# MIC-DKFZ/MultiTalent

Measured on AMD Instinct MI355X. Metric: CT patches/s (48x192x192) train fwd+bwd, higher is better.
Workload: dtype f32; 1 GPU; Task009_Spleen Generic_UNet nc=2 softmax Dice+CE; batch_per_gpu=2, global_batch=2, parallelism=dp1, step=fwd+loss+bwd+clip12+SGD-nesterov, precision=fp32

## Files before the change

multitalent_amd/csrc/conv_bf16.inc:

```
#define BFP 12
#ifndef BF_SWZ
#define BF_SWZ 1
#endif
#define BFP_SWZ 8
#define BF_BPF 6
#ifndef BF_ABL
#define BF_ABL 0
#endif

#include "conv16_common.h"

template <int LD, int LH, int NW> __host__ __device__ constexpr int bstage_rows() { return ((LD * LH + NW - 1) / NW) * NW; }
template <int LD, int LH, int LW, int VEC, int NW, int PITCH = BFP> __host__ __device__ constexpr int bstage_lwp() {
  constexpr int vps = 64 / (FCK / VEC);
  constexpr int padded = ((LW + vps - 1) / vps) * vps;
  return ((size_t)bstage_rows<LD, LH, NW>() * padded * PITCH * 4 <= (PITCH == BFP ? 80 : 40) * 1024) ? padded : LW;
}
template <int LD, int LH, int LW, int VEC, int NW, int PITCH = BFP> __host__ __device__ constexpr size_t bstage_lds_bytes() {
  return (size_t)bstage_rows<LD, LH, NW>() * bstage_lwp<LD, LH, LW, VEC, NW, PITCH>() * PITCH * 4;
}

template <int LD, int LH, int LW, int VEC, int NW, int XS = MT_F32, int MTY = MT_BF16, int PITCH = BFP>
__device__ __forceinline__ void mt_stage_bf16(unsigned* __restrict__ lds, const mt_conv3d_t& c, const ConvChunk ch,
                                              int nb, int ud0, int uh0, int uw0, int lane, int wave) {
  constexpr int EB = mt_ebytes<XS>();
  constexpr bool XB = XS != MT_F32;
  constexpr int LPV = FCK / VEC, VPS = 64 / LPV, NI = (LW + VPS - 1) / VPS, R = LD * LH, RPW = (R + NW - 1) / NW;
  constexpr int LWP = bstage_lwp<LD, LH, LW, VEC, NW, PITCH>();
  constexpr bool PADW = LWP >= NI * VPS;
  constexpr bool SWZ = PITCH == BFP_SWZ;
  constexpr int RG = (RPW * NI * VEC > 64) ? (RPW + 1) / 2 : RPW;
  typedef float f32x2 __attribute__((ext_vector_type(2)));
  const mt_src_t& S = c.src[ch.src];
  const int cl = (lane % LPV) * VEC, vl = lane / LPV;
  const bool has_aff = S.scale != nullptr;
  float sc[VEC], sh[VEC];
#pragma unroll
  for (int e = 0; e < VEC; ++e) {
    const bool cv = (cl + e) < ch.ck;
    sc[e] = cv ? 1.f : 0.f; sh[e] = 0.f;
    if (has_aff && cv) {
      sc[e] = S.scale[(size_t)nb * S.C + ch.c0 + cl + e];
      sh[e] = S.shift[(size_t)nb * S.C + ch.c0 + cl + e];
    }
  }
  const float slope = has_aff ? S.slope : 1.f;
  const int cs = S.cs;
  const size_t sample_elems = (size_t)c.Di * c.Hi * c.Wi * cs;
  __amdgpu_buffer_rsrc_t rsrc =
      __builtin_amdgcn_make_buffer_rsrc((void*)((const char*)S.ptr + (size_t)nb * sample_elems * EB), 0, (int)(sample_elems * EB), 0x00020000);
  int voff[NI];
  unsigned mval[NI];
#pragma unroll
  for (int i = 0; i < NI; ++i) {
    const int lw = vl + i * VPS;
    const int uw = uw0 + lw;
    const bool ok = (lw < LW) && ((unsigned)uw < (unsigned)c.Wi);
    voff[i] = ok ? (uw * cs + ch.c0 + cl) * EB : (int)0x80000000;
    mval[i] = ok ? 0xffffffffu : 0u;
  }
  unsigned* lbase = lds + (wave * LWP + vl) * PITCH + (SWZ ? (cl & 7) / 2 : cl / 2);
  int hoff[NI];
#pragma unroll
  for (int i = 0; i < NI; ++i) hoff[i] = SWZ ? (((cl >> 3) ^ ((vl + i * VPS) >> 3)) & 1) * 4 : 0;
  const int rowbytes = c.Wi * cs * EB;
  if constexpr (XB && XS == MTY && VEC == 4) {
    if (!has_aff) {
      unsigned cm[2];
      cm[0] = ((cl < ch.ck) ? 0x0000ffffu : 0u) | ((cl + 1 < ch.ck) ? 0xffff0000u : 0u);
      cm[1] = ((cl + 2 < ch.ck) ? 0x0000ffffu : 0u) | ((cl + 3 < ch.ck) ? 0xffff0000u : 0u);
#pragma unroll
      for (int r0 = 0; r0 < RPW; r0 += RG) {
        uint2 rw[RG][NI];
#pragma unroll
        for (int q = 0; q < RG; ++q) {
          if (r0 + q < RPW) {
            const int row = wave + NW * (r0 + q);
            const int ld = row / LH, lhh = row - ld * LH;
            const int ud = ud0 + ld, uh = uh0 + lhh;
            const int rm = ((row < R) && ((unsigned)ud < (unsigned)c.Di) && ((unsigned)uh < (unsigned)c.Hi)) ? -1 : 0;
            const int srow = ((ud * c.Hi + uh) & rm) * rowbytes;
            const int oob = ~rm & (int)0x80000000;
#pragma unroll
            for (int i = 0; i < NI; ++i) rw[q][i] = __builtin_bit_cast(uint2, __builtin_amdgcn_raw_buffer_load_b64(rsrc, voff[i] | oob, srow, 0));
          }
        }
#pragma unroll
        for (int q = 0; q < RG; ++q) {
          if (r0 + q < RPW) {
            unsigned* lrow = lbase + NW * (r0 + q) * (LWP * PITCH);
#pragma unroll
            for (int i = 0; i < NI; ++i) {
              if (PADW || (i + 1) * VPS <= LW || vl + i * VPS < LW) {
                uint2 t; t.x = rw[q][i].x & cm[0]; t.y = rw[q][i].y & cm[1];
                *(uint2*)(lrow + i * VPS * PITCH + hoff[i]) = t;
              }
            }
          }
        }
      }
      return;
    }
  }
#pragma unroll
  for (int r0 = 0; r0 < RPW; r0 += RG) {
    float v[RG][NI][VEC];
    int rowm[RG];
#pragma unroll
    for (int q = 0; q < RG; ++q) {
      if (r0 + q < RPW) {
        const int row = wave + NW * (r0 + q);
        const int ld = row / LH, lhh = row - ld * LH;
        const int ud = ud0 + ld, uh = uh0 + lhh;
        rowm[q] = ((row < R) && ((unsigned)ud < (unsigned)c.Di) && ((unsigned)uh < (unsigned)c.Hi)) ? -1 : 0;
        const int srow = ((ud * c.Hi + uh) & rowm[q]) * rowbytes;
        const int oob = ~rowm[q] & (int)0x80000000;
#pragma unroll
        for (int i = 0; i < NI; ++i) {
          if constexpr (XB && VEC == 4) {
            const uint2 t = __builtin_bit_cast(uint2, __builtin_amdgcn_raw_buffer_load_b64(rsrc, voff[i] | oob, srow, 0));
            v[q][i][0] = mt_lo16<XS>(t.x); v[q][i][1] = mt_hi16<XS>(t.x); v[q][i][2] = mt_lo16<XS>(t.y); v[q][i][3] = mt_hi16<XS>(t.y);
          } else if constexpr (XB) {
            const unsigned t = __builtin_amdgcn_raw_buffer_load_b32(rsrc, voff[i] | oob, srow, 0);
            v[q][i][0] = mt_lo16<XS>(t); v[q][i][1] = mt_hi16<XS>(t);
          } else if constexpr (VEC == 4) {
            const f32x4 t = __builtin_bit_cast(f32x4, __builtin_amdgcn_raw_buffer_load_b128(rsrc, voff[i] | oob, srow, 0));
            v[q][i][0] = t[0]; v[q][i][1] = t[1]; v[q][i][2] = t[2]; v[q][i][3] = t[3];
          } else {
            const float2 t = __builtin_bit_cast(float2, __builtin_amdgcn_raw_buffer_load_b64(rsrc, voff[i] | oob, srow, 0));
            v[q][i][0] = t.x; v[q][i][1] = t.y;
          }
        }
      }
    }
#pragma unroll
    for (int q = 0; q < RG; ++q) {
      if (r0 + q < RPW) {
        float scq[VEC], shq[VEC];
#pragma unroll
        for (int e = 0; e < VEC; ++e) {
          scq[e] = __builtin_bit_cast(float, __builtin_bit_cast(unsigned, sc[e]) & (unsigned)rowm[q]);
          shq[e] = __builtin_bit_cast(float, __builtin_bit_cast(unsigned, sh[e]) & (unsigned)rowm[q]);
        }
        unsigned* lrow = lbase + NW * (r0 + q) * (LWP * PITCH);
#pragma unroll
        for (int i = 0; i < NI; ++i) {
          unsigned pk[VEC / 2];
#pragma unroll
          for (int h = 0; h < VEC / 2; ++h) {
            f32x2 xv2, sc2, sh2, sl2;
            xv2[0] = v[q][i][2 * h]; xv2[1] = v[q][i][2 * h + 1];
            sc2[0] = scq[2 * h]; sc2[1] = scq[2 * h + 1]; sh2[0] = shq[2 * h]; sh2[1] = shq[2 * h + 1];
            sl2[0] = slope; sl2[1] = slope;
            const f32x2 t = __builtin_elementwise_fma(xv2, sc2, sh2);
            const f32x2 u = t * sl2;
            pk[h] = mt_pk16<MTY>(fmaxf(t[0], u[0]), fmaxf(t[1], u[1])) & mval[i];
          }
          if (PADW || (i + 1) * VPS <= LW || vl + i * VPS < LW) {
            if constexpr (VEC == 4) {
              uint2 t; t.x = pk[0]; t.y = pk[1];
              *(uint2*)(lrow + i * VPS * PITCH + hoff[i]) = t;
            } else {
              lrow[i * VPS * PITCH + hoff[i]] = pk[0];
            }
          }
        }
      }
    }
  }
}

template <int MT, int NT, int LH, int LW, int KD = 3, int MTY = MT_BF16, int PITCH = BFP>
__device__ __forceinline__ void bf16_chunk(const unsigned* __restrict__ lds, const int (&abase)[MT][3],
                                           const unsigned* __restrict__ wlane, int wstride, f32x16 (&acc)[NT][MT]) {
  constexpr int NTAP = KD * 9;
  constexpr int NB = BF_BPF + 1;
  bf16x8 b[NB][NT];
  bf16x8 a[2][MT];
#pragma unroll
  for (int t = 0; t < BF_BPF; ++t)
#pragma unroll
    for (int n = 0; n < NT; ++n) b[t][n] = *(const bf16x8*)(wlane + n * wstride + t * 256);
#pragma unroll
  for (int m = 0; m < MT; ++m) a[0][m] = *(const bf16x8*)(lds + abase[m][0]);
#pragma unroll
  for (int t = 0; t < NTAP; ++t) {
    if (t + BF_BPF < NTAP)
#pragma unroll
      for (int n = 0; n < NT; ++n) b[(t + BF_BPF) % NB][n] = *(const bf16x8*)(wlane + n * wstride + (t + BF_BPF) * 256);
    if (t + 1 < NTAP) {
      const int t1 = t + 1;
      const int toff = (((t1 / 9) * LH + (t1 / 3) % 3) * LW + t1 % 3) * PITCH;
#pragma unroll
      for (int m = 0; m < MT; ++m) a[t1 & 1][m] = *(const bf16x8*)(lds + abase[m][t1 % 3] + toff);
    }
    __builtin_amdgcn_sched_barrier(0);
#pragma unroll
    for (int m = 0; m < MT; ++m)
#pragma unroll
      for (int n = 0; n < NT; ++n)
        acc[n][m] = mt_mfma16<MTY>(a[t & 1][m], b[t % NB][n], acc[n][m]);
    __builtin_amdgcn_sched_barrier(0);
  }
}


template <int MW, int RH, int TD, int VEC, int NT, int NW, int KD = 3, int XS = MT_F32, int OS = MT_F32, int MTY = MT_BF16>
__global__ __launch_bounds__(64 * NW) __attribute__((amdgpu_waves_per_eu(TD == 4 ? 3 : 4))) void conv_bf16_kernel(const ConvKParams P) {
  constexpr bool OB = OS != MT_F32;
  constexpr int MH = 32 / MW, TH = MH * RH, TW = MW, NMT = TD * RH, MT = NMT / NW;
  constexpr int PITCH = BF_SWZ ? BFP_SWZ : BFP;
  constexpr int LD = TD + KD - 1, LH = TH + 2, LW = TW + 2, LWP = bstage_lwp<LD, LH, LW, VEC, NW, PITCH>();
  constexpr int NTAP = KD * 9;
  static_assert(NMT % NW == 0, "M tiles must split over the waves");
  extern __shared__ __attribute__((aligned(16))) unsigned ldsu[];
  const mt_conv3d_t& c = P.c;
  const int tid = threadIdx.x, lane = tid & 63;
  const int wave = __builtin_amdgcn_readfirstlane(tid >> 6);
  const int li = lane & 31, lhalf = lane >> 5;
  int ntile_b, td, th, tw, nb;
  const int tile = mt_block_decode(ntile_b);
  const int ntile0 = ntile_b * NT;
  mt_tile_coords(tile, P.tilesD, P.tilesH, P.tilesW, td, th, tw, nb);
  const int sb = (td * P.tilesH + th) * P.tilesW + tw;
  const int od0 = td * TD, oh0 = th * TH, ow0 = tw * TW;

  int abase[MT][3];
#pragma unroll
  for (int m = 0; m < MT; ++m) {
    const int mt = wave * MT + m;
    const int dm = mt / RH, rh = mt % RH;
    const int r = li / MW, col = li % MW;
#pragma unroll
    for (int kw = 0; kw < 3; ++kw)
      abase[m][kw] = ((dm * LH + rh * MH + r) * LWP + col) * PITCH + (BF_SWZ ? ((lhalf ^ ((col + kw) >> 3)) & 1) : lhalf) * 4;
  }
  f32x16 acc[NT][MT];
#pragma unroll
  for (int n = 0; n < NT; ++n)
#pragma unroll
    for (int m = 0; m < MT; ++m)
#pragma unroll
      for (int j = 0; j < 16; ++j) acc[n][m][j] = 0.f;

  const unsigned* wbase = (const unsigned*)c.wpack;
  const int wstride = P.nchunks * (NTAP * 256);
  for (int ch = 0; ch < P.nchunks; ++ch) {
    const ConvChunk cc = P.chunk[ch];
    const unsigned* wlane = wbase + (size_t)(ntile0 * P.nchunks + ch) * (NTAP * 256) + lane * 4;
    __syncthreads();
    if (!(BF_ABL & 1)) mt_stage_bf16<LD, LH, LW, VEC, NW, XS, MTY, PITCH>(ldsu, c, cc, nb, od0 - (KD - 1) / 2, oh0 - 1, ow0 - 1, lane, wave);
    __syncthreads();
    if (!(BF_ABL & 8)) bf16_chunk<MT, NT, LH, LWP, KD, MTY, PITCH>(ldsu, abase, wlane, wstride, acc);
  }

  if (BF_ABL & 4) { if (acc[0][0][0] == 12345.678f) c.out0[0] = acc[NT - 1][MT - 1][3]; return; }
  float* lds = (float*)ldsu;
  if (c.stats_part != nullptr) __syncthreads();
  float a1[NT], a2[NT];
  bf16_store_tile<MW, RH, TD, NT, NW, OS>(c, acc, wave, lane, nb, od0, oh0, ow0, ntile0, a1, a2);
  if (c.stats_part != nullptr) {
#pragma unroll
    for (int n = 0; n < NT; ++n)
      if (lhalf == 0) { lds[((n * NW + wave) * 32 + li) * 2] = a1[n]; lds[((n * NW + wave) * 32 + li) * 2 + 1] = a2[n]; }
  }
  if (c.stats_part != nullptr) {
    __syncthreads();
    if (tid < 32 * NT) {
      const int n = tid >> 5, l = tid & 31;
      const int co = (ntile0 + n) * 32 + l;
      if (co < c.Cout) {
        float t1 = 0.f, t2 = 0.f;
#pragma unroll
        for (int w = 0; w < NW; ++w) { t1 += lds[((n * NW + w) * 32 + l) * 2]; t2 += lds[((n * NW + w) * 32 + l) * 2 + 1]; }
        float* sp = c.stats_part + ((size_t)((size_t)nb * P.nsb + sb) * c.Cout + co) * 2;
        sp[0] = t1; sp[1] = t2;
      }
    }
  }
}
```

multitalent_amd/csrc/conv_lds.hip:

```cpp
#include "mt_common.h"
#include "bwdw_common.h"
#include "conv_stage.h"
#include <cstring>
#include <stdlib.h>
#include <type_traits>


__device__ __forceinline__ int mt_block_decode(int& ntile) {
  const int ny = (int)gridDim.y;
  const int b = mt_xcd_remap((int)(blockIdx.x + gridDim.x * blockIdx.y), (int)(gridDim.x * ny));
  const int t = b / ny;
  ntile = b - t * ny;
  return t;
}
__device__ __forceinline__ void mt_tile_coords(int tile, int tilesD, int tilesH, int tilesW, int& td, int& th, int& tw, int& nb) {
  td = tile % tilesD; tile /= tilesD;
  th = tile % tilesH; tile /= tilesH;
  tw = tile % tilesW;
  nb = tile / tilesW;
}

template <int CK, int LD, int LH, int LW>
__device__ __forceinline__ void mt_stage_fast(float* __restrict__ lds, const mt_conv3d_t& c, const ConvChunk ch,
                                              int nb, int ud0, int uh0, int uw0, int lane, int wave) {
// ... 392 lines not shown
    a[0][m][1] = *(const f32x4*)(lds + abase[m] + 4);
  }
#pragma unroll
  for (int t = 0; t < NTAP; ++t) {
    if (t + CF_BPF < NTAP && !(CF_ABL & 64)) {
      b[(t + CF_BPF) % NB][0] = *(const f32x4*)(wlane + (t + CF_BPF) * 512);
      b[(t + CF_BPF) % NB][1] = *(const f32x4*)(wlane + (t + CF_BPF) * 512 + 256);
    }
    if (t + 1 < NTAP && !(CF_ABL & 32)) {
      const int t1 = t + 1;
      const int toff = (((t1 / 9) * LH + (t1 / 3) % 3) * LW + t1 % 3) * FCKP;
#pragma unroll
      for (int m = 0; m < MT; ++m) {
        a[t1 & 1][m][0] = *(const f32x4*)(lds + abase[m] + toff);
        a[t1 & 1][m][1] = *(const f32x4*)(lds + abase[m] + toff + 4);
      }
    }
    __builtin_amdgcn_sched_barrier(0);
#pragma unroll
    for (int kp = 0; kp < 8; ++kp)
#pragma unroll
      for (int m = 0; m < MT; ++m)
        acc[m] = __builtin_amdgcn_mfma_f32_32x32x2f32(a[(CF_ABL & 32) ? 0 : (t & 1)][m][kp >> 2][kp & 3], b[(CF_ABL & 64) ? 0 : (t % NB)][kp >> 2][kp & 3], acc[m], 0, 0, 0);
    __builtin_amdgcn_sched_barrier(0);
  }
}

template <int MW, int RH, int TD, int VEC, int KD = 3>
__global__ __launch_bounds__(256) void conv_fast_kernel(const ConvKParams P) {
  constexpr int MH = 32 / MW, TH = MH * RH, TW = MW, NMT = TD * RH, MT = NMT / 4;
  constexpr int LD = TD + KD - 1, LH = TH + 2, LW = TW + 2, LWP = stage_lwp<LD, LH, LW, VEC>();
  static_assert(NMT % 4 == 0, "M tiles must split over 4 waves");
  extern __shared__ __attribute__((aligned(16))) float lds[];
  const mt_conv3d_t& c = P.c;
  const int tid = threadIdx.x, lane = tid & 63;
  const int wave = __builtin_amdgcn_readfirstlane(tid >> 6);
  const int li = lane & 31, lhalf = lane >> 5;
  int ntile, td, th, tw, nb;
  mt_tile_coords(mt_block_decode(ntile), P.tilesD, P.tilesH, P.tilesW, td, th, tw, nb);
  const int sb = (td * P.tilesH + th) * P.tilesW + tw;
  const int od0 = td * TD, oh0 = th * TH, ow0 = tw * TW;

  int abase[MT];
#pragma unroll
  for (int m = 0; m < MT; ++m) {
    const int mt = wave * MT + m;
    const int dm = mt / RH, rh = mt % RH;
    const int r = li / MW, col = li % MW;
    abase[m] = ((dm * LH + rh * MH + r) * LWP + col) * FCKP + lhalf * 8;
  }
  f32x16 acc[MT];
#pragma unroll
  for (int m = 0; m < MT; ++m)
#pragma unroll
    for (int j = 0; j < 16; ++j) acc[m][j] = 0.f;

  for (int ch = 0; ch < P.nchunks; ++ch) {
    const ConvChunk cc = P.chunk[ch];
    const float* wlane = c.wpack + (size_t)(ntile * P.nchunks + ch) * (KD * 9 * 512) + lane * 4;
    if (!(CF_ABL & 16)) __syncthreads();
    if (!(CF_ABL & 1)) mt_stage_fast2<LD, LH, LW, VEC>(lds, c, cc, nb, od0 - (KD - 1) / 2, oh0 - 1, ow0 - 1, lane, wave);
    if (!(CF_ABL & 16)) __syncthreads();
    if (!(CF_ABL & 8)) fast_chunk<MT, LH, LWP, KD>(lds, abase, wlane, acc);
  }

  if (CF_ABL & 4) { if (acc[0][0] == 12345.678f) c.out0[0] = acc[MT - 1][3]; return; }
  const int co = ntile * 32 + li;
  const bool covalid = co < c.Cout;
  const float bv = (c.bias != nullptr && covalid) ? c.bias[co] : 0.f;
  float* optr; int ocs, cofs;
  if (co < c.csplit) { optr = c.out0; ocs = c.ocs0; cofs = co; }
  else               { optr = c.out1; ocs = c.ocs1; cofs = co - c.csplit; }
  float s1 = 0.f, s2 = 0.f;
  const bool interior = (od0 + TD <= c.Do) && (oh0 + TH <= c.Ho) && (ow0 + TW <= c.Wo);
  const size_t out_sample = (size_t)c.Do * c.Ho * c.Wo;
  __amdgpu_buffer_rsrc_t r0d = __builtin_amdgcn_make_buffer_rsrc((void*)(c.out0 + (size_t)nb * out_sample * c.ocs0), 0,
                                                                 (int)(out_sample * c.ocs0 * 4), 0x00020000);
  const bool split = c.csplit < c.Cout;
  __amdgpu_buffer_rsrc_t r1d = r0d;
  if (split) r1d = __builtin_amdgcn_make_buffer_rsrc((void*)(c.out1 + (size_t)nb * out_sample * c.ocs1), 0,
                                                     (int)(out_sample * c.ocs1 * 4), 0x00020000);
  const bool use1 = split && !(co < c.csplit);
  (void)optr;
  const int lane_col = 4 * lhalf;
  const int loff = covalid ? (lane_col * ocs + cofs) * 4 : (int)0x80000000;
#pragma unroll
  for (int m = 0; m < MT; ++m) {
    const int mt = wave * MT + m;
    const int dm = mt / RH, rh = mt % RH;
    const int od = od0 + dm;
    const int vox0 = ((od * c.Ho) + (oh0 + rh * MH)) * c.Wo + ow0;
    auto jgeom = [&](int j, int& off, int& so0, int& so1) {
      const int ivj = (j & 3) + 8 * (j >> 2);
      const int r = ivj / MW, colj = ivj % MW;
      off = loff;
      if (!interior) {
        const bool ok = (od < c.Do) && (oh0 + rh * MH + r < c.Ho) && (ow0 + colj + lane_col < c.Wo);
        off = ok ? loff : (int)0x80000000;
      }
      so0 = (vox0 + r * c.Wo + colj) * c.ocs0 * 4;
      so1 = (vox0 + r * c.Wo + colj) * c.ocs1 * 4;
    };
    float prev[16];
    if (c.accumulate) {
#pragma unroll
      for (int j = 0; j < 16; ++j) {
        int off, so0, so1; jgeom(j, off, so0, so1);
        if (!split) prev[j] = __builtin_bit_cast(float, __builtin_amdgcn_raw_buffer_load_b32(r0d, off, so0, 0));
        else {
          const int offa = use1 ? (int)0x80000000 : off, offb = use1 ? off : (int)0x80000000;
          prev[j] = __builtin_bit_cast(float, __builtin_amdgcn_raw_buffer_load_b32(r0d, offa, so0, 0)) +
                    __builtin_bit_cast(float, __builtin_amdgcn_raw_buffer_load_b32(r1d, offb, so1, 0));
        }
      }
    }
#pragma unroll
    for (int j = 0; j < 16; ++j) {
      int off, so0, so1; jgeom(j, off, so0, so1);
      float v = acc[m][j] + bv;
      if (c.accumulate) v += prev[j];
      if (!split) {
        __builtin_amdgcn_raw_buffer_store_b32(__builtin_bit_cast(unsigned, v), r0d, off, so0, 0);
      } else {
        const int offa = use1 ? (int)0x80000000 : off, offb = use1 ? off : (int)0x80000000;
        __builtin_amdgcn_raw_buffer_store_b32(__builtin_bit_cast(unsigned, v), r0d, offa, so0, 0);
        __builtin_amdgcn_raw_buffer_store_b32(__builtin_bit_cast(unsigned, v), r1d, offb, so1, 0);
      }
      if (interior) { s1 += v; s2 = fmaf(v, v, s2); }
      else if (off >= 0) { s1 += v; s2 = fmaf(v, v, s2); }
    }
  }
  if (!covalid) { s1 = 0.f; s2 = 0.f; }
  if (c.stats_part != nullptr) {
    s1 += __shfl_xor(s1, 32, 64);
    s2 += __shfl_xor(s2, 32, 64);
    __syncthreads();
    if (lhalf == 0) { lds[(wave * 32 + li) * 2] = s1; lds[(wave * 32 + li) * 2 + 1] = s2; }
    __syncthreads();
    if (tid < 32 && (ntile * 32 + tid) < c.Cout) {
      float t1 = 0.f, t2 = 0.f;
#pragma unroll
      for (int w = 0; w < 4; ++w) { t1 += lds[(w * 32 + tid) * 2]; t2 += lds[(w * 32 + tid) * 2 + 1]; }
      float* sp = c.stats_part + ((size_t)((size_t)nb * P.nsb + sb) * c.Cout + ntile * 32 + tid) * 2;
      sp[0] = t1; sp[1] = t2;
    }
  }
}

#include "conv_bf16.inc"

#ifndef FS_ABL
#define FS_ABL 0
#endif
template <int SD, int SH, int SW, int VEC, bool BF = false, int XS = MT_F32, int OS = MT_F32, int MTY = MT_BF16>
__global__ __launch_bounds__(256) void conv_fast_strided_kernel(const ConvKParams P) {
  static_assert(BF || (XS == MT_F32 && OS == MT_F32), "16-bit storage is served by the 16-bit matrix path");
  constexpr bool OB = OS != MT_F32;
  constexpr int TD = 2, TH = 4, TW = 8;
  constexpr int LD = (TD - 1) * SD + 3, LH = (TH - 1) * SH + 3, LW = (TW - 1) * SW + 3;
  constexpr int LWP = BF ? bstage_lwp<LD, LH, LW, VEC, 4>() : stage_lwp<LD, LH, LW, VEC>();
  constexpr int PITCH = BF ? BFP : FCKP;
  extern __shared__ __attribute__((aligned(16))) float lds[];
  const mt_conv3d_t& c = P.c;
  const int tid = threadIdx.x, lane = tid & 63;
  const int wave = __builtin_amdgcn_readfirstlane(tid >> 6);
  const int li = lane & 31, lhalf = lane >> 5;
  int by, td, th, tw, nb;
  mt_tile_coords(mt_block_decode(by), P.tilesD, P.tilesH, P.tilesW, td, th, tw, nb);
  const int dm = wave & 1, nt2 = wave >> 1;
  const int ntile_raw = by * 2 + nt2;
  const bool nt_ok = ntile_raw * 32 < c.Cout;
  const int ntile = nt_ok ? ntile_raw : 0;
  const int sb = (td * P.tilesH + th) * P.tilesW + tw;
  const int od0 = td * TD, oh0 = th * TH, ow0 = tw * TW;

  int abase[1];
  abase[0] = ((dm * SD * LH + (li >> 3) * SH) * LWP + (li & 7) * SW) * PITCH + lhalf * (BF ? 4 : 8);
  f32x16 accb[1][1];
  f32x16 (&acc)[1] = accb[0];
#pragma unroll
  for (int j = 0; j < 16; ++j) acc[0][j] = 0.f;

  for (int ch = 0; ch < P.nchunks; ++ch) {
    const ConvChunk cc = P.chunk[ch];
    __syncthreads();
    if constexpr (BF) {
      const unsigned* wlane = (const unsigned*)c.wpack + (size_t)(ntile * P.nchunks + ch) * (27 * 256) + lane * 4;
      mt_stage_bf16<LD, LH, LW, VEC, 4, XS, MTY>((unsigned*)lds, c, cc, nb, od0 * SD - 1, oh0 * SH - 1, ow0 * SW - 1, lane, wave);
      __syncthreads();
      const int abase3[1][3] = {{abase[0], abase[0], abase[0]}};
      bf16_chunk<1, 1, LH, LWP, 3, MTY>((const unsigned*)lds, abase3, wlane, 0, accb);
    } else {
      const float* wlane = c.wpack + (size_t)(ntile * P.nchunks + ch) * (27 * 512) + lane * 4;
      if (!(FS_ABL & 1)) mt_stage_fast2<LD, LH, LW, VEC>(lds, c, cc, nb, od0 * SD - 1, oh0 * SH - 1, ow0 * SW - 1, lane, wave);
      __syncthreads();
      if (!(FS_ABL & 8)) fast_chunk<1, LH, LWP>(lds, abase, wlane, acc);
    }
  }
  if ((FS_ABL & 4) && acc[0][0] != 12345.f) return;

  const int co = ntile_raw * 32 + li;
  const bool covalid = nt_ok && co < c.Cout;
  const float bv = (c.bias != nullptr && covalid) ? c.bias[co] : 0.f;
  const int ocs = c.ocs0;
  const size_t out_sample = (size_t)c.Do * c.Ho * c.Wo;
  constexpr int OEB = mt_ebytes<OS>();
  __amdgpu_buffer_rsrc_t rd = __builtin_amdgcn_make_buffer_rsrc((void*)((char*)c.out0 + (size_t)nb * out_sample * ocs * OEB), 0,
                                                                (int)(out_sample * ocs * OEB), 0x00020000);
  const int od = od0 + dm;
  float s1 = 0.f, s2 = 0.f;
  if constexpr (OB) {
    const bool odd = li & 1;
    const int coe = co & ~1;
    const bool pvalid = nt_ok && coe + 1 < c.Cout;
    float q1[2] = {0.f, 0.f}, q2[2] = {0.f, 0.f};
#pragma unroll
    for (int j = 0; j < 16; j += 2) {
      const int iv = (j & 3) + 8 * (j >> 2) + 4 * lhalf + (odd ? 1 : 0);
      const int oh = oh0 + (iv >> 3), ow = ow0 + (iv & 7);
      const bool ok = pvalid && (od < c.Do) && (oh < c.Ho) && (ow < c.Wo);
      const int off = ok ? (((od * c.Ho + oh) * c.Wo + ow) * ocs + coe) * 2 : (int)0x80000000;
      float a, b;
      mt_pair_exchange(acc[0][j] + bv, acc[0][j + 1] + bv, odd, a, b);
      if (c.accumulate) { const unsigned pv = __builtin_amdgcn_raw_buffer_load_b32(rd, off, 0, 0); a += mt_lo16<OS>(pv); b += mt_hi16<OS>(pv); }
      const unsigned pk = mt_pk16<OS>(a, b);
      __builtin_amdgcn_raw_buffer_store_b32(pk, rd, off, 0, 0);
      if (ok) {
        const float ar = mt_lo16<OS>(pk), br = mt_hi16<OS>(pk);
        q1[0] += ar; q2[0] = fmaf(ar, ar, q2[0]); q1[1] += br; q2[1] = fmaf(br, br, q2[1]);
      }
    }
    s1 = mt_pair_combine(q1[0], q1[1], odd);
    s2 = mt_pair_combine(q2[0], q2[1], odd);
  } else {
#pragma unroll
  for (int j = 0; j < 16; ++j) {
    const int iv = (j & 3) + 8 * (j >> 2) + 4 * lhalf;
    const int oh = oh0 + (iv >> 3), ow = ow0 + (iv & 7);
    const bool ok = covalid && (od < c.Do) && (oh < c.Ho) && (ow < c.Wo);
    const int off = ok ? (((od * c.Ho + oh) * c.Wo + ow) * ocs + co) * 4 : (int)0x80000000;
    float v = acc[0][j] + bv;
    if (c.accumulate) v += __builtin_bit_cast(float, __builtin_amdgcn_raw_buffer_load_b32(rd, off, 0, 0));
    __builtin_amdgcn_raw_buffer_store_b32(__builtin_bit_cast(unsigned, v), rd, off, 0, 0);
    if (ok) { s1 += v; s2 = fmaf(v, v, s2); }
  }
  }
  if (c.stats_part != nullptr) {
    s1 += __shfl_xor(s1, 32, 64);
    s2 += __shfl_xor(s2, 32, 64);
    __syncthreads();
    if (lhalf == 0) { lds[(wave * 32 + li) * 2] = s1; lds[(wave * 32 + li) * 2 + 1] = s2; }
    __syncthreads();
    if (tid < 64) {
      const int n2 = tid >> 5, cl = tid & 31;
      const int cg = (by * 2 + n2) * 32 + cl;
      if (cg < c.Cout) {
        const float t1 = lds[((n2 * 2) * 32 + cl) * 2] + lds[((n2 * 2 + 1) * 32 + cl) * 2];
        const float t2 = lds[((n2 * 2) * 32 + cl) * 2 + 1] + lds[((n2 * 2 + 1) * 32 + cl) * 2 + 1];
        float* sp = c.stats_part + ((size_t)((size_t)nb * P.nsb + sb) * c.Cout + cg) * 2;
        sp[0] = t1; sp[1] = t2;
      }
    }
  }
}

#ifndef TS_ABL
#define TS_ABL 0
#endif
template <int VEC, bool BF = false, int XS = MT_F32, int OS = MT_F32, int MTY = MT_BF16, int SD = 1, int SH = 1, int SW = 1>
__global__ __launch_bounds__(256) void conv_tapsplit_kernel(const ConvKParams P) {
  static_assert(BF || (XS == MT_F32 && OS == MT_F32), "16-bit storage is served by the 16-bit matrix path");
  constexpr int TD = 2, TH = 4, TW = 4, LD = (TD - 1) * SD + 3, LH = (TH - 1) * SH + 3, LW = (TW - 1) * SW + 3;
  constexpr int LWP = BF ? bstage_lwp<LD, LH, LW, VEC, 4>() : stage_lwp<LD, LH, LW, VEC>();
  constexpr int PITCH = BF ? BFP : FCKP;
  extern __shared__ __attribute__((aligned(16))) float lds[];
  const mt_conv3d_t& c = P.c;
  const int tid = threadIdx.x, lane = tid & 63;
  const int wave = __builtin_amdgcn_readfirstlane(tid >> 6);
  const int li = lane & 31, lhalf = lane >> 5;
  int ntile, td, th, tw, nb;
  mt_tile_coords(mt_block_decode(ntile), P.tilesD, P.tilesH, P.tilesW, td, th, tw, nb);
  const int sb = (td * P.tilesH + th) * P.tilesW + tw;
  const int od0 = td * TD, oh0 = th * TH, ow0 = tw * TW;
  const int abase = (((li >> 4) * SD * LH + ((li >> 2) & 3) * SH) * LWP + (li & 3) * SW) * PITCH + lhalf * (BF ? 4 : 8);

  f32x16 acc;
#pragma unroll
  for (int j = 0; j < 16; ++j) acc[j] = 0.f;

  for (int ch = 0; ch < P.nchunks; ++ch) {
    const ConvChunk cc = P.chunk[ch];
    __syncthreads();
    if constexpr (BF) {
      mt_stage_bf16<LD, LH, LW, VEC, 4, XS, MTY>((unsigned*)lds, c, cc, nb, od0 * SD - 1, oh0 * SH - 1, ow0 * SW - 1, lane, wave);
      __syncthreads();
      const unsigned* ldsu = (const unsigned*)lds;
      const unsigned* wl = (const unsigned*)c.wpack + (size_t)(ntile * P.nchunks + ch) * (27 * 256) + lane * 4;
      bf16x8 fa[7], fb[7];
#pragma unroll
      for (int i = 0; i < 7; ++i) {
        const int tt = (wave + 4 * i) < 27 ? wave + 4 * i : 26;
        fa[i] = *(const bf16x8*)(ldsu + abase + (((tt / 9) * LH + (tt / 3) % 3) * LWP + tt % 3) * PITCH);
        fb[i] = *(const bf16x8*)(wl + tt * 256);
      }
#pragma unroll
      for (int i = 0; i < 7; ++i)
        if (i < 6 || wave < 3) acc = mt_mfma16<MTY>(fa[i], fb[i], acc);
      continue;
    }
    const float* wlane = c.wpack + ((TS_ABL & 2) ? (size_t)0 : (size_t)(ntile * P.nchunks + ch) * (27 * 512)) + lane * 4;
    if (!(TS_ABL & 1)) mt_stage_fast2<LD, LH, LW, VEC>(lds, c, cc, nb, od0 * SD - 1, oh0 * SH - 1, ow0 * SW - 1, lane, wave);
    __syncthreads();
    f32x4 a[2][2], b[2][2];
    {
      const int t = wave;
      const int toff = (((t / 9) * LH + (t / 3) % 3) * LWP + t % 3) * FCKP;
      a[0][0] = *(const f32x4*)(lds + abase + toff); a[0][1] = *(const f32x4*)(lds + abase + toff + 4);
      b[0][0] = *(const f32x4*)(wlane + t * 512);    b[0][1] = *(const f32x4*)(wlane + t * 512 + 256);
    }
#pragma unroll
    for (int i = 0; i < 7; ++i) {
      const int t = wave + 4 * i, t1 = t + 4;
      if (i + 1 < 7) {
        const int tt = t1 < 27 ? t1 : 26;
        const int toff = (((tt / 9) * LH + (tt / 3) % 3) * LWP + tt % 3) * FCKP;
        a[(i + 1) & 1][0] = *(const f32x4*)(lds + abase + toff); a[(i + 1) & 1][1] = *(const f32x4*)(lds + abase + toff + 4);
        b[(i + 1) & 1][0] = *(const f32x4*)(wlane + tt * 512);   b[(i + 1) & 1][1] = *(const f32x4*)(wlane + tt * 512 + 256);
      }
      if (i < 6 || wave < 3) {
        if (TS_ABL & 4) { acc[0] += a[i & 1][0][0] + a[i & 1][1][3] + b[i & 1][0][1] + b[i & 1][1][2]; continue; }
#pragma unroll
        for (int kp = 0; kp < 8; ++kp)
          acc = __builtin_amdgcn_mfma_f32_32x32x2f32(a[i & 1][kp >> 2][kp & 3], b[i & 1][kp >> 2][kp & 3], acc, 0, 0, 0);
      }
    }
  }

  __syncthreads();
  float* red = lds;
#pragma unroll
  for (int j = 0; j < 16; ++j) red[(wave * 16 + j) * 64 + lane] = acc[j];
  __syncthreads();
  float v[4];
#pragma unroll
  for (int jj = 0; jj < 4; ++jj) {
    const float* rp = red + ((wave * 4 + jj)) * 64 + lane;
    v[jj] = ((rp[0] + rp[16 * 64]) + rp[32 * 64]) + rp[48 * 64];
  }
  const int co = ntile * 32 + li;
  const bool covalid = co < c.Cout;
// ... 513 lines not shown
}

template <int MT>
__device__ __forceinline__ void rt_frag_load(FastFrag<MT>& f, const float* __restrict__ lds, const int (&abase)[MT], int off,
                                             const float* __restrict__ wq) {
  f.b[0] = *(const f32x4*)(wq);
  f.b[1] = *(const f32x4*)(wq + 256);
#pragma unroll
  for (int m = 0; m < MT; ++m) {
    const float* a = lds + abase[m] + off;
    f.a[m][0] = *(const f32x4*)(a);
    f.a[m][1] = *(const f32x4*)(a + 4);
  }
}

template <int MW, int RH, int TD, int VEC>
__global__ __launch_bounds__(256) void conv_rt_kernel(const ConvKParams P) {
  constexpr int MH = 32 / MW, TH = MH * RH, TW = MW, NMT = TD * RH, MT = NMT / 4;
  static_assert(NMT % 4 == 0, "M tiles must split over 4 waves");
  extern __shared__ __attribute__((aligned(16))) float lds[];
  const mt_conv3d_t& c = P.c;
  const int tid = threadIdx.x, lane = tid & 63;
  const int wave = __builtin_amdgcn_readfirstlane(tid >> 6);
  const int li = lane & 31, lhalf = lane >> 5;
  int ntile, td, th, tw, nb;
  mt_tile_coords(mt_block_decode(ntile), P.tilesD, P.tilesH, P.tilesW, td, th, tw, nb);
  const int sb = (td * P.tilesH + th) * P.tilesW + tw;
  const int LD = (TD - 1) * c.SD + c.KD, LH = (TH - 1) * c.SH + c.KH, LW = (TW - 1) * c.SW + c.KW;
  const int od0 = td * TD, oh0 = th * TH, ow0 = tw * TW;

  int abase[MT];
#pragma unroll
  for (int m = 0; m < MT; ++m) {
    const int mt = wave * MT + m;
    const int dm = mt / RH, rh = mt % RH;
    const int r = li / MW, col = li % MW;
    abase[m] = ((dm * c.SD * LH + (rh * MH + r) * c.SH) * LW + col * c.SW) * FCKP + lhalf * 8;
  }
  f32x16 acc[MT];
#pragma unroll
  for (int m = 0; m < MT; ++m)
#pragma unroll
    for (int j = 0; j < 16; ++j) acc[m][j] = 0.f;

  const int ntaps = P.ntaps;
  const int step_w = FCKP, step_h = (LW - c.KW) * FCKP, step_d = (LH - c.KH) * LW * FCKP;
  for (int ch = 0; ch < P.nchunks; ++ch) {
    const ConvChunk cc = P.chunk[ch];
    const float* wq = c.wpack + (size_t)(ntile * P.nchunks + ch) * ntaps * 512 + lane * 4;
    __syncthreads();
    mt_stage_rt<VEC>(lds, c, cc, nb, od0 * c.SD - c.PD, oh0 * c.SH - c.PH, ow0 * c.SW - c.PW, LD, LH, LW, lane, wave);
    __syncthreads();
    FastFrag<MT> f0, f1;
    int off = 0, kw = 0, kh = 0, tap = 0;
    auto advance = [&]() {
      if (tap + 1 < ntaps) {
        off += step_w;
        if (++kw == c.KW) { kw = 0; off += step_h; if (++kh == c.KH) { kh = 0; off += step_d; } }
        wq += 512;
      }
      ++tap;
    };
    rt_frag_load<MT>(f0, lds, abase, off, wq);
    while (tap + 2 <= ntaps) {
      advance();
      __builtin_amdgcn_sched_barrier(0);
      rt_frag_load<MT>(f1, lds, abase, off, wq);
      __builtin_amdgcn_sched_barrier(0);
      fast_frag_mfma<MT>(f0, acc);
      __builtin_amdgcn_sched_barrier(0);
      advance();
      __builtin_amdgcn_sched_barrier(0);
      rt_frag_load<MT>(f0, lds, abase, off, wq);
      __builtin_amdgcn_sched_barrier(0);
      fast_frag_mfma<MT>(f1, acc);
      __builtin_amdgcn_sched_barrier(0);
    }
    if (tap < ntaps) fast_frag_mfma<MT>(f0, acc);
  }

  const int co = ntile * 32 + li;
  const bool covalid = co < c.Cout;
  const float bv = (c.bias != nullptr && covalid) ? c.bias[co] : 0.f;
  const int osD = c.osD > 0 ? c.osD : 1, osH = c.osH > 0 ? c.osH : 1, osW = c.osW > 0 ? c.osW : 1;
  const int OD = c.osD > 0 ? c.OD : c.Do, OH = c.osD > 0 ? c.OH : c.Ho, OW = c.osD > 0 ? c.OW : c.Wo;
  const int ooD = c.osD > 0 ? c.ooD : 0, ooH = c.osD > 0 ? c.ooH : 0, ooW = c.osD > 0 ? c.ooW : 0;
  const bool split = c.csplit < c.Cout;
  const bool use1 = split && co >= c.csplit;
  const int ocs = use1 ? c.ocs1 : c.ocs0;
  const int cofs = use1 ? co - c.csplit : co;
  const size_t out_sample = (size_t)OD * OH * OW;
  __amdgpu_buffer_rsrc_t rd = __builtin_amdgcn_make_buffer_rsrc((void*)(c.out0 + (size_t)nb * out_sample * c.ocs0), 0,
                                                                (int)(out_sample * c.ocs0 * 4), 0x00020000);
  __amdgpu_buffer_rsrc_t rd1 = rd;
  if (split) rd1 = __builtin_amdgcn_make_buffer_rsrc((void*)(c.out1 + (size_t)nb * out_sample * c.ocs1), 0,
                                                     (int)(out_sample * c.ocs1 * 4), 0x00020000);
  const int m0 = use1 ? (int)0x80000000 : 0, m1 = use1 ? 0 : (int)0x80000000;
  const int lane_col = 4 * lhalf;
  float s1 = 0.f, s2 = 0.f;
#pragma unroll
  for (int m = 0; m < MT; ++m) {
    const int mt = wave * MT + m;
    const int dm = mt / RH, rh = mt % RH;
    const int od = od0 + dm;
    auto jgeom = [&](int j, bool& ok) -> int {
      const int ivj = (j & 3) + 8 * (j >> 2);
      const int r = ivj / MW, colj = ivj % MW;
      const int oh = oh0 + rh * MH + r, ow = ow0 + colj + lane_col;
      ok = covalid && (od < c.Do) && (oh < c.Ho) && (ow < c.Wo);
      const int vox = ((od * osD + ooD) * OH + (oh * osH + ooH)) * OW + (ow * osW + ooW);
      return ok ? (vox * ocs + cofs) * 4 : (int)0x80000000;
    };
    float prev[16];
    if (c.accumulate) {
#pragma unroll
      for (int j = 0; j < 16; ++j) {
        bool ok; const int off = jgeom(j, ok);
        prev[j] = __builtin_bit_cast(float, __builtin_amdgcn_raw_buffer_load_b32(rd, off | m0, 0, 0));
        if (split) prev[j] += __builtin_bit_cast(float, __builtin_amdgcn_raw_buffer_load_b32(rd1, off | m1, 0, 0));
      }
    }
#pragma unroll
    for (int j = 0; j < 16; ++j) {
      bool ok; const int off = jgeom(j, ok);
      float v = acc[m][j] + bv;
      if (c.accumulate) v += prev[j];
      __builtin_amdgcn_raw_buffer_store_b32(__builtin_bit_cast(unsigned, v), rd, off | m0, 0, 0);
      if (split) __builtin_amdgcn_raw_buffer_store_b32(__builtin_bit_cast(unsigned, v), rd1, off | m1, 0, 0);
      if (ok) { s1 += v; s2 = fmaf(v, v, s2); }
    }
  }
  if (c.stats_part != nullptr) {
    s1 += __shfl_xor(s1, 32, 64);
    s2 += __shfl_xor(s2, 32, 64);
    __syncthreads();
    if (lhalf == 0) { lds[(wave * 32 + li) * 2] = s1; lds[(wave * 32 + li) * 2 + 1] = s2; }
    __syncthreads();
    if (tid < 32 && (ntile * 32 + tid) < c.Cout) {
      float t1 = 0.f, t2 = 0.f;
#pragma unroll
      for (int w = 0; w < 4; ++w) { t1 += lds[(w * 32 + tid) * 2]; t2 += lds[(w * 32 + tid) * 2 + 1]; }
      float* sp = c.stats_part + ((size_t)((size_t)nb * P.nsb + sb) * c.Cout + ntile * 32 + tid) * 2;
      sp[0] = t1; sp[1] = t2;
    }
  }
}

template <int S> __host__ __device__ constexpr int bd_par(int k) { return S == 2 ? (k == 1 ? 0 : 1) : 0; }
template <int S> __host__ __device__ constexpr int bd_off(int k) { return S == 2 ? (k == 0 ? 1 : 0) : 2 - k; }

#ifndef BDS_ABL
#define BDS_ABL 0
#endif
template <int SD, int SH, int SW, int VEC, bool BF = false, int XS = MT_F32, int OS = MT_F32>
__global__ __launch_bounds__(256) __attribute__((amdgpu_waves_per_eu(2))) void conv_bwdd_strided_kernel(const ConvKParams P) {
  static_assert(BF || (XS == MT_F32 && OS == MT_F32), "16-bit storage is served by the bf16 matrix path");
  constexpr bool OB = OS != MT_F32;
  constexpr int TD = 2, TH = 4, TW = 16;
  constexpr int LD = TD + (SD == 2 ? 1 : 2), LH = TH + (SH == 2 ? 1 : 2), LW = TW + (SW == 2 ? 1 : 2);
  constexpr int NC = SD * SH * SW, LWP = BF ? bstage_lwp<LD, LH, LW, VEC, 4>() : stage_lwp<LD, LH, LW, VEC>();
  constexpr int PITCH = BF ? BFP : FCKP;
  extern __shared__ __attribute__((aligned(16))) float lds[];
  const mt_conv3d_t& c = P.c;
  const int tid = threadIdx.x, lane = tid & 63;
  const int wave = __builtin_amdgcn_readfirstlane(tid >> 6);
  const int li = lane & 31, lhalf = lane >> 5;
  int ntile, td, th, tw, nb;
  mt_tile_coords(mt_block_decode(ntile), P.tilesD, P.tilesH, P.tilesW, td, th, tw, nb);
  const int md0 = td * TD, mh0 = th * TH, mw0 = tw * TW;

  const int dm = wave >> 1, rbase = (wave & 1) * 2;
  const int abase = ((dm * LH + rbase + (li >> 4)) * LWP + (li & 15)) * PITCH + lhalf * (BF ? 4 : 8);

  f32x16 acc[NC];
#pragma unroll
  for (int q = 0; q < NC; ++q)
#pragma unroll
    for (int j = 0; j < 16; ++j) acc[q][j] = 0.f;

  for (int ch = 0; ch < P.nchunks; ++ch) {
    const ConvChunk cc = P.chunk[ch];
    const float* wlane = c.wpack + (size_t)(ntile * P.nchunks + ch) * (27 * 512) + lane * 4;
    __syncthreads();
    if constexpr (BF) {
      mt_stage_bf16<LD, LH, LW, VEC, 4, XS, MT_BF16>((unsigned*)lds, c, cc, nb, md0 - (SD == 1 ? 1 : 0), mh0 - (SH == 1 ? 1 : 0), mw0 - (SW == 1 ? 1 : 0), lane, wave);
      __syncthreads();
      const unsigned* ldsu = (const unsigned*)lds;
      const unsigned* wl = (const unsigned*)c.wpack + (size_t)(ntile * P.nchunks + ch) * (27 * 256) + lane * 4;
      constexpr int BPF = 5, NB = BPF + 1;
      bf16x8 b[NB], a[2];
#pragma unroll
      for (int t = 0; t < BPF; ++t) b[t] = *(const bf16x8*)(wl + t * 256);
      {
        constexpr int o0 = ((bd_off<SD>(0) * LH + bd_off<SH>(0)) * LWP + bd_off<SW>(0)) * PITCH;
        a[0] = *(const bf16x8*)(ldsu + abase + o0);
      }
#pragma unroll
      for (int t = 0; t < 27; ++t) {
        if (t + BPF < 27) b[(t + BPF) % NB] = *(const bf16x8*)(wl + (t + BPF) * 256);
        if (t + 1 < 27) {
          const int t1 = t + 1;
          const int o1 = ((bd_off<SD>(t1 / 9) * LH + bd_off<SH>((t1 / 3) % 3)) * LWP + bd_off<SW>(t1 % 3)) * PITCH;
          a[t1 & 1] = *(const bf16x8*)(ldsu + abase + o1);
        }
        __builtin_amdgcn_sched_barrier(0);
        const int q = (bd_par<SD>(t / 9) * SH + bd_par<SH>((t / 3) % 3)) * SW + bd_par<SW>(t % 3);
        acc[q] = __builtin_amdgcn_mfma_f32_32x32x16_bf16(a[t & 1], b[t % NB], acc[q], 0, 0, 0);
        __builtin_amdgcn_sched_barrier(0);
      }
      continue;
    }
    if (!(BDS_ABL & 1)) mt_stage_fast2<LD, LH, LW, VEC>(lds, c, cc, nb, md0 - (SD == 1 ? 1 : 0), mh0 - (SH == 1 ? 1 : 0), mw0 - (SW == 1 ? 1 : 0), lane, wave);
    __syncthreads();
    if (BDS_ABL & 2) wlane = c.wpack + lane * 4;
    {
      constexpr int NB = 4;
      f32x4 b[NB][2];
      f32x4 a[2][2];
#pragma unroll
      for (int t = 0; t < 3; ++t) {
        b[t][0] = *(const f32x4*)(wlane + t * 512);
        b[t][1] = *(const f32x4*)(wlane + t * 512 + 256);
      }
      {
        constexpr int o0 = ((bd_off<SD>(0) * LH + bd_off<SH>(0)) * LWP + bd_off<SW>(0)) * FCKP;
        a[0][0] = *(const f32x4*)(lds + abase + o0);
        a[0][1] = *(const f32x4*)(lds + abase + o0 + 4);
      }
#pragma unroll
      for (int t = 0; t < 27; ++t) {
        if (t + 3 < 27 && !(BDS_ABL & 2)) {
          b[(t + 3) % NB][0] = *(const f32x4*)(wlane + (t + 3) * 512);
          b[(t + 3) % NB][1] = *(const f32x4*)(wlane + (t + 3) * 512 + 256);
        }
        if (t + 1 < 27) {
          const int t1 = t + 1;
          const int o1 = ((bd_off<SD>(t1 / 9) * LH + bd_off<SH>((t1 / 3) % 3)) * LWP + bd_off<SW>(t1 % 3)) * FCKP;
          a[t1 & 1][0] = *(const f32x4*)(lds + abase + o1);
          a[t1 & 1][1] = *(const f32x4*)(lds + abase + o1 + 4);
        }
        __builtin_amdgcn_sched_barrier(0);
        const int q = (bd_par<SD>(t / 9) * SH + bd_par<SH>((t / 3) % 3)) * SW + bd_par<SW>(t % 3);
        if (BDS_ABL & 8) { acc[q][0] += a[t & 1][0][0] + a[t & 1][1][3] + b[t % NB][0][1] + b[t % NB][1][2]; continue; }
#pragma unroll
        for (int e = 0; e < 4; ++e) acc[q] = __builtin_amdgcn_mfma_f32_32x32x2f32(a[t & 1][0][e], b[t % NB][0][e], acc[q], 0, 0, 0);
#pragma unroll
        for (int e = 0; e < 4; ++e) acc[q] = __builtin_amdgcn_mfma_f32_32x32x2f32(a[t & 1][1][e], b[t % NB][1][e], acc[q], 0, 0, 0);
        __builtin_amdgcn_sched_barrier(0);
      }
    }
  }

  const int co = ntile * 32 + li;
  const bool covalid = co < c.Cout;
  const int ocs = c.ocs0;
  const size_t out_sample = (size_t)c.OD * c.OH * c.OW;
  constexpr int OEB = mt_ebytes<OS>();
  __amdgpu_buffer_rsrc_t rd = __builtin_amdgcn_make_buffer_rsrc((void*)((char*)c.out0 + (size_t)nb * out_sample * ocs * OEB), 0,
                                                                (int)(out_sample * ocs * OEB), 0x00020000);
  const int md = md0 + dm;
  if (BDS_ABL & 4) { float t = 0.f; for (int q = 0; q < NC; ++q) t += acc[q][3] + acc[q][9]; if (t == 1234.5f) c.out0[0] = t; return; }
  if constexpr (OB) {
    const bool odd = li & 1;
    const int coe = co & ~1;
    const bool pvalid = coe + 1 < c.Cout;
    auto pair_off = [&](int j, int (&off)[NC]) {
      const int iv = (j & 3) + 8 * (j >> 2) + 4 * lhalf + (odd ? 1 : 0);
      const int mh = mh0 + rbase + (iv >> 4), mw = mw0 + (iv & 15);
#pragma unroll
      for (int q = 0; q < NC; ++q) {
        const int pd = q / (SH * SW), ph = (q / SW) % SH, pw = q % SW;
        const int xd = md * SD + pd, xh = mh * SH + ph, xw = mw * SW + pw;
        const bool ok = pvalid && xd < c.OD && xh < c.OH && xw < c.OW;
        off[q] = ok ? (((xd * c.OH + xh) * c.OW + xw) * ocs + coe) * 2 : (int)0x80000000;
      }
    };
    int poff[2][NC];
    unsigned pprev[2][NC];
    pair_off(0, poff[0]);
    if (c.accumulate) {
#pragma unroll
      for (int q = 0; q < NC; ++q) pprev[0][q] = __builtin_amdgcn_raw_buffer_load_b32(rd, poff[0][q], 0, 0);
    }
#pragma unroll
    for (int jp = 0; jp < 8; ++jp) {
      const int j = 2 * jp;
      if (jp + 1 < 8) {
        pair_off(j + 2, poff[(jp + 1) & 1]);
        if (c.accumulate) {
#pragma unroll
          for (int q = 0; q < NC; ++q) pprev[(jp + 1) & 1][q] = __builtin_amdgcn_raw_buffer_load_b32(rd, poff[(jp + 1) & 1][q], 0, 0);
        }
      }
#pragma unroll
      for (int q = 0; q < NC; ++q) {
        float a, b;
        mt_pair_exchange(acc[q][j], acc[q][j + 1], odd, a, b);
        if (c.accumulate) { a += mt_lo16<OS>(pprev[jp & 1][q]); b += mt_hi16<OS>(pprev[jp & 1][q]); }
        __builtin_amdgcn_raw_buffer_store_b32(mt_pk16<OS>(a, b), rd, poff[jp & 1][q], 0, 0);
      }
    }
    return;
  }
  auto row_off = [&](int j, int (&off)[NC]) {
    const int iv = (j & 3) + 8 * (j >> 2) + 4 * lhalf;
    const int mh = mh0 + rbase + (iv >> 4), mw = mw0 + (iv & 15);
#pragma unroll
    for (int q = 0; q < NC; ++q) {
      const int pd = q / (SH * SW), ph = (q / SW) % SH, pw = q % SW;
      const int xd = md * SD + pd, xh = mh * SH + ph, xw = mw * SW + pw;
      const bool ok = covalid && xd < c.OD && xh < c.OH && xw < c.OW;
      off[q] = ok ? (((xd * c.OH + xh) * c.OW + xw) * ocs + co) * 4 : (int)0x80000000;
    }
  };
  int off[2][NC];
  float prev[2][NC];
  row_off(0, off[0]);
  if (c.accumulate) {
#pragma unroll
    for (int q = 0; q < NC; ++q) prev[0][q] = __builtin_bit_cast(float, __builtin_amdgcn_raw_buffer_load_b32(rd, off[0][q], 0, 0));
  }
#pragma unroll
  for (int j = 0; j < 16; ++j) {
    if (j + 1 < 16) {
      row_off(j + 1, off[(j + 1) & 1]);
      if (c.accumulate) {
#pragma unroll
        for (int q = 0; q < NC; ++q)
          prev[(j + 1) & 1][q] = __builtin_bit_cast(float, __builtin_amdgcn_raw_buffer_load_b32(rd, off[(j + 1) & 1][q], 0, 0));
      }
    }
#pragma unroll
    for (int q = 0; q < NC; ++q) {
      float v = acc[q][j];
      if (c.accumulate) v += prev[j & 1][q];
      __builtin_amdgcn_raw_buffer_store_b32(__builtin_bit_cast(unsigned, v), rd, off[j & 1][q], 0, 0);
    }
  }
}

template <int SD, int SH, int SW>
__global__ __launch_bounds__(256) void conv_bwdd_strided_ks_kernel(const ConvKParams P) {
  constexpr int TD = 2, TH = 4, TW = 4;
  constexpr int LD = TD + (SD == 2 ? 1 : 2), LH = TH + (SH == 2 ? 1 : 2), LW = TW + (SW == 2 ? 1 : 2);
  constexpr int NC = SD * SH * SW, LWP = stage_lwp<LD, LH, LW, 2>();
  extern __shared__ __attribute__((aligned(16))) float lds[];
  const mt_conv3d_t& c = P.c;
  const int tid = threadIdx.x, lane = tid & 63;
  const int wave = __builtin_amdgcn_readfirstlane(tid >> 6);
  const int li = lane & 31, lhalf = lane >> 5;
  int ntile, td, th, tw, nb;
  mt_tile_coords(mt_block_decode(ntile), P.tilesD, P.tilesH, P.tilesW, td, th, tw, nb);
  const int md0 = td * TD, mh0 = th * TH, mw0 = tw * TW;
  const int abase = (((li >> 4) * LH + ((li >> 2) & 3)) * LWP + (li & 3)) * FCKP + lhalf * 8 + 2 * wave;

  f32x16 acc[NC];
#pragma unroll
  for (int q = 0; q < NC; ++q)
#pragma unroll
    for (int j = 0; j < 16; ++j) acc[q][j] = 0.f;
// ... 16 lines not shown
    for (int t = 0; t < 27; ++t) {
      if (t + 1 < 27) {
        const int t1 = t + 1;
        const int o1 = ((bd_off<SD>(t1 / 9) * LH + bd_off<SH>((t1 / 3) % 3)) * LWP + bd_off<SW>(t1 % 3)) * FCKP;
        a[t1 & 1] = *(const float2*)(lds + abase + o1);
      }
      const int q = (bd_par<SD>(t / 9) * SH + bd_par<SH>((t / 3) % 3)) * SW + bd_par<SW>(t % 3);
      acc[q] = __builtin_amdgcn_mfma_f32_32x32x2f32(a[t & 1].x, b[t].x, acc[q], 0, 0, 0);
      acc[q] = __builtin_amdgcn_mfma_f32_32x32x2f32(a[t & 1].y, b[t].y, acc[q], 0, 0, 0);
    }
  }

  const int co = ntile * 32 + li;
  const bool covalid = co < c.Cout;
  const int ocs = c.ocs0;
  const size_t out_sample = (size_t)c.OD * c.OH * c.OW;
  __amdgpu_buffer_rsrc_t rd = __builtin_amdgcn_make_buffer_rsrc((void*)(c.out0 + (size_t)nb * out_sample * ocs), 0, (int)(out_sample * ocs * 4), 0x00020000);
  float* red = lds;
  __syncthreads();
#pragma unroll
  for (int q = 0; q < NC; ++q) {
    const int pd = q / (SH * SW), ph = (q / SW) % SH, pw = q % SW;
    int off[4];
    float prev[4];
#pragma unroll
    for (int jj = 0; jj < 4; ++jj) {
      const int iv = jj + 8 * wave + 4 * lhalf;
      const int xd = (md0 + (iv >> 4)) * SD + pd, xh = (mh0 + ((iv >> 2) & 3)) * SH + ph, xw = (mw0 + (iv & 3)) * SW + pw;
      const bool ok = covalid && xd < c.OD && xh < c.OH && xw < c.OW;
      off[jj] = ok ? (((xd * c.OH + xh) * c.OW + xw) * ocs + co) * 4 : (int)0x80000000;
      prev[jj] = 0.f;
      if (c.accumulate) prev[jj] = __builtin_bit_cast(float, __builtin_amdgcn_raw_buffer_load_b32(rd, off[jj], 0, 0));
    }
#pragma unroll
    for (int j = 0; j < 16; ++j) red[(wave * 16 + j) * 64 + lane] = acc[q][j];
    __syncthreads();
#pragma unroll
    for (int jj = 0; jj < 4; ++jj) {
      const float* rp = red + (wave * 4 + jj) * 64 + lane;
      const float v = (((rp[0] + rp[16 * 64]) + rp[32 * 64]) + rp[48 * 64]) + prev[jj];
      __builtin_amdgcn_raw_buffer_store_b32(__builtin_bit_cast(unsigned, v), rd, off[jj], 0, 0);
    }
    __syncthreads();
  }
}

#include "conv_wino.inc"

struct ConvCfg { int MW, RH, TD, CK; };
static const ConvCfg kCfgs[] = {
  {32, 4, 2, 16}, {16, 2, 2, 16}, {8, 2, 2, 16}, {32, 4, 2, 8}, {16, 2, 2, 8}, {8, 2, 2, 8}, {32, 4, 4, 16},
};

static const ConvCfg kBfCfgs[] = { {32, 4, 4, 16}, {32, 4, 2, 16}, {16, 4, 2, 16} };

static void cfg_tile(const ConvCfg& g, int* TD, int* TH, int* TW) {
  *TD = g.TD; *TH = (32 / g.MW) * g.RH; *TW = g.MW;
}
static size_t cfg_lds(const ConvCfg& g, const mt_conv3d_t* p) {
  int TD, TH, TW; cfg_tile(g, &TD, &TH, &TW);
  const size_t LD = (TD - 1) * p->SD + p->KD, LH = (TH - 1) * p->SH + p->KH, LW = (TW - 1) * p->SW + p->KW;
  size_t b = LD * LH * LW * g.CK * sizeof(float);
  return b < 1024 ? 1024 : b;
}
static int pick_cfg(const mt_conv3d_t* p) {
  int best = -1; double bestcost = 1e300;
  for (int i = 0; i < (int)(sizeof(kCfgs) / sizeof(kCfgs[0])); ++i) {
    const ConvCfg& g = kCfgs[i];
    const size_t l = cfg_lds(g, p);
    if (l > 160 * 1024) continue;
    int TD, TH, TW; cfg_tile(g, &TD, &TH, &TW);
    double vol = (double)mt_cdiv(p->Do, TD) * TD * mt_cdiv(p->Ho, TH) * TH * mt_cdiv(p->Wo, TW) * TW;
    double cost = vol;
    if (l > 80 * 1024) cost *= 1.25;
    if (g.CK == 8) cost *= 1.10;
    if (cost < bestcost - 1e-9) { bestcost = cost; best = i; }
  }
  return best;
}

static int conv_validate(const mt_conv3d_t* p) {
  MT_REQUIRE(p != nullptr, "conv3d: null params");
  MT_REQUIRE(p->nsrc == 1 || p->nsrc == 2, "conv3d: nsrc must be 1 or 2 (got %d)", p->nsrc);
  MT_REQUIRE(p->KD >= 1 && p->KD <= 3 && p->KH >= 1 && p->KH <= 3 && p->KW >= 1 && p->KW <= 3, "conv3d: kernel size must be 1..3");
  MT_REQUIRE(p->SD >= 1 && p->SD <= 2 && p->SH >= 1 && p->SH <= 2 && p->SW >= 1 && p->SW <= 2, "conv3d: stride must be 1 or 2");
  MT_REQUIRE((p->dilD == 1 || p->dilD == 2) && (p->dilH == 1 || p->dilH == 2) && (p->dilW == 1 || p->dilW == 2), "conv3d: dilation (zero insertion) must be 1 or 2");
  int csum = p->src[0].C + (p->nsrc == 2 ? p->src[1].C : 0);
  MT_REQUIRE(csum == p->Cin, "conv3d: source channels (%d) != Cin (%d)", csum, p->Cin);
  MT_REQUIRE(p->N > 0 && p->Do > 0 && p->Ho > 0 && p->Wo > 0 && p->Cout > 0 && p->Cin > 0, "conv3d: empty problem");
  MT_REQUIRE(p->wpack != nullptr && p->out0 != nullptr, "conv3d: null pointers");
  MT_REQUIRE(p->csplit >= p->Cout || p->out1 != nullptr, "conv3d: out1 required when csplit < Cout");
  return MT_OK;
}

static bool conv_slopes_ok(const mt_conv3d_t* p) {
  for (int i = 0; i < p->nsrc; ++i)
    if (p->src[i].scale != nullptr && !(p->src[i].slope >= 0.f && p->src[i].slope <= 1.f)) return false;
  return true;
}
static bool conv_is_fast(const mt_conv3d_t* p) {
  if (!conv_slopes_ok(p)) return false;
  if (!(p->KD == 3 && p->KH == 3 && p->KW == 3 && p->SD == 1 && p->SH == 1 && p->SW == 1 && p->PD == 1 && p->PH == 1 &&
        p->PW == 1 && p->dilD == 1 && p->dilH == 1 && p->dilW == 1)) return false;
  for (int i = 0; i < p->nsrc; ++i)
    if ((double)p->Di * p->Hi * p->Wi * p->src[i].cs * 4.0 >= 2147483648.0) return false;
  return true;
}
static bool conv_is_133(const mt_conv3d_t* p) {
  if (!conv_slopes_ok(p)) return false;
  if (!(p->KD == 1 && p->KH == 3 && p->KW == 3 && p->SD == 1 && p->SH == 1 && p->SW == 1 && p->PD == 0 && p->PH == 1 &&
        p->PW == 1 && p->dilD == 1 && p->dilH == 1 && p->dilW == 1)) return false;
  for (int i = 0; i < p->nsrc; ++i)
    if ((double)p->Di * p->Hi * p->Wi * p->src[i].cs * 4.0 >= 2147483648.0) return false;
  return true;
}
static bool out_pairs_aligned(const mt_conv3d_t* p) {
  if ((p->Cout & 1) || (p->ocs0 & 1) || (((uintptr_t)p->out0) & 3)) return false;
  if (p->csplit < p->Cout && ((p->csplit & 1) || (p->ocs1 & 1) || (((uintptr_t)p->out1) & 3))) return false;
  return true;
}
static bool conv_fast_strided_ok(const mt_conv3d_t* p) {
  if (!conv_slopes_ok(p)) return false;
  if (!(p->KD == 3 && p->KH == 3 && p->KW == 3 && p->PD == 1 && p->PH == 1 && p->PW == 1)) return false;
  if (!(p->dilD == 1 && p->dilH == 1 && p->dilW == 1 && p->SH == 2 && p->SW == 2 && (p->SD == 1 || p->SD == 2))) return false;
  if (p->csplit < p->Cout || p->osD > 0) return false;
  for (int i = 0; i < p->nsrc; ++i)
    if ((double)p->Di * p->Hi * p->Wi * p->src[i].cs * 4.0 >= 2147483648.0) return false;
  if ((double)p->Do * p->Ho * p->Wo * p->ocs0 * 4.0 >= 2147483648.0) return false;
  return true;
}
static int conv_bf16_cfg(const mt_conv3d_t* p) {
  const int use = mt_sel3(p, MT_SEL_M16);
  if (!use || !(conv_is_fast(p) || conv_is_133(p)) || p->osD > 0 || p->Cin < 16 || conv_fast_vec(p) != 2) return -1;
  if ((double)p->Do * p->Ho * p->Wo * p->ocs0 * 4.0 >= 2147483648.0) return -1;
  if (p->csplit < p->Cout && (double)p->Do * p->Ho * p->Wo * p->ocs1 * 4.0 >= 2147483648.0) return -1;
  if (mt_cdiv(p->src[0].C, FCK) + (p->nsrc == 2 ? mt_cdiv(p->src[1].C, FCK) : 0) > MT_MAX_CHUNKS) return -1;
  int best = -1; double bestcost = 1e300;
  for (int i = 0; i < (int)(sizeof(kBfCfgs) / sizeof(kBfCfgs[0])); ++i) {
    int TD, TH, TW; cfg_tile(kBfCfgs[i], &TD, &TH, &TW);
    const double vol = (double)mt_cdiv(p->Do, TD) * TD * mt_cdiv(p->Ho, TH) * TH * mt_cdiv(p->Wo, TW) * TW;
    const double halo = (double)(TD + 2) * (TH + 2) * (TW + 2) / ((double)TD * TH * TW);
    const double cost = vol * (0.5 + 0.5 * halo / 2.0);
    if (cost < bestcost - 1e-9) { bestcost = cost; best = i; }
  }
  if (best < 0) return -1;
  int TD, TH, TW; cfg_tile(kBfCfgs[best], &TD, &TH, &TW);
  const long wgs = (long)p->N * mt_cdiv(p->Do, TD) * mt_cdiv(p->Ho, TH) * mt_cdiv(p->Wo, TW) * mt_cdiv(p->Cout, 32);
  if (wgs < 256 && use != 2) return -1;
  return best;
}
static bool strided_use_bf16(const mt_conv3d_t* p) {
  return mt_sel3(p, MT_SEL_M16) && p->mma == 1 && p->Cin >= 16 && conv_fast_vec(p) == 2;
}

static bool conv_x16_geometry_ok(const mt_conv3d_t* p, int cfg) {
  if (cfg != 0 || p->mma != 1) return false;
  const int sd = conv_src_dtype(p);
  if (!mt_is16(sd) || p->odtype != sd || !out_pairs_aligned(p)) return false;
  if (p->csplit < p->Cout || p->osD > 0 || p->bstats.y != nullptr) return false;
  if (!(p->KH == 3 && p->KW == 3 && (p->KD == 3 || p->KD == 1) && p->SD == 1 && p->SH == 1 && p->SW == 1 && p->PH == 1 && p->PW == 1 &&
        p->PD == (p->KD == 3 ? 1 : 0) && p->dilD == 1 && p->dilH == 1 && p->dilW == 1)) return false;
  for (int i = 0; i < p->nsrc; ++i) {
    if ((double)p->Di * p->Hi * p->Wi * p->src[i].cs * 2.0 >= 2147483648.0) return false;
    if ((p->src[i].cs & 1) || (((uintptr_t)p->src[i].ptr) & 3)) return false;
    if (p->src[i].scale != nullptr && !(p->src[i].slope >= 0.f && p->src[i].slope <= 1.f)) return false;
  }
  if ((double)p->Do * p->Ho * p->Wo * p->ocs0 * 2.0 >= 2147483648.0) return false;
  if ((long)p->N * mt_cdiv(p->Do, 4) * mt_cdiv(p->Ho, 4) * mt_cdiv(p->Wo, 32) * mt_cdiv(p->Cout, 32) >= 2147483647L) return false;
  return true;
}
static bool conv_x16_ok(const mt_conv3d_t* p, int cfg) {
  const int g_x16 = mt_sel3(p, MT_SEL_X16);
  if (!g_x16) return false;
  if (g_x16 == 1) {
    const int nch = mt_cdiv(p->src[0].C, FCK) + (p->nsrc == 2 ? mt_cdiv(p->src[1].C, FCK) : 0);
    if (p->Cout > 32 && nch < 8) return false;
  }
  return conv_x16_geometry_ok(p, cfg);
}

static bool wino_persist_geometry_ok(const mt_conv3d_t* p) { return (5.0 * p->Hi + 5.0) * p->Wi + 17.0 < 1048576.0; }
static bool conv_wino_ok(const mt_conv3d_t* p) {
  const int use = mt_sel3(p, MT_SEL_WINO);
  if (!use) return false;
  if (p->Cin < 16 || conv_fast_vec(p) != 2 || !wino_persist_geometry_ok(p)) return false;
  if (p->csplit < p->Cout && (double)p->Do * p->Ho * p->Wo * p->ocs1 * 4.0 >= 2147483648.0) return false;
  if (mt_cdiv(p->src[0].C, WCK) + (p->nsrc == 2 ? mt_cdiv(p->src[1].C, WCK) : 0) > MT_MAX_CHUNKS) return false;
  if ((double)p->Do * p->Ho * p->Wo * p->ocs0 * 4.0 >= 2147483648.0) return false;
  const long wgs = (long)p->N * mt_cdiv(p->Do, 4) * mt_cdiv(p->Ho, 4) * mt_cdiv(p->Wo, 16) * mt_cdiv(p->Cout, 32);
  return wgs >= 256 || use == 2;
}
static bool wino_serves_bwd_stats(const mt_conv3d_t* p) {
  return wino_persist_geometry_ok(p);
}

static bool conv_gather_ok(const mt_conv3d_t* p) {
  if (p->nsrc != 1 || p->csplit < p->Cout || p->osD > 0 || p->stats_part != nullptr) return false;
  if (!(p->KD == p->SD && p->KH == p->SH && p->KW == p->SW && p->PD == 0 && p->PH == 0 && p->PW == 0)) return false;
  if (!(p->dilD == 1 && p->dilH == 1 && p->dilW == 1)) return false;
  if ((double)p->Do * p->Ho * p->Wo * p->ocs0 * 4.0 >= 2147483648.0) return false;
  return true;
}
static bool gather_use_bf16(const mt_conv3d_t* p) {
  return p->mma == 1 && p->src[0].dtype == MT_BF16 && p->src[0].scale == nullptr && !(p->src[0].cs & 1) && !(((uintptr_t)p->src[0].ptr) & 3);
}
#ifndef GATHER_NT2
#define GATHER_NT2 1
#endif
static bool gather_nt2(const mt_conv3d_t* p) {
  if (!(GATHER_NT2 && !gather_use_bf16(p) && p->src[0].dtype == MT_F32 && p->odtype == MT_F32 && p->Cout > 32)) return false;
  const long wgs = (((long)p->Do * p->Ho * p->Wo + 127) / 128) * p->N * mt_cdiv(mt_cdiv(p->Cout, 32), 2);
  return wgs >= 4L * mt_device_cus(mt_current_device());
}

static size_t rt_lds(const ConvCfg& g, const mt_conv3d_t* p) {
  int TD, TH, TW; cfg_tile(g, &TD, &TH, &TW);
  const size_t LD = (TD - 1) * p->SD + p->KD, LH = (TH - 1) * p->SH + p->KH, LW = (TW - 1) * p->SW + p->KW;
  size_t b = LD * LH * LW * FCKP * sizeof(float);
  return b < 1024 ? 1024 : b;
}
static bool conv_rt_ok(const mt_conv3d_t* p) {
  if (!(p->dilD == 1 && p->dilH == 1 && p->dilW == 1)) return false;
  if (p->csplit < p->Cout && (p->osD > 0 || (double)p->Do * p->Ho * p->Wo * p->ocs1 * 4.0 >= 2147483648.0)) return false;
  for (int i = 0; i < p->nsrc; ++i)
    if ((double)p->Di * p->Hi * p->Wi * p->src[i].cs * 4.0 >= 2147483648.0) return false;
  const double od = p->osD > 0 ? (double)p->OD * p->OH * p->OW : (double)p->Do * p->Ho * p->Wo;
  if (od * p->ocs0 * 4.0 >= 2147483648.0) return false;
  return true;
}
static int pick_rt_cfg(const mt_conv3d_t* p) {
  int best = -1; double bestcost = 1e300;
  for (int i = 0; i < 3; ++i) {
    const ConvCfg& g = kCfgs[i];
    const size_t l = rt_lds(g, p);
    if (l > 160 * 1024) continue;
    int TD, TH, TW; cfg_tile(g, &TD, &TH, &TW);
    double cost = (double)mt_cdiv(p->Do, TD) * TD * mt_cdiv(p->Ho, TH) * TH * mt_cdiv(p->Wo, TW) * TW;
    if (l > 80 * 1024) cost *= 1.15;
    if (cost < bestcost - 1e-9) { bestcost = cost; best = i; }
  }
  return best;
}

enum ConvFamily { CONV_NONE = 0, CONV_STEM, CONV_WINO, CONV_WINO_B, CONV_FAST, CONV_TAPSPLIT, CONV_FAST_STRIDED, CONV_BF16, CONV_X16, CONV_GATHER,
                  CONV_RT, CONV_GENERIC };
struct ConvChoice {
  int family;
  ConvCfg g;
  int ck;
  int vec, xs, os, mty;
  bool m16;
  bool nt2;
  bool bstats;
  bool fast;
};
static ConvChoice conv_resolve(const mt_conv3d_t* p) {
  ConvChoice c = {};
  const int cfg = pick_cfg(p), sd = conv_src_dtype(p);
  c.family = cfg < 0 ? CONV_NONE : CONV_GENERIC;
  if (cfg >= 0) c.g = kCfgs[cfg];
  c.ck = c.g.CK; c.vec = conv_fast_vec(p); c.xs = MT_F32; c.os = MT_F32; c.mty = MT_BF16;
  auto strided_instance = [&] {
    c.m16 = strided_use_bf16(p);
    if (c.m16 && sd > 0) { c.vec = 4; c.xs = sd; c.os = p->odtype == sd ? sd : MT_F32; c.mty = sd == MT_F16 ? MT_F16 : MT_BF16; }
  };
  if (p->mma == 1) {
    const int bc = conv_bf16_cfg(p);
    if (bc >= 0) {
      c.family = conv_x16_ok(p, bc) ? CONV_X16 : CONV_BF16;
      c.g = kBfCfgs[bc]; c.ck = FCK; c.m16 = true;
      c.vec = sd > 0 ? 4 : 2; c.xs = c.os = sd > 0 ? sd : MT_F32; c.mty = sd == MT_F16 ? MT_F16 : MT_BF16;
      return c;
    }
  }
  const bool fast = conv_is_fast(p), small = cfg >= 0 && cfg <= 2 && p->osD <= 0;
  const bool out31 = (double)p->Do * p->Ho * p->Wo * p->ocs0 * 4.0 < 2147483648.0;
  if (fast && p->osD <= 0 && p->nsrc == 1 && p->Cin == 1 && p->csplit >= p->Cout && out31) {
    c.family = CONV_STEM; c.g = kCfgs[0]; c.ck = c.g.CK; c.os = p->odtype;
    return c;
  }
  if (fast && small && conv_wino_ok(p)) {
    c.bstats = wino_serves_bwd_stats(p);
    c.family = p->bstats.y != nullptr ? CONV_WINO_B : CONV_WINO; c.ck = WCK;
    return c;
  }
  if (fast && small) {
    c.family = CONV_FAST;
    int TD, TH, TW; cfg_tile(c.g, &TD, &TH, &TW);
    const long wgs = (long)p->N * mt_cdiv(p->Do, TD) * mt_cdiv(p->Ho, TH) * mt_cdiv(p->Wo, TW) * mt_cdiv(p->Cout, 32);
    if (mt_sel3(p, MT_SEL_TAPSPLIT) && wgs < 300 && p->csplit >= p->Cout && out31) { c.family = CONV_TAPSPLIT; strided_instance(); }
    return c;
  }
  if (conv_is_133(p) && small && p->Cin >= 8) { c.family = CONV_FAST; return c; }
  if (conv_fast_strided_ok(p)) {
    c.family = CONV_FAST_STRIDED; c.g = kCfgs[0]; c.ck = c.g.CK;
    strided_instance();
    const int g_tapsplit = mt_sel3(p, MT_SEL_TAPSPLIT);
    const long wgs = (long)p->N * mt_cdiv(p->Do, 2) * mt_cdiv(p->Ho, 4) * mt_cdiv(p->Wo, 8) * mt_cdiv(p->Cout, 64);
    const bool inst = c.m16 ? mt_is16(sd) && (p->odtype == sd || p->odtype == MT_F32) : (sd == MT_F32 && p->odtype == MT_F32 && c.vec == 2);
    if (g_tapsplit && (wgs < 256 || g_tapsplit >= 2) && inst) c.family = CONV_TAPSPLIT;
    return c;
  }
  if (conv_rt_ok(p)) {
    const int i = pick_rt_cfg(p);
    if (i >= 0) {
      c.family = CONV_RT; c.g = kCfgs[i]; c.ck = c.g.CK;
      if (conv_gather_ok(p)) {
        c.family = CONV_GATHER; c.ck = FCK; c.vec = 4; c.xs = p->src[0].dtype; c.os = p->odtype;
        c.m16 = gather_use_bf16(p); c.nt2 = gather_nt2(p);
      }
      return c;
    }
  }
  c.fast = fast && (cfg <= 3 || cfg == 6);
  return c;
}
struct ConvTile { int D, H, W; };
static ConvTile conv_tile(const ConvChoice& c) {
  switch (c.family) {
    case CONV_FAST_STRIDED: return {2, 4, 8};
    case CONV_TAPSPLIT: return {2, 4, 4};
    case CONV_WINO: case CONV_WINO_B: return {4, 4, 16};
    default: { ConvTile t; cfg_tile(c.g, &t.D, &t.H, &t.W); return t; }
  }
}

extern "C" int mt_conv3d_ck(const mt_conv3d_t* p) {
  const ConvChoice c = conv_resolve(p);
  return c.family == CONV_NONE ? -1 : c.ck;
}
extern "C" int mt_conv3d_pack_layout(const mt_conv3d_t* p) {
  const ConvChoice c = conv_resolve(p);
  if (c.m16) return c.mty == MT_F16 ? 4 : 3;
  return (c.family == CONV_WINO || c.family == CONV_WINO_B) ? 2 : 1;
}
extern "C" int mt_conv3d_stats_blocks(const mt_conv3d_t* p) {
  const ConvChoice c = conv_resolve(p);
  if (c.family == CONV_NONE) return -1;
  const ConvTile t = conv_tile(c);
  return mt_cdiv(p->Do, t.D) * mt_cdiv(p->Ho, t.H) * mt_cdiv(p->Wo, t.W);
}
extern "C" int mt_conv3d_bwd_stats_supported(const mt_conv3d_t* p) {
  if (p == nullptr || conv_validate(p) != MT_OK) return 0;
  return conv_resolve(p).bstats ? 1 : 0;
}

static int conv_io_served(const mt_conv3d_t* p, const ConvChoice& c) {
  const int sd = conv_src_dtype(p);
  if (sd < 0 || !mt_dtype_ok(p->odtype)) return 0;
  if (sd == MT_F32 && p->odtype == MT_F32) return 1;
  if (p->bstats.y != nullptr) return 0;
  switch (c.family) {
    case CONV_BF16: case CONV_X16: return (mt_is16(sd) && p->odtype == sd && out_pairs_aligned(p)) ? 1 : 0;
    case CONV_FAST_STRIDED: case CONV_TAPSPLIT:
      return (c.m16 && mt_is16(sd) && (p->odtype == MT_F32 || (p->odtype == sd && out_pairs_aligned(p)))) ? 1 : 0;
    case CONV_STEM: return (sd == MT_F32 && out_pairs_aligned(p)) ? 1 : 0;
    case CONV_GATHER:
      if (sd == MT_F16 || p->odtype == MT_F16) return 0;
      if (sd == MT_BF16 && ((p->src[0].cs & 1) || (((uintptr_t)p->src[0].ptr) & 3))) return 0;
      return (p->odtype == MT_F32 || out_pairs_aligned(p)) ? 1 : 0;
    default: return 0;
  }
}
extern "C" int mt_conv3d_io_supported(const mt_conv3d_t* p) {
  if (p == nullptr) return 0;
  return conv_io_served(p, conv_resolve(p));
}

extern "C" int mt_conv3d_kernel_name(const mt_conv3d_t* p, char* buf, size_t n) {
  if (p == nullptr || buf == nullptr || n == 0) return MT_EINVAL;
  const ConvChoice c = conv_resolve(p);
  const ConvCfg& g = c.g;
  const char* b = c.m16 ? "true" : "false";
  switch (c.family) {
    case CONV_STEM: snprintf(buf, n, "conv_stem_kernel<%d>", c.os); break;
    case CONV_WINO: snprintf(buf, n, "conv_wino8p_kernel"); break;
    case CONV_WINO_B: snprintf(buf, n, "conv_wino8pb_kernel"); break;
    case CONV_FAST: snprintf(buf, n, "conv_fast_kernel<%d, %d, %d, %d, %d>", g.MW, g.RH, g.TD, c.vec, p->KD); break;
    case CONV_TAPSPLIT:
      if (p->SH == 2) snprintf(buf, n, "conv_tapsplit_kernel<%d, %s, %d, %d, %d, %d, 2, 2>", c.vec, b, c.xs, c.os, c.mty, p->SD);
      else snprintf(buf, n, "conv_tapsplit_kernel<%d, %s, %d, %d, %d>", c.vec, b, c.xs, c.os, c.mty);
      break;
    case CONV_FAST_STRIDED: snprintf(buf, n, "conv_fast_strided_kernel<%d, %d, %d, %d, %s, %d, %d, %d>", p->SD, p->SH, p->SW, c.vec, b, c.xs, c.os, c.mty); break;
    case CONV_BF16: snprintf(buf, n, "conv_bf16_kernel<%d, %d, %d, %d, 1, 4, %d, %d, %d, %d>", g.MW, g.RH, g.TD, c.vec, p->KD, c.xs, c.os, c.mty); break;
    case CONV_X16: snprintf(buf, n, "conv_x16_kernel<%d, %d>", p->KD, c.xs); break;
    case CONV_GATHER: snprintf(buf, n, c.m16 ? "conv_gather_kernel<%d, %d, %d, true>" : c.nt2 ? "conv_gather_kernel<%d, %d, %d, false, 2>" : "conv_gather_kernel<%d, %d, %d>", c.vec, c.xs, c.os); break;
    case CONV_RT: snprintf(buf, n, "conv_rt_kernel<%d, %d, %d, %d>", g.MW, g.RH, g.TD, c.vec); break;
    case CONV_GENERIC: snprintf(buf, n, "conv_fwd_kernel<%d, %d, %d, %d, %s>", g.MW, g.RH, g.TD, g.CK, c.fast ? "true" : "false"); break;
    default: return MT_EINVAL;
  }
  return MT_OK;
}

static int conv_fill(ConvKParams& P, const mt_conv3d_t* p, const ConvTile& t, int ntaps, int ck) {
  P.c = *p;
  if (P.c.nsrc == 1) { P.c.src[1] = P.c.src[0]; P.c.src[1].C = 0; }
  P.tilesD = mt_cdiv(p->Do, t.D); P.tilesH = mt_cdiv(p->Ho, t.H); P.tilesW = mt_cdiv(p->Wo, t.W);
  P.nsb = P.tilesD * P.tilesH * P.tilesW;
  P.ntaps = ntaps; P.dbg = 0; P.stagger = 0;
  P.nchunks = mt_build_chunks(p->src[0].C, p->nsrc == 2 ? p->src[1].C : 0, ck, P.chunk);
  MT_REQUIRE(P.nchunks > 0, "conv3d: too many channel chunks (Cin=%d, ck=%d)", p->Cin, ck);
  return MT_OK;
}
template <class K>
static int conv_launch_lds(K kfn, dim3 grid, dim3 block, size_t ldsb, hipStream_t st, const ConvKParams& P, const char* what) {
  if (ldsb > 64 * 1024) {
    hipError_t e = hipFuncSetAttribute((const void*)kfn, hipFuncAttributeMaxDynamicSharedMemorySize, (int)ldsb);
    if (e != hipSuccess) { mt_set_error("conv3d: cannot raise dynamic LDS to %zu: %s", ldsb, hipGetErrorString(e)); return MT_EHIP; }
  }
  hipLaunchKernelGGL(kfn, grid, block, ldsb, st, P);
  MT_CHECK_LAUNCH(what);
  return MT_OK;
}
static dim3 conv_grid(const ConvKParams& P, int cout_per_wg) {
  return dim3((unsigned)(P.nsb * P.c.N), (unsigned)mt_cdiv(P.c.Cout, cout_per_wg), 1);
}

static int launch_fast(const mt_conv3d_t* p, const ConvChoice& c, hipStream_t st) {
  ConvKParams P;
  if (int rc = conv_fill(P, p, conv_tile(c), p->KD * 9, FCK)) return rc;
#define MT_F_INST(MW_, RH_, TD_, VEC_, KD_) \
  conv_launch_lds(conv_fast_kernel<MW_, RH_, TD_, VEC_, KD_>, conv_grid(P, 32), dim3(256), stage_lds_bytes<TD_ + KD_ - 1, (32 / MW_) * RH_ + 2, MW_ + 2, VEC_>(), st, P, "conv3d_fast")
#define MT_F_CASE(MW_, RH_, TD_)                                                                                           \
  if (c.g.MW == MW_) {                                                                                                     \
    if (p->KD == 1) return c.vec == 2 ? MT_F_INST(MW_, RH_, TD_, 2, 1) : MT_F_INST(MW_, RH_, TD_, 1, 1);                   \
    return c.vec == 2 ? MT_F_INST(MW_, RH_, TD_, 2, 3) : MT_F_INST(MW_, RH_, TD_, 1, 3);                                   \
  }
  MT_F_CASE(32, 4, 2)
  MT_F_CASE(16, 2, 2)
  MT_F_CASE(8, 2, 2)
#undef MT_F_CASE
#undef MT_F_INST
  return MT_EINVAL;
}

#define MT_IO16_SWITCH(c_, LAUNCH_)                                                        \
  do {                                                                                     \
    if (c_.xs == MT_F16 && c_.os == MT_F16) LAUNCH_(MT_F16, MT_F16, MT_F16);               \
    else if (c_.xs == MT_F16) LAUNCH_(MT_F16, MT_F32, MT_F16);                             \
    else if (c_.os == MT_BF16) LAUNCH_(MT_BF16, MT_BF16, MT_BF16);                         \
    else LAUNCH_(MT_BF16, MT_F32, MT_BF16);                                                \
  } while (0)

template <int SD>
static int launch_fast_strided_t(const mt_conv3d_t* p, const ConvChoice& c, hipStream_t st) {
  constexpr int TD = 2, TH = 4, TW = 8, LD = (TD - 1) * SD + 3, LH = (TH - 1) * 2 + 3, LW = (TW - 1) * 2 + 3;
  ConvKParams P;
  if (int rc = conv_fill(P, p, conv_tile(c), 27, FCK)) return rc;
  const dim3 grid = conv_grid(P, 64);
#define MT_FS_LAUNCH(XS_, OS_, MTY_) hipLaunchKernelGGL((conv_fast_strided_kernel<SD, 2, 2, 4, true, XS_, OS_, MTY_>), grid, dim3(256), (bstage_lds_bytes<LD, LH, LW, 4, 4>()), st, P)
  if (c.m16 && c.vec == 4) MT_IO16_SWITCH(c, MT_FS_LAUNCH);
  else if (c.m16) hipLaunchKernelGGL((conv_fast_strided_kernel<SD, 2, 2, 2, true, MT_F32, MT_F32, MT_BF16>), grid, dim3(256), (bstage_lds_bytes<LD, LH, LW, 2, 4>()), st, P);
  else if (c.vec == 2) hipLaunchKernelGGL((conv_fast_strided_kernel<SD, 2, 2, 2>), grid, dim3(256), (stage_lds_bytes<LD, LH, LW, 2>()), st, P);
  else return conv_launch_lds(conv_fast_strided_kernel<SD, 2, 2, 1>, grid, dim3(256), stage_lds_bytes<LD, LH, LW, 1>(), st, P, "conv3d_fast_strided");
#undef MT_FS_LAUNCH
  MT_CHECK_LAUNCH("conv3d_fast_strided");
  return MT_OK;
}

template <int SD, int S2>
static void launch_tapsplit_t(const ConvChoice& c, dim3 grid, hipStream_t st, const ConvKParams& P) {
  constexpr int LD = SD + 3, LH = 3 * S2 + 3;
  size_t l = (size_t)4 * 16 * 64 * sizeof(float);
#define MT_TS_LAUNCH(VEC_, BF_, XS_, OS_, MTY_) hipLaunchKernelGGL((conv_tapsplit_kernel<VEC_, BF_, XS_, OS_, MTY_, SD, S2, S2>), grid, dim3(256), l, st, P)
#define MT_TS_LAUNCH16(XS_, OS_, MTY_) MT_TS_LAUNCH(4, true, XS_, OS_, MTY_)
  if (c.m16 && c.vec == 4) {
    l = std::max(l, bstage_lds_bytes<LD, LH, LH, 4, 4>());
    MT_IO16_SWITCH(c, MT_TS_LAUNCH16);
  } else if (!c.m16 && c.vec == 2) {
    l = std::max(l, stage_lds_bytes<LD, LH, LH, 2>());
    MT_TS_LAUNCH(2, false, MT_F32, MT_F32, MT_BF16);
  } else if constexpr (S2 == 1) {
    if (c.m16) {
      l = std::max(l, bstage_lds_bytes<LD, LH, LH, 2, 4>());
      MT_TS_LAUNCH(2, true, MT_F32, MT_F32, MT_BF16);
    } else {
      l = std::max(l, stage_lds_bytes<LD, LH, LH, 1>());
      MT_TS_LAUNCH(1, false, MT_F32, MT_F32, MT_BF16);
    }
  }
#undef MT_TS_LAUNCH16
#undef MT_TS_LAUNCH
}
static int launch_tapsplit(const mt_conv3d_t* p, const ConvChoice& c, hipStream_t st) {
  ConvKParams P;
  if (int rc = conv_fill(P, p, conv_tile(c), 27, FCK)) return rc;
  const dim3 grid = conv_grid(P, 32);
  if (p->SH != 2) launch_tapsplit_t<1, 1>(c, grid, st, P);
  else if (p->SD == 2) launch_tapsplit_t<2, 2>(c, grid, st, P);
  else launch_tapsplit_t<1, 2>(c, grid, st, P);
  MT_CHECK_LAUNCH("conv3d_tapsplit");
  return MT_OK;
}

static int launch_stem(const mt_conv3d_t* p, const ConvChoice& c, hipStream_t st) {
  ConvKParams P;
  if (int rc = conv_fill(P, p, conv_tile(c), 27, FCK)) return rc;
  const dim3 grid = conv_grid(P, 32);
  if (c.os == MT_F16) hipLaunchKernelGGL((conv_stem_kernel<MT_F16>), grid, dim3(256), 0, st, P);
  else if (c.os == MT_BF16) hipLaunchKernelGGL((conv_stem_kernel<MT_BF16>), grid, dim3(256), 0, st, P);
  else hipLaunchKernelGGL((conv_stem_kernel<MT_F32>), grid, dim3(256), 0, st, P);
  MT_CHECK_LAUNCH("conv3d_stem");
  return MT_OK;
}

template <int MW, int RH, int TD, int VEC, int NT, int NW, int KD = 3, int XS = MT_F32, int OS = MT_F32, int MTY = MT_BF16>
static int launch_bf16_t(const mt_conv3d_t* p, const ConvChoice& c, hipStream_t st) {
  ConvKParams P;
  if (int rc = conv_fill(P, p, conv_tile(c), KD * 9, FCK)) return rc;
  constexpr int TH = (32 / MW) * RH, TW = MW;
  const size_t ldsb = bstage_lds_bytes<TD + KD - 1, TH + 2, TW + 2, VEC, NW, (BF_SWZ ? BFP_SWZ : BFP)>();
  dim3 grid((unsigned)(P.nsb * p->N), (unsigned)mt_cdiv(mt_cdiv(p->Cout, 32), NT), 1);
  return conv_launch_lds(conv_bf16_kernel<MW, RH, TD, VEC, NT, NW, KD, XS, OS, MTY>, grid, dim3(64 * NW), ldsb, st, P, "conv3d_bf16");
}
static int launch_bf16(const mt_conv3d_t* p, const ConvChoice& c, hipStream_t st) {
  MT_REQUIRE(c.xs == conv_src_dtype(p) && c.xs == p->odtype, "conv3d: conv_bf16_kernel takes ONE storage type on all operands (ask mt_conv3d_io_supported)");
#define MT_BF_CASE(MW_, RH_, TD_, NW_)                                                       \
  if (c.g.MW == MW_ && c.g.TD == TD_) {                                                      \
    if (c.xs == MT_F16) return p->KD == 1 ? launch_bf16_t<MW_, RH_, TD_, 4, 1, NW_, 1, MT_F16, MT_F16, MT_F16>(p, c, st) : launch_bf16_t<MW_, RH_, TD_, 4, 1, NW_, 3, MT_F16, MT_F16, MT_F16>(p, c, st); \
    if (c.xs == MT_BF16) return p->KD == 1 ? launch_bf16_t<MW_, RH_, TD_, 4, 1, NW_, 1, MT_BF16, MT_BF16, MT_BF16>(p, c, st) : launch_bf16_t<MW_, RH_, TD_, 4, 1, NW_, 3, MT_BF16, MT_BF16, MT_BF16>(p, c, st); \
    return p->KD == 1 ? launch_bf16_t<MW_, RH_, TD_, 2, 1, NW_, 1>(p, c, st) : launch_bf16_t<MW_, RH_, TD_, 2, 1, NW_>(p, c, st); \
  }
  MT_BF_CASE(32, 4, 4, 4)
  MT_BF_CASE(32, 4, 2, 4)
  MT_BF_CASE(16, 4, 2, 4)
#undef MT_BF_CASE
  mt_set_error("conv3d bf16: bad tile configuration %d x %d x %d", c.g.MW, c.g.RH, c.g.TD);
  return MT_EINVAL;
}

static int launch_x16(const mt_conv3d_t* p, const ConvChoice& c, hipStream_t st) {
  const ConvTile t = conv_tile(c);
  X16Params P;
  P.c = *p;
  if (P.c.nsrc == 1) { P.c.src[1] = P.c.src[0]; P.c.src[1].C = 0; }
  P.tilesD = mt_cdiv(p->Do, t.D); P.tilesH = mt_cdiv(p->Ho, t.H); P.tilesW = mt_cdiv(p->Wo, t.W);
  P.nsb = P.tilesD * P.tilesH * P.tilesW;
  P.ncot = mt_cdiv(p->Cout, 32);
  P.nitems = p->N * P.nsb * P.ncot;
  P.nchunks = mt_build_chunks(p->src[0].C, p->nsrc == 2 ? p->src[1].C : 0, FCK, P.chunk);
  MT_REQUIRE(P.nchunks > 0, "conv3d (x16): too many channel chunks (Cin=%d)", p->Cin);
  P.npairs = 0;
  for (int i = 0; i < P.nchunks; ++P.npairs) {
    const bool two = i + 1 < P.nchunks && P.chunk[i + 1].src == P.chunk[i].src && P.chunk[i + 1].c0 == P.chunk[i].c0 + 16;
    P.pair[P.npairs][0] = (short)i; P.pair[P.npairs][1] = (short)(two ? i + 1 : -1);
    i += two ? 2 : 1;
  }
  P.nwg = mt_conv_x16_workgroups(P.nitems);
  if (p->max_workgroups > 0 && P.nwg > p->max_workgroups) P.nwg = p->max_workgroups;
  return mt_launch_conv_x16(P, p->KD, c.xs, st);
}

static int launch_wino(const mt_conv3d_t* p, const ConvChoice& c, hipStream_t st) {
  MT_REQUIRE(p->bstats.y == nullptr || (c.bstats && p->stats_part != nullptr && p->bstats.mean && p->bstats.rstd &&
                                        p->bstats.c0 >= 0 && p->bstats.C > 0 && p->bstats.c0 + p->bstats.C <= p->Cout),
             "conv3d: bstats set on a problem this kernel does not compute them for (ask mt_conv3d_bwd_stats_supported)");
  ConvKParams P;
  if (int rc = conv_fill(P, p, conv_tile(c), 27, WCK)) return rc;
  const int devid = mt_current_device();
  const size_t l8 = (size_t)(2 * W_RAWF + W_VF) * sizeof(float) + 11 * 256 * 4;
  const int T = P.nsb * p->N, nct = mt_cdiv(p->Cout, 32);
  int nw = mt_device_cus(devid) / nct; if (nw < 1) nw = 1; if (nw > T) nw = T;
  if (p->max_workgroups > 0 && nw > p->max_workgroups) nw = p->max_workgroups;
  const bool b = c.family == CONV_WINO_B;
  static std::atomic<uint64_t> attrb{0}, attrp{0};
  std::atomic<uint64_t>& attr = b ? attrb : attrp;
  if (mt_device_pending(attr, devid)) {
    hipError_t e = hipFuncSetAttribute(b ? (const void*)conv_wino8pb_kernel : (const void*)conv_wino8p_kernel, hipFuncAttributeMaxDynamicSharedMemorySize, (int)l8);
    if (e != hipSuccess) { mt_set_error("conv3d: cannot raise dynamic LDS to %zu: %s", l8, hipGetErrorString(e)); return MT_EHIP; }
    mt_mark_device_done(attr, devid);
  }
  if (b) hipLaunchKernelGGL(conv_wino8pb_kernel, dim3((unsigned)nw, (unsigned)nct, 1), dim3(512), l8, st, P);
  else hipLaunchKernelGGL(conv_wino8p_kernel, dim3((unsigned)nw, (unsigned)nct, 1), dim3(512), l8, st, P);
  MT_CHECK_LAUNCH(b ? "conv3d_wino8pb" : "conv3d_wino8p");
  return MT_OK;
}

static int launch_gather(const mt_conv3d_t* p, const ConvChoice& c, hipStream_t st) {
  ConvKParams P;
  if (int rc = conv_fill(P, p, {1, 1, 1}, p->KD * p->KH * p->KW, FCK)) return rc;
  const long V = (long)p->Do * p->Ho * p->Wo;
  P.tilesD = P.tilesH = P.tilesW = 1; P.nsb = (int)((V + 127) / 128);
  dim3 grid = conv_grid(P, 32);
  if (c.m16 && c.os == MT_BF16) hipLaunchKernelGGL((conv_gather_kernel<4, MT_BF16, MT_BF16, true>), grid, dim3(256), 0, st, P);
  else if (c.m16) hipLaunchKernelGGL((conv_gather_kernel<4, MT_BF16, MT_F32, true>), grid, dim3(256), 0, st, P);
  else if (c.xs == MT_BF16 && c.os == MT_BF16) hipLaunchKernelGGL((conv_gather_kernel<4, MT_BF16, MT_BF16>), grid, dim3(256), 0, st, P);
  else if (c.xs == MT_BF16) hipLaunchKernelGGL((conv_gather_kernel<4, MT_BF16, MT_F32>), grid, dim3(256), 0, st, P);
  else if (c.os == MT_BF16) hipLaunchKernelGGL((conv_gather_kernel<4, MT_F32, MT_BF16>), grid, dim3(256), 0, st, P);
  else if (c.vec == 4 && c.nt2) {
    grid.y = (unsigned)mt_cdiv(mt_cdiv(p->Cout, 32), 2);
    hipLaunchKernelGGL((conv_gather_kernel<4, MT_F32, MT_F32, false, 2>), grid, dim3(256), 0, st, P);
  }
  else if (c.vec == 4) hipLaunchKernelGGL(conv_gather_kernel<4>, grid, dim3(256), 0, st, P);
  else if (c.vec == 2) hipLaunchKernelGGL(conv_gather_kernel<2>, grid, dim3(256), 0, st, P);
  else hipLaunchKernelGGL(conv_gather_kernel<1>, grid, dim3(256), 0, st, P);
  MT_CHECK_LAUNCH("conv3d_gather");
  return MT_OK;
}

static int launch_rt(const mt_conv3d_t* p, const ConvChoice& c, hipStream_t st) {
  ConvKParams P;
  if (int rc = conv_fill(P, p, conv_tile(c), p->KD * p->KH * p->KW, FCK)) return rc;
  const size_t ldsb = rt_lds(c.g, p);
#define MT_RT_CASE(MW_, RH_, TD_)                                                                                              \
  if (c.g.MW == MW_) return c.vec == 2 ? conv_launch_lds(conv_rt_kernel<MW_, RH_, TD_, 2>, conv_grid(P, 32), dim3(256), ldsb, st, P, "conv3d_rt") \
                                       : conv_launch_lds(conv_rt_kernel<MW_, RH_, TD_, 1>, conv_grid(P, 32), dim3(256), ldsb, st, P, "conv3d_rt");
  MT_RT_CASE(32, 4, 2)
  MT_RT_CASE(16, 2, 2)
  MT_RT_CASE(8, 2, 2)
#undef MT_RT_CASE
  return MT_EINVAL;
}

static int launch_generic(const mt_conv3d_t* p, const ConvChoice& c, hipStream_t st) {
  ConvKParams P;
  if (int rc = conv_fill(P, p, conv_tile(c), p->KD * p->KH * p->KW, c.g.CK)) return rc;
  const size_t ldsb = cfg_lds(c.g, p);
#define MT_G_INST(MW_, RH_, TD_, CK_, FAST_) conv_launch_lds(conv_fwd_kernel<MW_, RH_, TD_, CK_, FAST_>, conv_grid(P, 32), dim3(256), ldsb, st, P, "conv3d_fwd")
#define MT_G_IS(MW_, TD_, CK_) (c.g.MW == MW_ && c.g.TD == TD_ && c.g.CK == CK_)
#define MT_G_CASE(MW_, RH_, TD_, CK_) if (MT_G_IS(MW_, TD_, CK_)) return c.fast ? MT_G_INST(MW_, RH_, TD_, CK_, true) : MT_G_INST(MW_, RH_, TD_, CK_, false);
  MT_G_CASE(32, 4, 2, 16)
  MT_G_CASE(16, 2, 2, 16)
  MT_G_CASE(8, 2, 2, 16)
  MT_G_CASE(32, 4, 2, 8)
  if (MT_G_IS(16, 2, 8)) return MT_G_INST(16, 2, 2, 8, false);
  if (MT_G_IS(8, 2, 8)) return MT_G_INST(8, 2, 2, 8, false);
  MT_G_CASE(32, 4, 4, 16)
#undef MT_G_CASE
#undef MT_G_IS
#undef MT_G_INST
  return MT_EINVAL;
}

extern "C" int mt_conv3d_fwd(const mt_conv3d_t* p, mt_stream_t stream) {
  int rc = conv_validate(p);
  if (rc != MT_OK) return rc;
  const ConvChoice c = conv_resolve(p);
  MT_REQUIRE(c.family != CONV_NONE, "conv3d: no tile configuration fits LDS");
  MT_REQUIRE(conv_io_served(p, c), "conv3d: storage types (src %d/%d, out %d) not taken by the kernel that serves this problem "
             "(ask mt_conv3d_io_supported, convert with mt_cast)", p->src[0].dtype, p->nsrc == 2 ? p->src[1].dtype : -1, p->odtype);
  MT_REQUIRE(p->bstats.y == nullptr || c.family == CONV_WINO_B, "conv3d: bstats set on a problem whose kernel does not compute them "
             "(ask mt_conv3d_bwd_stats_supported)");
  MT_REQUIRE(p->osD <= 0 || c.family == CONV_RT, "conv3d: strided output placement needs the runtime-geometry kernel");
  MT_REQUIRE(p->osD <= 0 || (p->stats_part == nullptr && p->osH > 0 && p->osW > 0 &&
             (p->Do - 1) * p->osD + p->ooD < p->OD && (p->Ho - 1) * p->osH + p->ooH < p->OH && (p->Wo - 1) * p->osW + p->ooW < p->OW),
             "conv3d: bad strided output placement");
  hipStream_t st = (hipStream_t)stream;
  switch (c.family) {
    case CONV_STEM: return launch_stem(p, c, st);
    case CONV_WINO: case CONV_WINO_B: return launch_wino(p, c, st);
    case CONV_FAST: return launch_fast(p, c, st);
    case CONV_TAPSPLIT: return launch_tapsplit(p, c, st);
    case CONV_FAST_STRIDED: return p->SD == 2 ? launch_fast_strided_t<2>(p, c, st) : launch_fast_strided_t<1>(p, c, st);
    case CONV_BF16: return launch_bf16(p, c, st);
    case CONV_X16: return launch_x16(p, c, st);
    case CONV_GATHER: return launch_gather(p, c, st);
    case CONV_RT: return launch_rt(p, c, st);
    default: return launch_generic(p, c, st);
  }
}


struct BwddChoice { bool ks, m16; int vec, xs, os; };
static BwddChoice bwdd_resolve(const mt_conv3d_t* p) {
  const mt_src_t& s0 = p->src[0];
  const bool pairs = !((s0.cs & 1) || (s0.C & 1));
  BwddChoice c = {};
  c.m16 = mt_sel3(p, MT_SEL_M16) && p->mma == 1 && p->Cout >= 16 && pairs && !(((uintptr_t)s0.ptr) & (mt_is16(s0.dtype) ? 3 : 7));
  c.vec = (pairs && !(((uintptr_t)s0.ptr) & 7)) ? 2 : 1;
  if (c.m16) {
    const bool yb = s0.dtype == MT_BF16 && p->odtype == MT_BF16;
    c.vec = yb ? 4 : 2; c.xs = yb ? MT_BF16 : MT_F32; c.os = p->odtype == MT_BF16 ? MT_BF16 : MT_F32;
    return c;
  }
  const int g_tapsplit = mt_sel3(p, MT_SEL_TAPSPLIT);
  if (g_tapsplit && s0.dtype == MT_F32 && p->odtype == MT_F32 && c.vec == 2) {
    const long wgs = (long)p->N * mt_cdiv(mt_cdiv(p->Di, p->SD), 2) * mt_cdiv(mt_cdiv(p->Hi, 2), 4) * mt_cdiv(mt_cdiv(p->Wi, 2), 16) * mt_cdiv(p->Cin, 32);
    c.ks = wgs < 256 || g_tapsplit >= 2;
  }
  return c;
}
extern "C" int mt_conv3d_bwd_data_strided_pack_layout(const mt_conv3d_t* p) { return (p != nullptr && bwdd_resolve(p).m16) ? 3 : 1; }
static int bwdd_io_served(const mt_conv3d_t* p, const BwddChoice& c) {
  if (!mt_dtype_ok(p->src[0].dtype) || !mt_dtype_ok(p->odtype)) return 0;
  if (p->src[0].dtype == MT_F32 && p->odtype == MT_F32) return 1;
  if (!c.m16 || p->src[0].dtype == MT_F16) return 0;
  return (p->odtype == MT_BF16 && !(p->Cin & 1) && !(p->ocs0 & 1) && !(((uintptr_t)p->out0) & 3)) ? 1 : 0;
}
extern "C" int mt_conv3d_bwd_data_strided_io_supported(const mt_conv3d_t* p) { return p == nullptr ? 0 : bwdd_io_served(p, bwdd_resolve(p)); }
template <int SD, int SH, int SW>
static int launch_bwdd_strided(const mt_conv3d_t* p, hipStream_t st) {
  constexpr int TD = 2, TH = 4, TW = 16;
  constexpr int LD = TD + (SD == 2 ? 1 : 2), LH = TH + (SH == 2 ? 1 : 2), LW = TW + (SW == 2 ? 1 : 2);
  const BwddChoice c = bwdd_resolve(p);
  MT_REQUIRE(bwdd_io_served(p, c), "bwd_data_strided: storage types not taken by the kernel that serves this problem (ask mt_conv3d_bwd_data_strided_io_supported)");
  const ConvTile t = c.ks ? ConvTile{TD, 4, 4} : ConvTile{TD, TH, TW};
  ConvKParams P;
  if (int rc = conv_fill(P, p, t, 27, FCK)) return rc;
  P.c.Di = p->Do; P.c.Hi = p->Ho; P.c.Wi = p->Wo;
  P.c.OD = p->Di; P.c.OH = p->Hi; P.c.OW = p->Wi;
  P.c.Cin = p->Cout; P.c.Cout = p->Cin;
  P.tilesD = mt_cdiv(mt_cdiv(p->Di, SD), t.D); P.tilesH = mt_cdiv(mt_cdiv(p->Hi, SH), t.H); P.tilesW = mt_cdiv(mt_cdiv(p->Wi, SW), t.W);
  P.nsb = P.tilesD * P.tilesH * P.tilesW;
  const dim3 grid = conv_grid(P, 32);
  if (c.ks) {
    constexpr int KLD = 2 + (SD == 2 ? 1 : 2), KLH = 4 + 1, KLW = 4 + 1;
    size_t l = stage_lds_bytes<KLD, KLH, KLW, 2>(); if (l < (size_t)4 * 16 * 64 * sizeof(float)) l = (size_t)4 * 16 * 64 * sizeof(float);
    hipLaunchKernelGGL((conv_bwdd_strided_ks_kernel<SD, SH, SW>), grid, dim3(256), l, st, P);
    MT_CHECK_LAUNCH("conv_bwdd_strided_ks");
    return MT_OK;
  }
  if (c.m16 && c.vec == 4) hipLaunchKernelGGL((conv_bwdd_strided_kernel<SD, SH, SW, 4, true, MT_BF16, MT_BF16>), grid, dim3(256), (bstage_lds_bytes<LD, LH, LW, 4, 4>()), st, P);
  else if (c.m16 && c.os == MT_BF16) hipLaunchKernelGGL((conv_bwdd_strided_kernel<SD, SH, SW, 2, true, MT_F32, MT_BF16>), grid, dim3(256), (bstage_lds_bytes<LD, LH, LW, 2, 4>()), st, P);
  else if (c.m16) hipLaunchKernelGGL((conv_bwdd_strided_kernel<SD, SH, SW, 2, true>), grid, dim3(256), (bstage_lds_bytes<LD, LH, LW, 2, 4>()), st, P);
  else if (c.vec == 2) hipLaunchKernelGGL((conv_bwdd_strided_kernel<SD, SH, SW, 2>), grid, dim3(256), (stage_lds_bytes<LD, LH, LW, 2>()), st, P);
  else hipLaunchKernelGGL((conv_bwdd_strided_kernel<SD, SH, SW, 1>), grid, dim3(256), (stage_lds_bytes<LD, LH, LW, 1>()), st, P);
  MT_CHECK_LAUNCH("conv_bwdd_strided");
  return MT_OK;
}
extern "C" int mt_conv3d_bwd_data_strided_supported(const mt_conv3d_t* p) {
  if (p == nullptr || p->nsrc != 1) return 0;
  if (p->src[0].scale != nullptr && !(p->src[0].slope >= 0.f && p->src[0].slope <= 1.f)) return 0;
  if (!(p->KD == 3 && p->KH == 3 && p->KW == 3 && p->PD == 1 && p->PH == 1 && p->PW == 1)) return 0;
  if (!(p->dilD == 1 && p->dilH == 1 && p->dilW == 1)) return 0;
  if (!(p->SH == 2 && p->SW == 2 && (p->SD == 1 || p->SD == 2))) return 0;
  if ((double)p->Do * p->Ho * p->Wo * p->src[0].cs * 4.0 >= 2147483648.0) return 0;
  if ((double)p->Di * p->Hi * p->Wi * p->ocs0 * 4.0 >= 2147483648.0) return 0;
  return 1;
}
extern "C" int mt_conv3d_bwd_data_strided_kernel_name(const mt_conv3d_t* p, char* buf, size_t n) {
  if (p == nullptr || buf == nullptr || n == 0 || !mt_conv3d_bwd_data_strided_supported(p)) return MT_EINVAL;
  const BwddChoice c = bwdd_resolve(p);
  if (c.ks) snprintf(buf, n, "conv_bwdd_strided_ks_kernel<%d, 2, 2>", p->SD);
  else snprintf(buf, n, "conv_bwdd_strided_kernel<%d, 2, 2, %d, %s, %d, %d>", p->SD, c.vec, c.m16 ? "true" : "false", c.xs, c.os);
  return MT_OK;
}
extern "C" int mt_conv3d_bwd_data_strided(const mt_conv3d_t* p, mt_stream_t stream) {
  MT_REQUIRE(p != nullptr, "bwd_data_strided: null params");
  MT_REQUIRE(mt_conv3d_bwd_data_strided_supported(p), "bwd_data_strided: unsupported geometry (needs 3x3x3, pad 1, stride (1|2,2,2), one source)");
  MT_REQUIRE(p->src[0].C == p->Cout, "bwd_data_strided: src[0].C (%d) != Cout (%d)", p->src[0].C, p->Cout);
  MT_REQUIRE(p->wpack != nullptr && p->out0 != nullptr && p->src[0].ptr != nullptr, "bwd_data_strided: null pointers");
  hipStream_t st = (hipStream_t)stream;
  return p->SD == 2 ? launch_bwdd_strided<2, 2, 2>(p, st) : launch_bwdd_strided<1, 2, 2>(p, st);
}

struct PackParams {
  const float* w; float* dst;
  int Cout, KD, KH, KW, nkp, nchunks, ntiles, flip, layout;
  int has_tm, tb[3], ts[3];
  int contig;
  long s_ci, s_co, s_kd, s_kh, s_kw;
  ConvChunk chunk[MT_MAX_CHUNKS];
};
#define PACK_TP (16 * 27 + 1)
#define PACK_LDS_BYTES (32 * PACK_TP * 4)
__device__ __forceinline__ void pack_weights_tiled(const PackParams& P, float* __restrict__ tile, int blk, int nblk) {
  const int K3 = P.KD * P.KH * P.KW;
  const int nq = P.layout == 1 ? P.nkp / 4 : 1;
  const int per_tap = nq * 256;
  const int tid = threadIdx.x;
  for (int g = blk; g < P.ntiles * P.nchunks; g += nblk) {
    const int nt = g / P.nchunks, ch = g - nt * P.nchunks;
    const ConvChunk cc = P.chunk[ch];
    const int rowlen = cc.ck * K3;
    __syncthreads();
    {
      float v0[32], v1[32];
      const float* src0 = P.w + (long)(nt * 32) * P.s_co + (long)cc.cglob * K3;
      const int nrow = P.Cout - nt * 32;
#pragma unroll
      for (int co = 0; co < 32; ++co) {
        const float* src = src0 + (long)co * P.s_co;
        v0[co] = (co < nrow && tid < rowlen) ? src[tid] : 0.f;
        v1[co] = (co < nrow && tid + 256 < rowlen) ? src[tid + 256] : 0.f;
      }
#pragma unroll
      for (int co = 0; co < 32; ++co) {
        if (tid < rowlen) tile[co * PACK_TP + tid] = v0[co];
        if (tid + 256 < rowlen) tile[co * PACK_TP + tid + 256] = v1[co];
      }
    }
    __syncthreads();
    float* dst = P.dst + (size_t)g * K3 * per_tap;
    for (int i = tid; i < per_tap; i += 256) {
      const int e = i & 3, l = (i >> 2) & 63, qq = i >> 8;
      const int co = l & 31;
      const int c0 = P.layout == 1 ? (l >> 5) * P.nkp + qq * 4 + e : (l >> 5) * 8 + 2 * e;
      const bool v0 = c0 < cc.ck, v1 = P.layout >= 3 && (c0 + 1) < cc.ck;
      const float* tp = tile + co * PACK_TP + c0 * K3;
      for (int tap = 0; tap < K3; ++tap) {
        const int zt = P.flip ? K3 - 1 - tap : tap;
        const float a0 = v0 ? tp[zt] : 0.f;
        if (P.layout == 1) dst[(size_t)tap * per_tap + i] = a0;
        else {
          const float a1 = v1 ? tp[K3 + zt] : 0.f;
          ((unsigned*)dst)[(size_t)tap * per_tap + i] = P.layout == 3 ? mt_pk16<MT_BF16>(a0, a1) : mt_pk16<MT_F16>(a0, a1);
        }
      }
    }
  }
}
__device__ __forceinline__ void pack_weights_body(const PackParams& P, long first, long stride) {
  if (P.layout == 2) {
    const long total = (long)P.ntiles * P.nchunks * 256;
    for (long i = first; i < total; i += stride) {
      long r = i;
      const int e = (int)(r % 4); r /= 4;
      const int l = (int)(r % 64); r /= 64;
      const int ch = (int)(r % P.nchunks); r /= P.nchunks;
      const int nt = (int)r;
      const ConvChunk cc = P.chunk[ch];
      const int cin_local = 4 * (l >> 5) + e, co = nt * 32 + (l & 31);
      float u[4][4][4];
      if (cin_local < cc.ck && co < P.Cout) {
        const float* wp = P.w + (cc.cglob + cin_local) * P.s_ci + co * P.s_co;
        float g[3][3][3];
#pragma unroll
        for (int kd = 0; kd < 3; ++kd)
#pragma unroll
          for (int kh = 0; kh < 3; ++kh)
#pragma unroll
            for (int kw = 0; kw < 3; ++kw) {
              const int zd = P.flip ? 2 - kd : kd, zh = P.flip ? 2 - kh : kh, zw = P.flip ? 2 - kw : kw;
              g[kd][kh][kw] = wp[zd * P.s_kd + zh * P.s_kh + zw * P.s_kw];
            }
        float t1[3][3][4], t2[3][4][4];
#pragma unroll
        for (int kd = 0; kd < 3; ++kd)
#pragma unroll
          for (int kh = 0; kh < 3; ++kh) {
            const float g0 = g[kd][kh][0], g1 = g[kd][kh][1], g2 = g[kd][kh][2];
            t1[kd][kh][0] = g0; t1[kd][kh][1] = 0.5f * (g0 + g1 + g2); t1[kd][kh][2] = 0.5f * (g0 - g1 + g2); t1[kd][kh][3] = g2;
          }
#pragma unroll
        for (int kd = 0; kd < 3; ++kd)
#pragma unroll
          for (int k = 0; k < 4; ++k) {
            const float g0 = t1[kd][0][k], g1 = t1[kd][1][k], g2 = t1[kd][2][k];
            t2[kd][0][k] = g0; t2[kd][1][k] = 0.5f * (g0 + g1 + g2); t2[kd][2][k] = 0.5f * (g0 - g1 + g2); t2[kd][3][k] = g2;
          }
#pragma unroll
        for (int b = 0; b < 4; ++b)
#pragma unroll
          for (int k = 0; k < 4; ++k) {
            const float g0 = t2[0][b][k], g1 = t2[1][b][k], g2 = t2[2][b][k];
            u[0][b][k] = g0; u[1][b][k] = 0.5f * (g0 + g1 + g2); u[2][b][k] = 0.5f * (g0 - g1 + g2); u[3][b][k] = g2;
          }
      } else {
#pragma unroll
        for (int a = 0; a < 4; ++a)
#pragma unroll
          for (int b = 0; b < 4; ++b)
#pragma unroll
            for (int k = 0; k < 4; ++k) u[a][b][k] = 0.f;
      }
      float* dp = P.dst + ((size_t)(nt * P.nchunks + ch) * 64) * 256 + l * 4 + e;
#pragma unroll
      for (int a = 0; a < 4; ++a)
#pragma unroll
        for (int b = 0; b < 4; ++b)
#pragma unroll
          for (int k = 0; k < 4; ++k) dp[((a * 4 + b) * 4 + k) * 256] = u[a][b][k];
    }
    return;
  }
  if (P.layout == 1 || P.layout == 3 || P.layout == 4) {
    const int K3 = P.KD * P.KH * P.KW;
    const int nq = P.layout == 1 ? P.nkp / 4 : 1;
    const int per_tap = nq * 256;
    const long items = (long)P.ntiles * P.nchunks * per_tap;
    for (long i = first; i < items; i += stride) {
      long r = i;
      const int e = (int)(r % 4); r /= 4;
      const int l = (int)(r % 64); r /= 64;
      const int q = (int)(r % nq); r /= nq;
      const int ch = (int)(r % P.nchunks); r /= P.nchunks;
      const int nt = (int)r;
      const ConvChunk cc = P.chunk[ch];
      const int co = nt * 32 + (l & 31);
      const int c0 = P.layout == 1 ? (l >> 5) * P.nkp + q * 4 + e : (l >> 5) * 8 + 2 * e;
      const bool v0 = c0 < cc.ck && co < P.Cout, v1 = P.layout >= 3 && (c0 + 1) < cc.ck && co < P.Cout;
      const float* w0 = P.w + (long)(cc.cglob + c0) * P.s_ci + (long)co * P.s_co;
      float* dp = P.dst + ((size_t)(nt * P.nchunks + ch) * K3) * per_tap + (q * 64 + l) * 4 + e;
      if (K3 <= 27) {
        float a0[27], a1[27];
#pragma unroll
        for (int tap = 0; tap < 27; ++tap) {
          a0[tap] = 0.f; a1[tap] = 0.f;
          if (tap < K3) {
            const int kw = tap % P.KW, kh = (tap / P.KW) % P.KH, kd = tap / (P.KW * P.KH);
            int zd = P.flip ? P.KD - 1 - kd : kd, zh = P.flip ? P.KH - 1 - kh : kh, zw = P.flip ? P.KW - 1 - kw : kw;
            if (P.has_tm) { zd = P.tb[0] + P.ts[0] * kd; zh = P.tb[1] + P.ts[1] * kh; zw = P.tb[2] + P.ts[2] * kw; }
            const long o = zd * P.s_kd + zh * P.s_kh + zw * P.s_kw;
            if (v0) a0[tap] = w0[o];
            if (v1) a1[tap] = w0[o + P.s_ci];
          }
        }
#pragma unroll
        for (int tap = 0; tap < 27; ++tap)
          if (tap < K3) {
            if (P.layout == 1) dp[(size_t)tap * per_tap] = a0[tap];
            else if (P.layout == 3) ((unsigned*)dp)[(size_t)tap * per_tap] = mt_pk16<MT_BF16>(a0[tap], a1[tap]);
            else ((unsigned*)dp)[(size_t)tap * per_tap] = mt_pk16<MT_F16>(a0[tap], a1[tap]);
          }
        continue;
      }
      int tap = 0;
      for (int kd = 0; kd < P.KD; ++kd)
        for (int kh = 0; kh < P.KH; ++kh)
          for (int kw = 0; kw < P.KW; ++kw, ++tap) {
            int zd = P.flip ? P.KD - 1 - kd : kd, zh = P.flip ? P.KH - 1 - kh : kh, zw = P.flip ? P.KW - 1 - kw : kw;
            if (P.has_tm) { zd = P.tb[0] + P.ts[0] * kd; zh = P.tb[1] + P.ts[1] * kh; zw = P.tb[2] + P.ts[2] * kw; }
            const long o = zd * P.s_kd + zh * P.s_kh + zw * P.s_kw;
            const float a0 = v0 ? w0[o] : 0.f;
            if (P.layout == 1) dp[(size_t)tap * per_tap] = a0;
            else if (P.layout == 3) ((unsigned*)dp)[(size_t)tap * per_tap] = mt_pk16<MT_BF16>(a0, v1 ? w0[o + P.s_ci] : 0.f);
            else ((unsigned*)dp)[(size_t)tap * per_tap] = mt_pk16<MT_F16>(a0, v1 ? w0[o + P.s_ci] : 0.f);
          }
    }
    return;
  }
  const long total = (long)P.ntiles * P.nchunks * P.KD * P.KH * P.KW * P.nkp * 64;
  for (long i = first; i < total; i += stride) {
    long r = i;
    int l, kp;
    if (P.layout == 1) {
      const int e = (int)(r % 4); r /= 4;
      l = (int)(r % 64); r /= 64;
      const int q = (int)(r % (P.nkp / 4)); r /= (P.nkp / 4);
      kp = q * 4 + e;
    } else {
      l = (int)(r % 64); r /= 64;
      kp = (int)(r % P.nkp); r /= P.nkp;
    }
    const int kw = (int)(r % P.KW); r /= P.KW;
    const int kh = (int)(r % P.KH); r /= P.KH;
    const int kd = (int)(r % P.KD); r /= P.KD;
    const int ch = (int)(r % P.nchunks); r /= P.nchunks;
    const int nt = (int)r;
    const ConvChunk cc = P.chunk[ch];
    const int cin_local = (P.layout == 1) ? (l >> 5) * P.nkp + kp : 2 * kp + (l >> 5);
    const int co = nt * 32 + (l & 31);
    float v = 0.f;
    if (cin_local < cc.ck && co < P.Cout) {
      const int ci = cc.cglob + cin_local;
      int zd = P.flip ? P.KD - 1 - kd : kd, zh = P.flip ? P.KH - 1 - kh : kh, zw = P.flip ? P.KW - 1 - kw : kw;
      if (P.has_tm) { zd = P.tb[0] + P.ts[0] * kd; zh = P.tb[1] + P.ts[1] * kh; zw = P.tb[2] + P.ts[2] * kw; }
      v = P.w[ci * P.s_ci + co * P.s_co + zd * P.s_kd + zh * P.s_kh + zw * P.s_kw];
    }
    P.dst[i] = v;
  }
}
__global__ void pack_weights_kernel(const PackParams P) {
  pack_weights_body(P, (long)blockIdx.x * blockDim.x + threadIdx.x, (long)gridDim.x * blockDim.x);
}
__global__ __launch_bounds__(256) void pack_weights_batched_kernel(const PackParams* __restrict__ tab) {
  extern __shared__ __attribute__((aligned(16))) float pack_tile[];
  const PackParams& P = tab[blockIdx.y];
  if (P.contig && (P.layout == 1 || P.layout >= 3)) { pack_weights_tiled(P, pack_tile, (int)blockIdx.x, (int)gridDim.x); return; }
  pack_weights_body(P, (long)blockIdx.x * blockDim.x + threadIdx.x, (long)gridDim.x * blockDim.x);
}

static int pack_fill(PackParams& P, size_t* packed_floats, const float* w, float* dst, int C0, int C1, int Cout, int KD, int KH,
                     int KW, long s_ci, long s_co, long s_kd, long s_kh, long s_kw, int flip, int ck, int layout,
                     const int32_t* tapmap) {
  MT_REQUIRE(ck >= 2 && (ck % 2) == 0, "pack: ck must be even (got %d)", ck);
  MT_REQUIRE(layout == 0 || (layout == 1 && (ck % 8) == 0) || (layout == 2 && ck == 8 && KD == 3 && KH == 3 && KW == 3 && tapmap == nullptr) ||
             ((layout == 3 || layout == 4) && ck == 16),
             "pack: layout 1 needs ck %% 8 == 0; layout 2 (Winograd) needs ck == 8 and a 3x3x3 kernel; layouts 3 / 4 (bf16 / fp16) need ck == 16");
  std::memset((void*)&P, 0, sizeof(P));
  P.nchunks = mt_build_chunks(C0, C1, ck, P.chunk);
  MT_REQUIRE(P.nchunks > 0, "pack: too many chunks");
  P.ntiles = mt_cdiv(Cout, 32);
  P.nkp = ck / 2;
  if (packed_floats) *packed_floats = layout == 2 ? (size_t)P.ntiles * P.nchunks * 64 * 256
                                    : layout >= 3 ? (size_t)P.ntiles * P.nchunks * KD * KH * KW * 256
                                                  : (size_t)P.ntiles * P.nchunks * KD * KH * KW * P.nkp * 64;
  P.w = w; P.dst = dst; P.Cout = Cout; P.KD = KD; P.KH = KH; P.KW = KW; P.flip = flip; P.layout = layout;
  P.has_tm = tapmap != nullptr;
  for (int d = 0; d < 3; ++d) { P.tb[d] = tapmap ? tapmap[2 * d] : 0; P.ts[d] = tapmap ? tapmap[2 * d + 1] : 1; }
  P.s_ci = s_ci; P.s_co = s_co; P.s_kd = s_kd; P.s_kh = s_kh; P.s_kw = s_kw;
  P.contig = (tapmap == nullptr && ck <= 16 && KD * KH * KW <= 27 && s_kw == 1 && s_kh == KW && s_kd == (long)KH * KW && s_ci == (long)KD * KH * KW) ? 1 : 0;
  return MT_OK;
}
extern "C" size_t mt_pack_desc_size(void) { return sizeof(PackParams); }
extern "C" int mt_pack_desc_fill(void* desc, const float* w, float* dst, int C0, int C1, int Cout, int KD, int KH, int KW,
                                 long s_ci, long s_co, long s_kd, long s_kh, long s_kw, int flip, int ck, int layout,
                                 const int32_t* tapmap) {
  MT_REQUIRE(desc != nullptr && w != nullptr && dst != nullptr, "pack_desc_fill: null pointers");
  return pack_fill(*(PackParams*)desc, nullptr, w, dst, C0, C1, Cout, KD, KH, KW, s_ci, s_co, s_kd, s_kh, s_kw, flip, ck, layout, tapmap);
}
static unsigned g_pack_blocks() {
  constexpr int v = 1024;
  return (unsigned)v;
}
extern "C" int mt_pack_batched(const void* descs_device, int n, mt_stream_t stream) {
  MT_REQUIRE(descs_device != nullptr && n > 0, "pack_batched: empty table");
  hipLaunchKernelGGL(pack_weights_batched_kernel, dim3(g_pack_blocks(), (unsigned)n, 1), dim3(256), PACK_LDS_BYTES, (hipStream_t)stream,
                     (const PackParams*)descs_device);
  MT_CHECK_LAUNCH("pack_weights_batched");
  return MT_OK;
}

extern "C" int mt_pack_conv_weights(const float* w, float* dst, size_t* packed_floats, int C0, int C1, int Cout,
                                    int KD, int KH, int KW, long s_ci, long s_co, long s_kd, long s_kh, long s_kw,
                                    int flip, int ck, int layout, const int32_t* tapmap, mt_stream_t stream) {
  PackParams P;
  size_t total = 0;
  int rc = pack_fill(P, &total, w, dst, C0, C1, Cout, KD, KH, KW, s_ci, s_co, s_kd, s_kh, s_kw, flip, ck, layout, tapmap);
  if (rc != MT_OK) return rc;
  if (packed_floats) *packed_floats = total;
  if (dst == nullptr) return MT_OK;
  MT_REQUIRE(w != nullptr, "pack: null weights");
  int blocks = mt_cdiv((long)total, 256); if (blocks > 4096) blocks = 4096;
  hipLaunchKernelGGL(pack_weights_kernel, dim3(blocks), dim3(256), 0, (hipStream_t)stream, P);
  MT_CHECK_LAUNCH("pack_weights");
  return MT_OK;
}
```

multitalent_amd/engine.py:

```python
import contextlib
import os

import torch
from torch import nn

from . import ops
from .ops import Act, ConvGeom

LRELU_DEFAULT = 1e-2


class Val:

    def __init__(self, name, C):
        self.name, self.C = name, C
        self.act = None
        self.grad = None
        self.grad_init = False
        self.spatial = None


class _Op:
    params = ()

    def plan(self, eng, N):
        raise NotImplementedError

    def param_list(self):
        return []

    def inputs(self):
        return []


def _strides(w, **kw):
    return ops.conv_weight_strides(w, **kw)


class ConvNormOp(_Op):

    def __init__(self, name, srcs, out, conv, norm, lrelu=True, pointwise=False):
        self.name, self.srcs, self.out, self.conv, self.norm, self.lrelu = name, srcs, out, conv, norm, lrelu
        self.kernel = tuple(conv.kernel_size)
        self.stride = tuple(conv.stride)
        self.pad = tuple(conv.padding)
        self.slope = LRELU_DEFAULT
        self.pointwise = pointwise
        self._pw_strided_geom = (not pointwise and self.kernel == (1, 1, 1) and self.stride != (1, 1, 1) and self.pad == (0, 0, 0)
                                 and len(srcs) == 1)
        self.pw_strided = False
        self.bwd_part = None

    def inputs(self):
        return list(self.srcs)

    def param_list(self):
        ps = [self.conv.weight]
        if self.conv.bias is not None:
            ps.append(self.conv.bias)
        if self.norm is not None:
            ps += [self.norm.weight, self.norm.bias]
        return ps

    def plan(self, eng, N):
        dev = eng.device
        sp = self.srcs[0].spatial
        self.geom = ConvGeom(sp, self.kernel, self.stride, self.pad)
        self.out.spatial = self.geom.out
        Cout = self.conv.out_channels
        self.pw_strided = self._pw_strided_geom and tuple(o * st for o, st in zip(self.geom.out, self.stride)) == tuple(self.geom.inp)
        self.mma = eng.mma
        buf = eng.buffer(self.name + '.y', (N,) + self.geom.out + (Cout,), self._out_dtype(eng))
        if self.norm is not None:
            st = eng.buffer(self.name + '.stats', (4, N, Cout))
            self.out.act = Act(buf, scale=st[2], shift=st[3], slope=self.slope if self.lrelu else 1.0, mean=st[0], rstd=st[1])
        else:
            self.out.act = Act(buf)
        self.part = None
        self.wf = self.wb = None

    def _out_dtype(self, eng):
        return eng.val_dtype(self.geom.out)

    def _fwd_io(self, eng):
        Cout = self.conv.out_channels
        acts = [s.act for s in self.srcs]
        if self.pointwise or self.pw_strided:
            def build(ins, outs):
                a = ins[0]
                return ops.fill_pointwise(a, self.geom.out, a.spatial, self.stride, (1, 1, 1), Cout, eng.dummy, self.conv.bias, outs[0],
                                          mma=eng.mma if self.pointwise else 0)
            return eng.io(self.name + '.fwd', acts, [self.out.act], build, ops.pointwise_io_supported)
        build = lambda ins, outs: ops.fill_conv(ins, self.geom, Cout, bias=self.conv.bias, out0=outs[0], mma=self.mma)
        return eng.io(self.name + '.fwd', acts, [self.out.act], build, ops.conv_io_supported)

    def _fwd_params(self, eng, io=None):
        Cout = self.conv.out_channels
        io = io if io is not None else self._fwd_io(eng)
        p = io.build()
        if self.norm is not None and self.part is None:
            nsb = ops.pointwise_stats_blocks(p) if (self.pointwise or self.pw_strided) else ops.conv_stats_blocks(p)
            self.part = eng.buffer(self.name + '.part', (io.ins[0].N, nsb, Cout, 2))
        if self.part is not None:
            p.stats_part = self.part.data_ptr()
        return p

    def pack(self, eng, need_bwd):
        w = self.conv.weight
        Cout = self.conv.out_channels
        C0 = self.srcs[0].C
        C1 = self.srcs[1].C if len(self.srcs) > 1 else 0
        if self.pointwise:
            self.wf = ops.pack_conv_weights(w, C0, 0, Cout, (1, 1, 1), _strides(w), False, ops.POINTWISE_CK, out=self.wf)
            lay = ops.pointwise_pack_layout(self._fwd_io(eng).build())
            self.wf16 = ops.pack_conv_weights(w, C0, 0, Cout, (1, 1, 1), _strides(w), False, ops.POINTWISE_CK, out=getattr(self, 'wf16', None),
                                              layout=lay) if lay != 1 else None
            if need_bwd and self.srcs[0].grad is not None and self.stride == (1, 1, 1):
                self.wb = ops.pack_conv_weights(w, Cout, 0, C0, (1, 1, 1), _strides(w, as_bwd_data=True), False, ops.POINTWISE_CK, out=self.wb)
            return
        if self.pw_strided:
            self.wf = ops.pack_conv_weights(w, C0, 0, Cout, (1, 1, 1), _strides(w), False, ops.POINTWISE_CK, out=self.wf)
            if need_bwd and self.srcs[0].grad is not None:
                self.wb = ops.pack_conv_weights(w, Cout, 0, C0, (1, 1, 1), _strides(w, as_bwd_data=True), False, ops.POINTWISE_CK, out=self.wb)
            return
        p = self._fwd_params(eng)
        self.ck_f = ops.conv_ck(p)
        self.wf = ops.pack_conv_weights(w, C0, C1, Cout, self.kernel, _strides(w), False, self.ck_f, out=self.wf,
                                        layout=ops.conv_pack_layout(p))
        if need_bwd and any(s.grad is not None for s in self.srcs):
            if self._use_strided_bwd(eng):
                self.wb = ops.pack_conv_weights(w, Cout, 0, C0, self.kernel, _strides(w, as_bwd_data=True), False, 16, out=self.wb,
                                                layout=ops.conv_bwd_data_strided_pack_layout(self._strided_bwd_io(eng, None).build()))
                return
            if self._use_parity_classes():
                cls = self._parity_classes()
                if self.wb is None:
                    self.wb = [None] * len(cls)
                for i, (geomc, place, tapmap) in enumerate(cls):
                    pb = ops.fill_conv([eng.as_fp32(Act(self.out.act.buf), geometry_only=True)], geomc, C0, place=place, mma=self.mma)
                    self.wb[i] = ops.pack_conv_weights(w, Cout, 0, C0, geomc.k, _strides(w, as_bwd_data=True), False,
                                                       ops.conv_ck(pb), out=self.wb[i], tapmap=tapmap)
                return
            pb = self._bwd_data_io(eng, None).build()
            self.ck_b = ops.conv_ck(pb)
            self.wb = ops.pack_conv_weights(w, Cout, 0, C0 + C1, self.kernel, _strides(w, as_bwd_data=True), True, self.ck_b, out=self.wb,
                                            layout=ops.conv_pack_layout(pb))

    def _strided_bwd_io(self, eng, g):
        s0 = self.srcs[0]
        gact = Act(g) if g is not None else Act(self._grad_like(eng, self.out))
        dx = Act(s0.grad) if s0.grad is not None else Act(self._grad_like(eng, s0))

        def build(ins, outs):
            p = ops.fill_conv(ins, self.geom, self.conv.out_channels, out0=outs[0], mma=self.mma)
            p.Cin = s0.C
            return p
        return eng.io(self.name + '.bwdd', [gact], [dx], build, ops.conv_bwd_data_strided_io_supported, grad_ins=True)

    def _strided_bwd_params(self, g, eng=None):
        return self._strided_bwd_io(eng if eng is not None else self._eng, g).build()

    @staticmethod
    def _grad_like(eng, val):
        if val.grad is not None:
            return val.grad
        return eng.buffer(val.name + '.grad', tuple(val.act.buf.shape[:4]) + (val.C,), eng.grad_dtype(val.spatial))

    def _use_strided_bwd(self, eng):
        if self.stride == (1, 1, 1) or len(self.srcs) != 1 or self.pointwise:
            return False
        return ops.conv3d_bwd_data_strided_supported(self._strided_bwd_io(eng, None).build())

    def _use_parity_classes(self):
        return self.stride != (1, 1, 1) and len(self.srcs) == 1 and not self.pointwise

    def _parity_classes(self):
        return ops.bwd_data_parity_classes(self.geom)

    def forward(self, eng):
        io = self._fwd_io(eng)
        p = self._fwd_params(eng, io)
        wf = self.wf
        if self.pointwise and ops.pointwise_pack_layout(p) != 1:
            wf = getattr(self, 'wf16', None)
            assert wf is not None, "head: fp16-product launch without fp16 weights (repack after a precision change)"
        p.wpack = wf.data_ptr()
        io.pre()
        if self.pointwise or self.pw_strided:
            ops.pointwise_fwd(p)
        else:
            ops.conv3d_fwd(p)
        io.post()
        if self.norm is not None:
            a = self.out.act
            nsb = self.part.shape[1]
            ops.inorm_finalize(self.part, a.N, nsb, a.C, a.V, self.norm.weight, self.norm.bias, self.norm.eps,
                               a.mean, a.rstd, a.scale, a.shift)

    def _bwd_data_io(self, eng, g):
        Cin = sum(s.C for s in self.srcs)
        geomT = ConvGeom(self.geom.out, self.kernel, (1, 1, 1), tuple(k - 1 - p for k, p in zip(self.kernel, self.pad)),
                         dil=self.stride, out_spatial=self.geom.inp)
        gact = Act(g) if g is not None else Act(self._grad_like(eng, self.out))
        outs = [Act(self._grad_like(eng, s)) for s in self.srcs]

        def build(ins, outs_):
            return ops.fill_conv(ins, geomT, Cin, out0=outs_[0], out1=outs_[1] if len(outs_) > 1 else None,
                                 csplit=self.srcs[0].C if len(outs_) > 1 else None, mma=self.mma)
        return eng.io(self.name + '.bwdd', [gact], outs, build, ops.conv_io_supported, grad_ins=True)

    def backward(self, eng):
        g = self.out.grad
        assert g is not None and self.out.grad_init, "gradient of %s was never produced" % self.name
        gact = Act(g)
        dbias = eng.grad_of(self.conv.bias) if self.conv.bias is not None else None
        if self.norm is not None:
            a = self.out.act
            ws = eng.workspace(ops.inorm_bwd_workspace(a.N, a.V, a.C))
            part, part_c0 = self.bwd_part if self.bwd_part is not None else (None, 0)
            self.bwd_part = None
            ops.inorm_lrelu_bwd(gact, a, self.norm.weight, self.norm.bias, eng.grad_of(self.norm.weight),
                                eng.grad_of(self.norm.bias), dbias, ws, part=part, part_c0=part_c0)
        elif dbias is not None:
            ws = eng.workspace(ops.channel_sum_workspace(gact.N, gact.V, gact.C))
            ops.channel_sum(gact, dbias, False, ws)
        dw = eng.grad_of(self.conv.weight)
        with eng.weight_stream() as side:
            iow = eng.io(self.name + '.bwdw', [s.act for s in self.srcs] + [gact], [],
                         lambda ins, outs: (ops.fill_conv(ins[:-1], self.geom, self.conv.out_channels, mma=self.mma), ins[-1]),
                         lambda py: ops.conv_bwd_weight_io_supported(py[0], py[1]), grad_ins=[False] * len(self.srcs) + [True])
            pw, yact = iow.build()
            iow.pre()
            ws = eng.workspace(ops.conv3d_bwd_weight_workspace(pw), side=side)
            ops.conv3d_bwd_weight(pw, yact, dw, _strides(self.conv.weight), False, ws)
        dsts = [s for s in self.srcs if s.grad is not None]
        if not dsts:
            return
        assert len(dsts) == len(self.srcs)
        inits = {s.grad_init for s in self.srcs}
        assert len(inits) == 1, "mixed accumulate state on the sources of %s" % self.name
        acc = inits.pop()
        if self.pointwise:
            if self.stride != (1, 1, 1):
                raise NotImplementedError("backward-data of a strided pointwise conv is handled by ResBlockOp")
            s0 = self.srcs[0]
            io = eng.io(self.name + '.bwdd', [gact], [Act(s0.grad)],
                        lambda ins, outs: ops.fill_pointwise(ins[0], self.geom.out, self.geom.out, (1, 1, 1), (1, 1, 1), s0.C, self.wb, None, outs[0]),
                        ops.pointwise_io_supported, grad_ins=True)
            p = io.build()
            p.accumulate = io.accumulate(acc)
            io.pre()
            ops.pointwise_fwd(p)
            io.post(acc)
        elif self.pw_strided:
            s0 = self.srcs[0]
            if not acc:
                s0.grad.zero_()
                acc = True

            def build(ins, outs):
                p = ops.fill_pointwise(ins[0], self.geom.out, self.geom.out, (1, 1, 1), self.stride, s0.C, self.wb, None, outs[0])
                p.scatter = 1
                return p
            io = eng.io(self.name + '.bwdd', [gact], [Act(s0.grad)], build, ops.pointwise_io_supported, grad_ins=True)
            p = io.build()
            p.accumulate = io.accumulate(acc)
            for t, _ in io._cout:
                t.buf.zero_()
            io.pre()
            ops.pointwise_fwd(p)
            io.post(acc)
        elif self._use_strided_bwd(eng):
            io = self._strided_bwd_io(eng, g)
            p = io.build()
            p.wpack = self.wb.data_ptr()
            p.accumulate = io.accumulate(acc)
            io.pre()
            ops.conv3d_bwd_data_strided(p)
            io.post(acc)
        elif self._use_parity_classes():
            s0 = self.srcs[0]
            cls = self._parity_classes()
            full = 1
            for st in self.stride:
                full *= st
            if len(cls) < full and not acc:
                s0.grad.zero_()
                acc = True
            gin = eng.as_fp32(gact, reuse=False)
            dx = Act(s0.grad) if s0.grad.dtype == torch.float32 else Act(eng.buffer(self.name + '.bwdd.out0', tuple(s0.grad.shape)))
            if dx.buf is not s0.grad and acc:
                ops.cast(Act(s0.grad), dx)
            for (geomc, place, _), wb in zip(cls, self.wb):
                p = ops.fill_conv([gin], geomc, s0.C, wpack=wb, out0=dx, accumulate=acc, place=place, mma=self.mma)
                ops.conv3d_fwd(p)
            if dx.buf is not s0.grad:
                ops.cast(dx, Act(s0.grad))
        else:
            io = self._bwd_data_io(eng, g)
            p = io.build()
            p.wpack = self.wb.data_ptr()
            p.accumulate = io.accumulate(acc)
            if io.native:
                self._fuse_norm_bwd_stats(eng, p)
            io.pre()
            ops.conv3d_fwd(p)
            io.post(acc)
# ... 97 lines not shown
            ops.conv3d_fwd(p)
            io.post(self.src.grad_init)
            self.src.grad_init = True


class ResAddOp(_Op):

    def __init__(self, name, main, res, out):
        self.name, self.main, self.res, self.out = name, main, res, out
        self.slope = LRELU_DEFAULT

    def inputs(self):
        return [self.main, self.res]

    def plan(self, eng, N):
        self.out.spatial = self.main.spatial
        self.out.act = Act(eng.buffer(self.name + '.a', (N,) + self.main.spatial + (self.main.C,), eng.val_dtype(self.main.spatial)))

    def pack(self, eng, need_bwd):
        pass

    def forward(self, eng):
        m = self.main.act
        y = Act(m.buf, scale=m.scale, shift=m.shift, slope=self.slope)
        ops.inorm_lrelu_apply(y, self.out.act, res=self.res.act)

    def backward(self, eng):
        g = self.out.grad
        assert g is not None and self.out.grad_init
        m, r = self.main.act, self.res.act
        from . import _lib
        import ctypes as C
        gm = self.main.grad
        prod = eng.producer.get(id(self.main)) if eng.fuse_norm_bwd in (1, 3) else None
        nblk = _lib.load().mt_lrelu_bwd_stats_blocks(m.V, m.C)
        gdt, ydt = ops._same_dt(Act(g), Act(gm)), ops._same_dt(m, r)
        if (prod is not None and isinstance(prod, ConvNormOp) and prod.norm is not None and m.mean is not None and nblk > 0
                and g.shape[4] == m.C and gm.shape[4] == m.C and m.cs == m.C and r.cs == m.C):
            part = eng.buffer(self.name + '.bwdpart', (m.N, nblk, m.C, 2))
            _lib.check(_lib.load().mt_lrelu_bwd_stats(
                C.c_void_p(g.data_ptr()), C.c_void_p(m.data_ptr()), ops._ptr(m.scale), ops._ptr(m.shift), self.slope,
                C.c_void_p(r.data_ptr()), ops._ptr(r.scale), ops._ptr(r.shift), r.slope, C.c_void_p(gm.data_ptr()),
                ops._ptr(m.mean), ops._ptr(m.rstd), ops._ptr(part), m.N, m.V, m.C, gdt, ydt, ops._stream()), 'lrelu_bwd_stats')
            prod.bwd_part = (part, 0)
        else:
            _lib.check(_lib.load().mt_lrelu_bwd(
                C.c_void_p(g.data_ptr()), g.shape[4], C.c_void_p(m.data_ptr()), m.cs, ops._ptr(m.scale), ops._ptr(m.shift), self.slope,
                C.c_void_p(r.data_ptr()), r.cs, ops._ptr(r.scale), ops._ptr(r.shift), r.slope,
                C.c_void_p(gm.data_ptr()), gm.shape[4], m.N, m.V, m.C, gdt, ydt, ops._stream()), 'lrelu_bwd')
        self.main.grad_init = True
        if self.res.grad is not None:
            if self.res.grad.data_ptr() == g.data_ptr():
                assert not self.res.grad_init, "gradient of %s was written before its residual add ran backward" % self.res.name
                self.res.grad_init = True
            elif self.res.grad_init:
                self.res.grad.add_(g)
            else:
                self.res.grad.copy_(g)
                self.res.grad_init = True


class HeadOp(ConvNormOp):

    def __init__(self, name, src, out, conv):
        super().__init__(name, [src], out, conv, None, lrelu=False, pointwise=True)

    def _out_dtype(self, eng):
        return torch.float32

    def backward(self, eng):
        s0 = self.srcs[0]
        Cout = self.conv.out_channels
        if s0.grad is None or self.wb is None or not ops.head_bwd_supported(s0.C, Cout) or self.stride != (1, 1, 1):
            return super().backward(eng)
        g = self.out.grad
        assert g is not None and self.out.grad_init, "gradient of %s was never produced" % self.name
        gact = Act(g)
        dbias = eng.grad_of(self.conv.bias) if self.conv.bias is not None else None
        w = self.conv.weight
        st = _strides(w)
        io = eng.io(self.name + '.hbwd', [s0.act], [Act(s0.grad)], lambda ins, outs: (ins[0], outs[0]),
                    lambda xo: ops.head_bwd_io_supported(xo[0], xo[1], Cout))
        a, dx = io.build()
        io.pre()
        ws = eng.workspace(ops.head_bwd_workspace(a.N, a.V, s0.C, Cout))
        done = ops.head_bwd(a, gact, self.wb, dx, bool(io.accumulate(s0.grad_init)), eng.grad_of(w), st[0], st[1], dbias, False, ws)
        io.post(s0.grad_init)
        if dbias is not None and not done:
            ws2 = eng.workspace(ops.channel_sum_workspace(gact.N, gact.V, gact.C))
            ops.channel_sum(gact, dbias, False, ws2)
        s0.grad_init = True


class _IO:

    def __init__(self, eng, key, ins, outs, build, flags, grad_ins):
        self.eng, self._build = eng, build
        cast_in, cast_out = flags
        self.native = not (cast_in or cast_out)
        self._cin = [(a, g) for a, g in zip(ins, grad_ins) if cast_in and a.dtype != torch.float32]
        self.ins = [eng.as_fp32(a, geometry_only=True) if (cast_in and a.dtype != torch.float32) else a for a in ins]
        self._cout = []
        self.outs = []
        for i, o in enumerate(outs):
            if cast_out and o.dtype != torch.float32:
                t = Act(eng.buffer('%s.out%d' % (key, i), tuple(o.buf.shape[:4]) + (o.C,)))
                self._cout.append((t, o))
                self.outs.append(t)
            else:
                self.outs.append(o)

    def build(self):
        return self._build(self.ins, self.outs)

    def pre(self):
        for a, is_grad in self._cin:
            self.eng.as_fp32(a, reuse=not is_grad)

    def accumulate(self, acc):
        return 0 if self._cout else int(bool(acc))

    def post(self, acc=False):
        for t, o in self._cout:
            ops.cast(t, o, accumulate=bool(acc))
            self.eng.io_cast_bytes += t.buf.numel() * 4


class Engine:
    def __init__(self, module, ops_list, x_val, head_vals, final_head_index):
        self.module = module
        self.ops = ops_list
        self.x = x_val
        self.heads = head_vals
        self.final_head = final_head_index
        self.device = None
        self._buffers = {}
        self._ws = None
        self._planned = None
        self._packed_version = None
        self._pack_programs = {}
        self.flat = None
        self.flat_grad = None
        self._views = {}
        self.params_version = 0
        self.wstreams = []
        self._wnext = 0
        self._late_pack = None
        self._mid_pack = None
        self._ws_side = {}
        self.bwdw_streams = int(os.environ.get('MT_BWDW_STREAMS', '1'))
        self.grad_ready_hook = None
        self.dummy = None
        self.mma = 0
        self._io_cache = {}
        self._fp32_copies = {}
        self._iter = 0
        self.io_cast_bytes = 0
        self._fuse_norm_bwd = None
        self._one_stream_at_init = self.bwdw_streams == 0
        self.producer, self.pending = {}, {}

    @property
    def fuse_norm_bwd(self):
        if self._fuse_norm_bwd is not None:
            return int(self._fuse_norm_bwd)
        if self._one_stream_at_init:
            return 1
        return 3 if self.mma else 0

    @fuse_norm_bwd.setter
    def fuse_norm_bwd(self, v):
        self._fuse_norm_bwd = v

    def set_precision(self, precision):
        mma = {'fp32': 0, 'bf16': 1, 0: 0, 1: 1, False: 0, True: 1}[precision]
        if mma != self.mma:
            self.mma = mma
            self._replan()

    def _replan(self):
        self._planned = None
        self._packed_version = None
        self._pack_programs = {}
        self._io_cache = {}
        self._fp32_copies.clear()

    def val_dtype(self, spatial):
        return torch.float16 if self.mma else torch.float32

    def grad_dtype(self, spatial):
        return torch.bfloat16 if self.val_dtype(spatial) != torch.float32 else torch.float32

    def io(self, key, ins, outs, build, supported, grad_ins=False):
        gi = list(grad_ins) if isinstance(grad_ins, (list, tuple)) else [bool(grad_ins)] * len(ins)
        sig = (key, tuple(a.dt for a in ins), tuple(o.dt for o in outs))
        flags = self._io_cache.get(sig)
        if flags is None:
            if all(a.dtype == torch.float32 for a in list(ins) + list(outs)):
                flags = (False, False)
            else:
                flags = (True, True)
                for cand in ((False, False), (True, False), (False, True)):
                    if cand[0] and all(a.dtype == torch.float32 for a in ins):
                        continue
                    if cand[1] and all(o.dtype == torch.float32 for o in outs):
                        continue
                    t = _IO(self, key, ins, outs, build, cand, gi)
                    if supported(t.build()):
                        flags = cand
                        break
            self._io_cache[sig] = flags
        return _IO(self, key, ins, outs, build, flags, gi)

    def as_fp32(self, a, reuse=True, geometry_only=False):
        if a.dtype == torch.float32:
            return a
        stream = torch.cuda.current_stream().cuda_stream if a.buf.is_cuda else 0
        key = (a.buf.data_ptr(), a.c0, a.C, tuple(a.buf.shape[:4]), stream)
        ent = self._fp32_copies.get(key)
        if ent is None:
            ent = self._fp32_copies[key] = [torch.empty(tuple(a.buf.shape[:4]) + (a.C,), dtype=torch.float32, device=a.buf.device), -1]
        t = a.with_buf(ent[0])
        if geometry_only:
            return t
        if not (reuse and ent[1] == self._iter):
            ops.cast(Act(a.buf, a.c0, a.C), Act(ent[0]))
            ent[1] = self._iter if reuse else -1
            self.io_cast_bytes += ent[0].numel() * 4
        return t

    def buffer(self, name, shape, dtype=torch.float32):
        t = self._buffers.get(name)
        if t is None or tuple(t.shape) != tuple(shape) or t.dtype != dtype:
            t = torch.empty(shape, dtype=dtype, device=self.device)
            self._buffers[name] = t
        return t

    def workspace(self, nbytes, side=None):
        n = (int(nbytes) + 3) // 4 + 16
        if side is not None:
            t = self._ws_side.get(side)
            if t is None or t.numel() < n:
                if t is not None:
                    torch.cuda.synchronize()
                t = self._ws_side[side] = torch.empty(max(n, 1 << 20), dtype=torch.float32, device=self.device)
            return t
        if self._ws is None or self._ws.numel() < n:
            self._ws = torch.empty(max(n, 1 << 20), dtype=torch.float32, device=self.device)
        return self._ws

    def _side_stream(self):
        return torch.cuda.Stream()

    @contextlib.contextmanager
    def weight_stream(self):
        if not self.wstreams:
            yield None
            return
        i = self._wnext
        self._wnext = (i + 1) % len(self.wstreams)
        st = self.wstreams[i]
        ev = torch.cuda.Event()
        ev.record(torch.cuda.current_stream())
        st.wait_event(ev)
        with torch.cuda.stream(st):
            yield i

    def ordered_params(self):
        seen, out = set(), []
        for op in reversed(self.ops):
            for p in op.param_list():
                if id(p) not in seen:
                    seen.add(id(p))
                    out.append(p)
        rest = [p for p in self.module.parameters() if id(p) not in seen]
        return out + rest

    def attach(self, device):
        params = self.ordered_params()
        ok = self.flat is not None and self.flat.device == device
        if ok:
            lo, hi = self.flat.data_ptr(), self.flat.data_ptr() + 4 * self.flat.numel()
            ok = all(lo <= p.data_ptr() < hi for p in params)
        if ok:
            return
        self.device = device
        if device.type == 'cuda':
            from . import _lib
            _lib.probe_device(device.index if device.index is not None else None)
        offs, n = [], 0
        for p in params:
            offs.append(n)
            n += (p.numel() + 3) // 4 * 4
        flat = torch.zeros(n, dtype=torch.float32, device=device)
        for p, o in zip(params, offs):
            flat[o:o + p.numel()].copy_(p.data.reshape(-1))
            p.data = flat[o:o + p.numel()].view(p.shape)
        self.flat = flat
        self.flat_grad = torch.zeros_like(flat)
        self._views = {id(p): (o, self.flat_grad[o:o + p.numel()].view(p.shape)) for p, o in zip(params, offs)}
        self._op_ranges = []
        for op in reversed(self.ops):
            ps = op.param_list()
            if ps:
                lo = min(self._views[id(p)][0] for p in ps)
                hi = max(self._views[id(p)][0] + (p.numel() + 3) // 4 * 4 for p in ps)
                self._op_ranges.append((op, lo, hi))
        self.dummy = torch.zeros(64, dtype=torch.float32, device=device)
        self._buffers.clear()
        self._fp32_copies.clear()
        self._replan()
        self.params_version += 1

    def grad_of(self, p):
        return self._views[id(p)][1]

    def mark_params_dirty(self):
        self.params_version += 1

    def _plan(self, N, spatial, need_grad):
        key = (N, tuple(spatial), need_grad)
        if self._planned == key:
            return
        self.x.spatial = tuple(spatial)
        for op in self.ops:
# ... 300 lines not shown
```

Baseline: 67.40 patches/s.

## Emulate fp32 strided conv backward-data with three-piece bf16 split MFMA

Adds a split-precision path that decomposes fp32 activations and weights into three bf16 pieces and accumulates six bf16 MFMA products per tap, emulating fp32 accuracy on matrix cores. It is enabled by default for strided non-pointwise convs in fp32 mode for backward-data, and optionally for forward. This adds a new weight pack layout, three LDS images per tile and a second accumulator. The aim is to replace slower fp32 FMA or xf32 convolution in the strided kernels, at the cost of six times the MFMA work, more LDS and extra registers.

```diff
diff --git a/multitalent_amd/csrc/conv_bf16.inc b/multitalent_amd/csrc/conv_bf16.inc
--- a/multitalent_amd/csrc/conv_bf16.inc
+++ b/multitalent_amd/csrc/conv_bf16.inc
@@ -11,22 +11,34 @@
 #include "conv16_common.h"
 
 template <int LD, int LH, int NW> __host__ __device__ constexpr int bstage_rows() { return ((LD * LH + NW - 1) / NW) * NW; }
-template <int LD, int LH, int LW, int VEC, int NW, int PITCH = BFP> __host__ __device__ constexpr int bstage_lwp() {
+template <int LD, int LH, int LW, int VEC, int NW, int PITCH = BFP, int NP = 1> __host__ __device__ constexpr int bstage_lwp() {
   constexpr int vps = 64 / (FCK / VEC);
   constexpr int padded = ((LW + vps - 1) / vps) * vps;
-  return ((size_t)bstage_rows<LD, LH, NW>() * padded * PITCH * 4 <= (PITCH == BFP ? 80 : 40) * 1024) ? padded : LW;
-}
-template <int LD, int LH, int LW, int VEC, int NW, int PITCH = BFP> __host__ __device__ constexpr size_t bstage_lds_bytes() {
-  return (size_t)bstage_rows<LD, LH, NW>() * bstage_lwp<LD, LH, LW, VEC, NW, PITCH>() * PITCH * 4;
-}
-
-template <int LD, int LH, int LW, int VEC, int NW, int XS = MT_F32, int MTY = MT_BF16, int PITCH = BFP>
+  return ((size_t)bstage_rows<LD, LH, NW>() * padded * PITCH * 4 * NP <= (PITCH == BFP ? 80 : 40) * 1024) ? padded : LW;
+}
+template <int LD, int LH, int LW, int VEC, int NW, int PITCH = BFP, int NP = 1, int RPAD = 0> __host__ __device__ constexpr int bstage_image_dwords() {
+  return bstage_rows<LD, LH, NW>() * (bstage_lwp<LD, LH, LW, VEC, NW, PITCH, NP>() * PITCH + RPAD);
+}
+template <int LD, int LH, int LW, int VEC, int NW, int PITCH = BFP, int NP = 1, int RPAD = 0> __host__ __device__ constexpr size_t bstage_lds_bytes() {
+  return (size_t)NP * bstage_image_dwords<LD, LH, LW, VEC, NW, PITCH, NP, RPAD>() * 4;
+}
+
+__device__ __forceinline__ void mt_split3_pk(float x0, float x1, unsigned (&pk)[3]) {
+  pk[0] = mt_pk16<MT_BF16>(x0, x1);
+  const float r0 = x0 - mt_lo16<MT_BF16>(pk[0]), r1 = x1 - mt_hi16<MT_BF16>(pk[0]);
+  pk[1] = mt_pk16<MT_BF16>(r0, r1);
+  pk[2] = mt_pk16<MT_BF16>(r0 - mt_lo16<MT_BF16>(pk[1]), r1 - mt_hi16<MT_BF16>(pk[1]));
+}
+
+template <int LD, int LH, int LW, int VEC, int NW, int XS = MT_F32, int MTY = MT_BF16, int PITCH = BFP, int NP = 1, int RPAD = 0, int SWS = 3>
 __device__ __forceinline__ void mt_stage_bf16(unsigned* __restrict__ lds, const mt_conv3d_t& c, const ConvChunk ch,
                                               int nb, int ud0, int uh0, int uw0, int lane, int wave) {
   constexpr int EB = mt_ebytes<XS>();
   constexpr bool XB = XS != MT_F32;
   constexpr int LPV = FCK / VEC, VPS = 64 / LPV, NI = (LW + VPS - 1) / VPS, R = LD * LH, RPW = (R + NW - 1) / NW;
-  constexpr int LWP = bstage_lwp<LD, LH, LW, VEC, NW, PITCH>();
+  constexpr int LWP = bstage_lwp<LD, LH, LW, VEC, NW, PITCH, NP>();
+  constexpr int ROWP = LWP * PITCH + RPAD, IMG = bstage_image_dwords<LD, LH, LW, VEC, NW, PITCH, NP, RPAD>();
+  static_assert(NP == 1 || (NP == 3 && XS == MT_F32 && MTY == MT_BF16), "three pieces: fp32 source, bf16 matrix type");
   constexpr bool PADW = LWP >= NI * VPS;
   constexpr bool SWZ = PITCH == BFP_SWZ;
   constexpr int RG = (RPW * NI * VEC > 64) ? (RPW + 1) / 2 : RPW;
@@ -35,9 +47,11 @@
   const int cl = (lane % LPV) * VEC, vl = lane / LPV;
   const bool has_aff = S.scale != nullptr;
   float sc[VEC], sh[VEC];
+  unsigned cmask[VEC];
 #pragma unroll
   for (int e = 0; e < VEC; ++e) {
     const bool cv = (cl + e) < ch.ck;
+    cmask[e] = cv ? 0xffffffffu : 0u;
     sc[e] = cv ? 1.f : 0.f; sh[e] = 0.f;
     if (has_aff && cv) {
       sc[e] = S.scale[(size_t)nb * S.C + ch.c0 + cl + e];
@@ -59,10 +73,10 @@
     voff[i] = ok ? (uw * cs + ch.c0 + cl) * EB : (int)0x80000000;
     mval[i] = ok ? 0xffffffffu : 0u;
   }
-  unsigned* lbase = lds + (wave * LWP + vl) * PITCH + (SWZ ? (cl & 7) / 2 : cl / 2);
+  unsigned* lbase = lds + wave * ROWP + vl * PITCH + (SWZ ? (cl & 7) / 2 : cl / 2);
   int hoff[NI];
 #pragma unroll
-  for (int i = 0; i < NI; ++i) hoff[i] = SWZ ? (((cl >> 3) ^ ((vl + i * VPS) >> 3)) & 1) * 4 : 0;
+  for (int i = 0; i < NI; ++i) hoff[i] = SWZ ? (((cl >> 3) ^ ((vl + i * VPS) >> SWS)) & 1) * 4 : 0;
   const int rowbytes = c.Wi * cs * EB;
   if constexpr (XB && XS == MTY && VEC == 4) {
     if (!has_aff) {
@@ -88,7 +102,7 @@
 #pragma unroll
         for (int q = 0; q < RG; ++q) {
           if (r0 + q < RPW) {
-            unsigned* lrow = lbase + NW * (r0 + q) * (LWP * PITCH);
+            unsigned* lrow = lbase + NW * (r0 + q) * ROWP;
 #pragma unroll
             for (int i = 0; i < NI; ++i) {
               if (PADW || (i + 1) * VPS <= LW || vl + i * VPS < LW) {
@@ -142,9 +156,25 @@
           scq[e] = __builtin_bit_cast(float, __builtin_bit_cast(unsigned, sc[e]) & (unsigned)rowm[q]);
           shq[e] = __builtin_bit_cast(float, __builtin_bit_cast(unsigned, sh[e]) & (unsigned)rowm[q]);
         }
-        unsigned* lrow = lbase + NW * (r0 + q) * (LWP * PITCH);
+        unsigned* lrow = lbase + NW * (r0 + q) * ROWP;
 #pragma unroll
         for (int i = 0; i < NI; ++i) {
+          if constexpr (NP == 3) {
+            static_assert(NP == 1 || VEC == 2, "three pieces: channel pairs");
+            const f32x2 xv2 = {v[q][i][0], v[q][i][1]}, sc2 = {sc[0], sc[1]}, sh2 = {sh[0], sh[1]}, sl2 = {slope, slope};
+            const f32x2 t = __builtin_elementwise_fma(xv2, sc2, sh2);
+            const f32x2 u = t * sl2;
+            const unsigned vm = mval[i] & (unsigned)rowm[q];
+            const float y0 = __builtin_bit_cast(float, __builtin_bit_cast(unsigned, fmaxf(t[0], u[0])) & vm & cmask[0]);
+            const float y1 = __builtin_bit_cast(float, __builtin_bit_cast(unsigned, fmaxf(t[1], u[1])) & vm & cmask[VEC - 1]);
+            unsigned pc[3];
+            mt_split3_pk(y0, y1, pc);
+            if (PADW || (i + 1) * VPS <= LW || vl + i * VPS < LW) {
+#pragma unroll
+              for (int pi = 0; pi < 3; ++pi) lrow[pi * IMG + i * VPS * PITCH + hoff[i]] = pc[pi];
+            }
+            continue;
+          }
           unsigned pk[VEC / 2];
 #pragma unroll
           for (int h = 0; h < VEC / 2; ++h) {
@@ -170,36 +200,66 @@
   }
 }
 
-template <int MT, int NT, int LH, int LW, int KD = 3, int MTY = MT_BF16, int PITCH = BFP>
+__device__ __forceinline__ f32x16 mt_mfma_split6(const bf16x8 (&a)[3], const bf16x8 (&b)[3], f32x16 c) {
+  c = __builtin_amdgcn_mfma_f32_32x32x16_bf16(a[1], b[1], c, 0, 0, 0);
+  c = __builtin_amdgcn_mfma_f32_32x32x16_bf16(a[0], b[2], c, 0, 0, 0);
+  c = __builtin_amdgcn_mfma_f32_32x32x16_bf16(a[2], b[0], c, 0, 0, 0);
+  c = __builtin_amdgcn_mfma_f32_32x32x16_bf16(a[0], b[1], c, 0, 0, 0);
+  c = __builtin_amdgcn_mfma_f32_32x32x16_bf16(a[1], b[0], c, 0, 0, 0);
+  return __builtin_amdgcn_mfma_f32_32x32x16_bf16(a[0], b[0], c, 0, 0, 0);
+}
+
+__device__ __forceinline__ void mt_mfma_split6_2(const bf16x8 (&a)[3], const bf16x8 (&b)[3], f32x16& c, f32x16& cs) {
+  cs = __builtin_amdgcn_mfma_f32_32x32x16_bf16(a[1], b[1], cs, 0, 0, 0);
+  cs = __builtin_amdgcn_mfma_f32_32x32x16_bf16(a[0], b[2], cs, 0, 0, 0);
+  cs = __builtin_amdgcn_mfma_f32_32x32x16_bf16(a[2], b[0], cs, 0, 0, 0);
+  cs = __builtin_amdgcn_mfma_f32_32x32x16_bf16(a[0], b[1], cs, 0, 0, 0);
+  cs = __builtin_amdgcn_mfma_f32_32x32x16_bf16(a[1], b[0], cs, 0, 0, 0);
+  c = __builtin_amdgcn_mfma_f32_32x32x16_bf16(a[0], b[0], c, 0, 0, 0);
+}
+
+template <int MT, int NT, int LH, int LW, int KD = 3, int MTY = MT_BF16, int PITCH = BFP, int NP = 1, int RPAD = 0, int IMG = 0, int BPF = BF_BPF>
 __device__ __forceinline__ void bf16_chunk(const unsigned* __restrict__ lds, const int (&abase)[MT][3],
-                                           const unsigned* __restrict__ wlane, int wstride, f32x16 (&acc)[NT][MT]) {
+                                           const unsigned* __restrict__ wlane, int wstride, f32x16 (&acc)[NT][MT], f32x16 (*accs)[MT] = nullptr) {
   constexpr int NTAP = KD * 9;
-  constexpr int NB = BF_BPF + 1;
-  bf16x8 b[NB][NT];
-  bf16x8 a[2][MT];
-#pragma unroll
-  for (int t = 0; t < BF_BPF; ++t)
-#pragma unroll
-    for (int n = 0; n < NT; ++n) b[t][n] = *(const bf16x8*)(wlane + n * wstride + t * 256);
-#pragma unroll
-  for (int m = 0; m < MT; ++m) a[0][m] = *(const bf16x8*)(lds + abase[m][0]);
+  constexpr int NB = BPF + 1;
+  constexpr int ROWP = LW * PITCH + RPAD, WT = NP * 256;
+  static_assert(NP == 1 || (NP == 3 && MTY == MT_BF16), "three pieces are bf16");
+  bf16x8 b[NB][NT][NP];
+  bf16x8 a[2][MT][NP];
+#pragma unroll
+  for (int t = 0; t < BPF; ++t)
+#pragma unroll
+    for (int n = 0; n < NT; ++n)
+#pragma unroll
+      for (int q = 0; q < NP; ++q) b[t][n][q] = *(const bf16x8*)(wlane + n * wstride + t * WT + q * 256);
+#pragma unroll
+  for (int m = 0; m < MT; ++m)
+#pragma unroll
+    for (int q = 0; q < NP; ++q) a[0][m][q] = *(const bf16x8*)(lds + abase[m][0] + q * IMG);
 #pragma unroll
   for (int t = 0; t < NTAP; ++t) {
-    if (t + BF_BPF < NTAP)
-#pragma unroll
-      for (int n = 0; n < NT; ++n) b[(t + BF_BPF) % NB][n] = *(const bf16x8*)(wlane + n * wstride + (t + BF_BPF) * 256);
+    if (t + BPF < NTAP)
+#pragma unroll
+      for (int n = 0; n < NT; ++n)
+#pragma unroll
+        for (int q = 0; q < NP; ++q) b[(t + BPF) % NB][n][q] = *(const bf16x8*)(wlane + n * wstride + (t + BPF) * WT + q * 256);
     if (t + 1 < NTAP) {
       const int t1 = t + 1;
-      const int toff = (((t1 / 9) * LH + (t1 / 3) % 3) * LW + t1 % 3) * PITCH;
-#pragma unroll
-      for (int m = 0; m < MT; ++m) a[t1 & 1][m] = *(const bf16x8*)(lds + abase[m][t1 % 3] + toff);
+      const int toff = ((t1 / 9) * LH + (t1 / 3) % 3) * ROWP + (t1 % 3) * PITCH;
+#pragma unroll
+      for (int m = 0; m < MT; ++m)
+#pragma unroll
+        for (int q = 0; q < NP; ++q) a[t1 & 1][m][q] = *(const bf16x8*)(lds + abase[m][t1 % 3] + toff + q * IMG);
     }
     __builtin_amdgcn_sched_barrier(0);
 #pragma unroll
     for (int m = 0; m < MT; ++m)
 #pragma unroll
-      for (int n = 0; n < NT; ++n)
-        acc[n][m] = mt_mfma16<MTY>(a[t & 1][m], b[t % NB][n], acc[n][m]);
+      for (int n = 0; n < NT; ++n) {
+        if constexpr (NP == 3) mt_mfma_split6_2(a[t & 1][m], b[t % NB][n], acc[n][m], accs[n][m]);
+        else acc[n][m] = mt_mfma16<MTY>(a[t & 1][m][0], b[t % NB][n][0], acc[n][m]);
+      }
     __builtin_amdgcn_sched_barrier(0);
   }
 }
diff --git a/multitalent_amd/csrc/conv_lds.hip b/multitalent_amd/csrc/conv_lds.hip
--- a/multitalent_amd/csrc/conv_lds.hip
+++ b/multitalent_amd/csrc/conv_lds.hip
@@ -568,14 +568,16 @@
 #ifndef FS_ABL
 #define FS_ABL 0
 #endif
-template <int SD, int SH, int SW, int VEC, bool BF = false, int XS = MT_F32, int OS = MT_F32, int MTY = MT_BF16>
+template <int SD, int SH, int SW, int VEC, bool BF = false, int XS = MT_F32, int OS = MT_F32, int MTY = MT_BF16, int NP = 1>
 __global__ __launch_bounds__(256) void conv_fast_strided_kernel(const ConvKParams P) {
   static_assert(BF || (XS == MT_F32 && OS == MT_F32), "16-bit storage is served by the 16-bit matrix path");
+  static_assert(NP == 1 || (NP == 3 && BF && XS == MT_F32 && OS == MT_F32 && MTY == MT_BF16 && SW == 2), "three pieces: fp32 storage, bf16 products");
   constexpr bool OB = OS != MT_F32;
   constexpr int TD = 2, TH = 4, TW = 8;
   constexpr int LD = (TD - 1) * SD + 3, LH = (TH - 1) * SH + 3, LW = (TW - 1) * SW + 3;
-  constexpr int LWP = BF ? bstage_lwp<LD, LH, LW, VEC, 4>() : stage_lwp<LD, LH, LW, VEC>();
-  constexpr int PITCH = BF ? BFP : FCKP;
+  constexpr int PITCH = BF ? (NP == 3 ? BFP_SWZ : BFP) : FCKP, RPAD = NP == 3 ? 4 : 0;
+  constexpr int LWP = BF ? bstage_lwp<LD, LH, LW, VEC, 4, PITCH, NP>() : stage_lwp<LD, LH, LW, VEC>();
+  constexpr int ROWP = LWP * PITCH + RPAD;
   extern __shared__ __attribute__((aligned(16))) float lds[];
   const mt_conv3d_t& c = P.c;
   const int tid = threadIdx.x, lane = tid & 63;
@@ -591,17 +593,26 @@
   const int od0 = td * TD, oh0 = th * TH, ow0 = tw * TW;
 
   int abase[1];
-  abase[0] = ((dm * SD * LH + (li >> 3) * SH) * LWP + (li & 7) * SW) * PITCH + lhalf * (BF ? 4 : 8);
-  f32x16 accb[1][1];
+  abase[0] = (dm * SD * LH + (li >> 3) * SH) * ROWP + (li & 7) * SW * PITCH + (NP == 3 ? 0 : lhalf * (BF ? 4 : 8));
+  f32x16 accb[1][1], accs[1][1];
   f32x16 (&acc)[1] = accb[0];
 #pragma unroll
-  for (int j = 0; j < 16; ++j) acc[0][j] = 0.f;
+  for (int j = 0; j < 16; ++j) { acc[0][j] = 0.f; accs[0][0][j] = 0.f; }
 
   for (int ch = 0; ch < P.nchunks; ++ch) {
     const ConvChunk cc = P.chunk[ch];
     __syncthreads();
     if constexpr (BF) {
-      const unsigned* wlane = (const unsigned*)c.wpack + (size_t)(ntile * P.nchunks + ch) * (27 * 256) + lane * 4;
+      const unsigned* wlane = (const unsigned*)c.wpack + (size_t)(ntile * P.nchunks + ch) * (27 * 256 * NP) + lane * 4;
+      if constexpr (NP == 3) {
+        constexpr int IMG = bstage_image_dwords<LD, LH, LW, VEC, 4, PITCH, NP, RPAD>();
+        if (!(FS_ABL & 1)) mt_stage_bf16<LD, LH, LW, VEC, 4, XS, MTY, PITCH, NP, RPAD, 1>((unsigned*)lds, c, cc, nb, od0 * SD - 1, oh0 * SH - 1, ow0 * SW - 1, lane, wave);
+        __syncthreads();
+        const int j = li & 7;
+        const int abase3[1][3] = {{abase[0] + ((lhalf ^ j) & 1) * 4, abase[0] + ((lhalf ^ j) & 1) * 4, abase[0] + ((lhalf ^ (j + 1)) & 1) * 4}};
+        if (!(FS_ABL & 8)) bf16_chunk<1, 1, LH, LWP, 3, MTY, PITCH, NP, RPAD, IMG, 4>((const unsigned*)lds, abase3, wlane, 0, accb, accs);
+        continue;
+      }
       mt_stage_bf16<LD, LH, LW, VEC, 4, XS, MTY>((unsigned*)lds, c, cc, nb, od0 * SD - 1, oh0 * SH - 1, ow0 * SW - 1, lane, wave);
       __syncthreads();
       const int abase3[1][3] = {{abase[0], abase[0], abase[0]}};
@@ -612,6 +623,10 @@
       __syncthreads();
       if (!(FS_ABL & 8)) fast_chunk<1, LH, LWP>(lds, abase, wlane, acc);
     }
+  }
+  if constexpr (NP == 3) {
+#pragma unroll
+    for (int j = 0; j < 16; ++j) acc[0][j] += accs[0][0][j];
   }
   if ((FS_ABL & 4) && acc[0][0] != 12345.f) return;
 
@@ -1431,13 +1446,14 @@
 #ifndef BDS_ABL
 #define BDS_ABL 0
 #endif
-template <int SD, int SH, int SW, int VEC, bool BF = false, int XS = MT_F32, int OS = MT_F32>
+template <int SD, int SH, int SW, int VEC, bool BF = false, int XS = MT_F32, int OS = MT_F32, int NP = 1>
 __global__ __launch_bounds__(256) __attribute__((amdgpu_waves_per_eu(2))) void conv_bwdd_strided_kernel(const ConvKParams P) {
   static_assert(BF || (XS == MT_F32 && OS == MT_F32), "16-bit storage is served by the bf16 matrix path");
+  static_assert(NP == 1 || (NP == 3 && BF && XS == MT_F32 && OS == MT_F32), "three pieces: fp32 storage, bf16 products");
   constexpr bool OB = OS != MT_F32;
   constexpr int TD = 2, TH = 4, TW = 16;
   constexpr int LD = TD + (SD == 2 ? 1 : 2), LH = TH + (SH == 2 ? 1 : 2), LW = TW + (SW == 2 ? 1 : 2);
-  constexpr int NC = SD * SH * SW, LWP = BF ? bstage_lwp<LD, LH, LW, VEC, 4>() : stage_lwp<LD, LH, LW, VEC>();
+  constexpr int NC = SD * SH * SW, LWP = BF ? bstage_lwp<LD, LH, LW, VEC, 4, BFP, NP>() : stage_lwp<LD, LH, LW, VEC>();
   constexpr int PITCH = BF ? BFP : FCKP;
   extern __shared__ __attribute__((aligned(16))) float lds[];
   const mt_conv3d_t& c = P.c;
@@ -1462,29 +1478,38 @@
     const float* wlane = c.wpack + (size_t)(ntile * P.nchunks + ch) * (27 * 512) + lane * 4;
     __syncthreads();
     if constexpr (BF) {
-      mt_stage_bf16<LD, LH, LW, VEC, 4, XS, MT_BF16>((unsigned*)lds, c, cc, nb, md0 - (SD == 1 ? 1 : 0), mh0 - (SH == 1 ? 1 : 0), mw0 - (SW == 1 ? 1 : 0), lane, wave);
+      constexpr int IMG = bstage_image_dwords<LD, LH, LW, VEC, 4, BFP, NP>();
+      if (!(BDS_ABL & 1)) mt_stage_bf16<LD, LH, LW, VEC, 4, XS, MT_BF16, BFP, NP>((unsigned*)lds, c, cc, nb, md0 - (SD == 1 ? 1 : 0), mh0 - (SH == 1 ? 1 : 0), mw0 - (SW == 1 ? 1 : 0), lane, wave);
       __syncthreads();
       const unsigned* ldsu = (const unsigned*)lds;
-      const unsigned* wl = (const unsigned*)c.wpack + (size_t)(ntile * P.nchunks + ch) * (27 * 256) + lane * 4;
-      constexpr int BPF = 5, NB = BPF + 1;
-      bf16x8 b[NB], a[2];
-#pragma unroll
-      for (int t = 0; t < BPF; ++t) b[t] = *(const bf16x8*)(wl + t * 256);
+      const unsigned* wl = (const unsigned*)c.wpack + (size_t)(ntile * P.nchunks + ch) * (27 * 256 * NP) + lane * 4;
+      constexpr int BPF = NP == 3 ? 3 : 5, NB = BPF + 1;
+      bf16x8 b[NB][NP], a[2][NP];
+#pragma unroll
+      for (int t = 0; t < BPF; ++t)
+#pragma unroll
+        for (int pc = 0; pc < NP; ++pc) b[t][pc] = *(const bf16x8*)(wl + (t * NP + pc) * 256);
       {
         constexpr int o0 = ((bd_off<SD>(0) * LH + bd_off<SH>(0)) * LWP + bd_off<SW>(0)) * PITCH;
-        a[0] = *(const bf16x8*)(ldsu + abase + o0);
+#pragma unroll
+        for (int pc = 0; pc < NP; ++pc) a[0][pc] = *(const bf16x8*)(ldsu + abase + o0 + pc * IMG);
       }
 #pragma unroll
       for (int t = 0; t < 27; ++t) {
-        if (t + BPF < 27) b[(t + BPF) % NB] = *(const bf16x8*)(wl + (t + BPF) * 256);
+        if (t + BPF < 27)
+#pragma unroll
+          for (int pc = 0; pc < NP; ++pc) b[(t + BPF) % NB][pc] = *(const bf16x8*)(wl + ((t + BPF) * NP + pc) * 256);
         if (t + 1 < 27) {
           const int t1 = t + 1;
           const int o1 = ((bd_off<SD>(t1 / 9) * LH + bd_off<SH>((t1 / 3) % 3)) * LWP + bd_off<SW>(t1 % 3)) * PITCH;
-          a[t1 & 1] = *(const bf16x8*)(ldsu + abase + o1);
+#pragma unroll
+          for (int pc = 0; pc < NP; ++pc) a[t1 & 1][pc] = *(const bf16x8*)(ldsu + abase + o1 + pc * IMG);
         }
         __builtin_amdgcn_sched_barrier(0);
         const int q = (bd_par<SD>(t / 9) * SH + bd_par<SH>((t / 3) % 3)) * SW + bd_par<SW>(t % 3);
-        acc[q] = __builtin_amdgcn_mfma_f32_32x32x16_bf16(a[t & 1], b[t % NB], acc[q], 0, 0, 0);
+        if (BDS_ABL & 8) { acc[q][0] += (float)a[t & 1][NP - 1][0] + (float)b[t % NB][NP - 1][3]; continue; }
+        if constexpr (NP == 3) acc[q] = mt_mfma_split6(a[t & 1], b[t % NB], acc[q]);
+        else acc[q] = __builtin_amdgcn_mfma_f32_32x32x16_bf16(a[t & 1][0], b[t % NB][0], acc[q], 0, 0, 0);
         __builtin_amdgcn_sched_barrier(0);
       }
       continue;
@@ -1807,6 +1832,13 @@
 static bool strided_use_bf16(const mt_conv3d_t* p) {
   return mt_sel3(p, MT_SEL_M16) && p->mma == 1 && p->Cin >= 16 && conv_fast_vec(p) == 2;
 }
+#ifndef SPLIT3_FWD
+#define SPLIT3_FWD 1
+#endif
+static bool strided_use_split3(const mt_conv3d_t* p) {
+  return SPLIT3_FWD && mt_sel3(p, MT_SEL_M16) && p->mma == 2 && p->Cin >= 16 && conv_fast_vec(p) == 2 && conv_src_dtype(p) == MT_F32 &&
+         p->odtype == MT_F32;
+}
 
 static bool conv_x16_geometry_ok(const mt_conv3d_t* p, int cfg) {
   if (cfg != 0 || p->mma != 1) return false;
@@ -1905,6 +1937,7 @@
   int ck;
   int vec, xs, os, mty;
   bool m16;
+  int np;
   bool nt2;
   bool bstats;
   bool fast;
@@ -1914,7 +1947,7 @@
   const int cfg = pick_cfg(p), sd = conv_src_dtype(p);
   c.family = cfg < 0 ? CONV_NONE : CONV_GENERIC;
   if (cfg >= 0) c.g = kCfgs[cfg];
-  c.ck = c.g.CK; c.vec = conv_fast_vec(p); c.xs = MT_F32; c.os = MT_F32; c.mty = MT_BF16;
+  c.ck = c.g.CK; c.vec = conv_fast_vec(p); c.xs = MT_F32; c.os = MT_F32; c.mty = MT_BF16; c.np = 1;
   auto strided_instance = [&] {
     c.m16 = strided_use_bf16(p);
     if (c.m16 && sd > 0) { c.vec = 4; c.xs = sd; c.os = p->odtype == sd ? sd : MT_F32; c.mty = sd == MT_F16 ? MT_F16 : MT_BF16; }
@@ -1954,6 +1987,7 @@
     const long wgs = (long)p->N * mt_cdiv(p->Do, 2) * mt_cdiv(p->Ho, 4) * mt_cdiv(p->Wo, 8) * mt_cdiv(p->Cout, 64);
     const bool inst = c.m16 ? mt_is16(sd) && (p->odtype == sd || p->odtype == MT_F32) : (sd == MT_F32 && p->odtype == MT_F32 && c.vec == 2);
     if (g_tapsplit && (wgs < 256 || g_tapsplit >= 2) && inst) c.family = CONV_TAPSPLIT;
+    else if (strided_use_split3(p)) { c.m16 = true; c.np = 3; }
     return c;
   }
   if (conv_rt_ok(p)) {
@@ -1986,6 +2020,7 @@
 }
 extern "C" int mt_conv3d_pack_layout(const mt_conv3d_t* p) {
   const ConvChoice c = conv_resolve(p);
+  if (c.np == 3) return 5;
   if (c.m16) return c.mty == MT_F16 ? 4 : 3;
   return (c.family == CONV_WINO || c.family == CONV_WINO_B) ? 2 : 1;
 }
@@ -2036,7 +2071,10 @@
       if (p->SH == 2) snprintf(buf, n, "conv_tapsplit_kernel<%d, %s, %d, %d, %d, %d, 2, 2>", c.vec, b, c.xs, c.os, c.mty, p->SD);
       else snprintf(buf, n, "conv_tapsplit_kernel<%d, %s, %d, %d, %d>", c.vec, b, c.xs, c.os, c.mty);
       break;
-    case CONV_FAST_STRIDED: snprintf(buf, n, "conv_fast_strided_kernel<%d, %d, %d, %d, %s, %d, %d, %d>", p->SD, p->SH, p->SW, c.vec, b, c.xs, c.os, c.mty); break;
+    case CONV_FAST_STRIDED:
+      snprintf(buf, n, c.np == 3 ? "conv_fast_strided_kernel<%d, %d, %d, %d, %s, %d, %d, %d, 3>" : "conv_fast_strided_kernel<%d, %d, %d, %d, %s, %d, %d, %d>",
+               p->SD, p->SH, p->SW, c.vec, b, c.xs, c.os, c.mty);
+      break;
     case CONV_BF16: snprintf(buf, n, "conv_bf16_kernel<%d, %d, %d, %d, 1, 4, %d, %d, %d, %d>", g.MW, g.RH, g.TD, c.vec, p->KD, c.xs, c.os, c.mty); break;
     case CONV_X16: snprintf(buf, n, "conv_x16_kernel<%d, %d>", p->KD, c.xs); break;
     case CONV_GATHER: snprintf(buf, n, c.m16 ? "conv_gather_kernel<%d, %d, %d, true>" : c.nt2 ? "conv_gather_kernel<%d, %d, %d, false, 2>" : "conv_gather_kernel<%d, %d, %d>", c.vec, c.xs, c.os); break;
@@ -2104,6 +2142,9 @@
   if (int rc = conv_fill(P, p, conv_tile(c), 27, FCK)) return rc;
   const dim3 grid = conv_grid(P, 64);
 #define MT_FS_LAUNCH(XS_, OS_, MTY_) hipLaunchKernelGGL((conv_fast_strided_kernel<SD, 2, 2, 4, true, XS_, OS_, MTY_>), grid, dim3(256), (bstage_lds_bytes<LD, LH, LW, 4, 4>()), st, P)
+  if (c.np == 3)
+    return conv_launch_lds(conv_fast_strided_kernel<SD, 2, 2, 2, true, MT_F32, MT_F32, MT_BF16, 3>, grid, dim3(256),
+                           bstage_lds_bytes<LD, LH, LW, 2, 4, BFP_SWZ, 3, 4>(), st, P, "conv3d_fast_strided");
   if (c.m16 && c.vec == 4) MT_IO16_SWITCH(c, MT_FS_LAUNCH);
   else if (c.m16) hipLaunchKernelGGL((conv_fast_strided_kernel<SD, 2, 2, 2, true, MT_F32, MT_F32, MT_BF16>), grid, dim3(256), (bstage_lds_bytes<LD, LH, LW, 2, 4>()), st, P);
   else if (c.vec == 2) hipLaunchKernelGGL((conv_fast_strided_kernel<SD, 2, 2, 2>), grid, dim3(256), (stage_lds_bytes<LD, LH, LW, 2>()), st, P);
@@ -2316,11 +2357,15 @@
 }
 
 
-struct BwddChoice { bool ks, m16; int vec, xs, os; };
+struct BwddChoice { bool ks, m16; int vec, xs, os, np; };
+#ifndef SPLIT3_BWDD
+#define SPLIT3_BWDD 1
+#endif
 static BwddChoice bwdd_resolve(const mt_conv3d_t* p) {
   const mt_src_t& s0 = p->src[0];
   const bool pairs = !((s0.cs & 1) || (s0.C & 1));
   BwddChoice c = {};
+  c.np = 1;
   c.m16 = mt_sel3(p, MT_SEL_M16) && p->mma == 1 && p->Cout >= 16 && pairs && !(((uintptr_t)s0.ptr) & (mt_is16(s0.dtype) ? 3 : 7));
   c.vec = (pairs && !(((uintptr_t)s0.ptr) & 7)) ? 2 : 1;
   if (c.m16) {
@@ -2333,9 +2378,16 @@
     const long wgs = (long)p->N * mt_cdiv(mt_cdiv(p->Di, p->SD), 2) * mt_cdiv(mt_cdiv(p->Hi, 2), 4) * mt_cdiv(mt_cdiv(p->Wi, 2), 16) * mt_cdiv(p->Cin, 32);
     c.ks = wgs < 256 || g_tapsplit >= 2;
   }
+  if (SPLIT3_BWDD && !c.ks && mt_sel3(p, MT_SEL_M16) && p->mma == 2 && mt_conv3d_bwd_data_strided_supported(p) && p->Cout >= 16 && s0.dtype == MT_F32 && p->odtype == MT_F32 && c.vec == 2) {
+    c.m16 = true; c.np = 3; c.xs = MT_F32; c.os = MT_F32;
+  }
   return c;
 }
-extern "C" int mt_conv3d_bwd_data_strided_pack_layout(const mt_conv3d_t* p) { return (p != nullptr && bwdd_resolve(p).m16) ? 3 : 1; }
+extern "C" int mt_conv3d_bwd_data_strided_pack_layout(const mt_conv3d_t* p) {
+  if (p == nullptr) return 1;
+  const BwddChoice c = bwdd_resolve(p);
+  return c.np == 3 ? 5 : c.m16 ? 3 : 1;
+}
 static int bwdd_io_served(const mt_conv3d_t* p, const BwddChoice& c) {
   if (!mt_dtype_ok(p->src[0].dtype) || !mt_dtype_ok(p->odtype)) return 0;
   if (p->src[0].dtype == MT_F32 && p->odtype == MT_F32) return 1;
@@ -2365,6 +2417,9 @@
     MT_CHECK_LAUNCH("conv_bwdd_strided_ks");
     return MT_OK;
   }
+  if (c.np == 3)
+    return conv_launch_lds(conv_bwdd_strided_kernel<SD, SH, SW, 2, true, MT_F32, MT_F32, 3>, grid, dim3(256), bstage_lds_bytes<LD, LH, LW, 2, 4, BFP, 3>(), st, P,
+                           "conv_bwdd_strided");
   if (c.m16 && c.vec == 4) hipLaunchKernelGGL((conv_bwdd_strided_kernel<SD, SH, SW, 4, true, MT_BF16, MT_BF16>), grid, dim3(256), (bstage_lds_bytes<LD, LH, LW, 4, 4>()), st, P);
   else if (c.m16 && c.os == MT_BF16) hipLaunchKernelGGL((conv_bwdd_strided_kernel<SD, SH, SW, 2, true, MT_F32, MT_BF16>), grid, dim3(256), (bstage_lds_bytes<LD, LH, LW, 2, 4>()), st, P);
   else if (c.m16) hipLaunchKernelGGL((conv_bwdd_strided_kernel<SD, SH, SW, 2, true>), grid, dim3(256), (bstage_lds_bytes<LD, LH, LW, 2, 4>()), st, P);
@@ -2387,6 +2442,7 @@
   if (p == nullptr || buf == nullptr || n == 0 || !mt_conv3d_bwd_data_strided_supported(p)) return MT_EINVAL;
   const BwddChoice c = bwdd_resolve(p);
   if (c.ks) snprintf(buf, n, "conv_bwdd_strided_ks_kernel<%d, 2, 2>", p->SD);
+  else if (c.np == 3) snprintf(buf, n, "conv_bwdd_strided_kernel<%d, 2, 2, %d, true, %d, %d, 3>", p->SD, c.vec, c.xs, c.os);
   else snprintf(buf, n, "conv_bwdd_strided_kernel<%d, 2, 2, %d, %s, %d, %d>", p->SD, c.vec, c.m16 ? "true" : "false", c.xs, c.os);
   return MT_OK;
 }
@@ -2412,7 +2468,7 @@
 __device__ __forceinline__ void pack_weights_tiled(const PackParams& P, float* __restrict__ tile, int blk, int nblk) {
   const int K3 = P.KD * P.KH * P.KW;
   const int nq = P.layout == 1 ? P.nkp / 4 : 1;
-  const int per_tap = nq * 256;
+  const int nitem = nq * 256, per_tap = P.layout == 5 ? 3 * 256 : nitem;
   const int tid = threadIdx.x;
   for (int g = blk; g < P.ntiles * P.nchunks; g += nblk) {
     const int nt = g / P.nchunks, ch = g - nt * P.nchunks;
@@ -2437,7 +2493,7 @@
     }
     __syncthreads();
     float* dst = P.dst + (size_t)g * K3 * per_tap;
-    for (int i = tid; i < per_tap; i += 256) {
+    for (int i = tid; i < nitem; i += 256) {
       const int e = i & 3, l = (i >> 2) & 63, qq = i >> 8;
       const int co = l & 31;
       const int c0 = P.layout == 1 ? (l >> 5) * P.nkp + qq * 4 + e : (l >> 5) * 8 + 2 * e;
@@ -2449,6 +2505,10 @@
         if (P.layout == 1) dst[(size_t)tap * per_tap + i] = a0;
         else {
           const float a1 = v1 ? tp[K3 + zt] : 0.f;
+          if (P.layout == 5) {
+            unsigned pc[3]; mt_split3_pk(a0, a1, pc);
+            for (int q = 0; q < 3; ++q) ((unsigned*)dst)[(size_t)tap * per_tap + q * 256 + i] = pc[q];
+          } else
           ((unsigned*)dst)[(size_t)tap * per_tap + i] = P.layout == 3 ? mt_pk16<MT_BF16>(a0, a1) : mt_pk16<MT_F16>(a0, a1);
         }
       }
@@ -2519,11 +2579,11 @@
     }
     return;
   }
-  if (P.layout == 1 || P.layout == 3 || P.layout == 4) {
+  if (P.layout == 1 || P.layout == 3 || P.layout == 4 || P.layout == 5) {
     const int K3 = P.KD * P.KH * P.KW;
     const int nq = P.layout == 1 ? P.nkp / 4 : 1;
-    const int per_tap = nq * 256;
-    const long items = (long)P.ntiles * P.nchunks * per_tap;
+    const int nitem = nq * 256, per_tap = P.layout == 5 ? 3 * 256 : nitem;
+    const long items = (long)P.ntiles * P.nchunks * nitem;
     for (long i = first; i < items; i += stride) {
       long r = i;
       const int e = (int)(r % 4); r /= 4;
@@ -2556,6 +2616,10 @@
           if (tap < K3) {
             if (P.layout == 1) dp[(size_t)tap * per_tap] = a0[tap];
             else if (P.layout == 3) ((unsigned*)dp)[(size_t)tap * per_tap] = mt_pk16<MT_BF16>(a0[tap], a1[tap]);
+            else if (P.layout == 5) {
+              unsigned pc[3]; mt_split3_pk(a0[tap], a1[tap], pc);
+              for (int pq = 0; pq < 3; ++pq) ((unsigned*)dp)[(size_t)tap * per_tap + pq * 256] = pc[pq];
+            }
             else ((unsigned*)dp)[(size_t)tap * per_tap] = mt_pk16<MT_F16>(a0[tap], a1[tap]);
           }
         continue;
@@ -2570,6 +2634,10 @@
             const float a0 = v0 ? w0[o] : 0.f;
             if (P.layout == 1) dp[(size_t)tap * per_tap] = a0;
             else if (P.layout == 3) ((unsigned*)dp)[(size_t)tap * per_tap] = mt_pk16<MT_BF16>(a0, v1 ? w0[o + P.s_ci] : 0.f);
+            else if (P.layout == 5) {
+              unsigned pc[3]; mt_split3_pk(a0, v1 ? w0[o + P.s_ci] : 0.f, pc);
+              for (int pq = 0; pq < 3; ++pq) ((unsigned*)dp)[(size_t)tap * per_tap + pq * 256] = pc[pq];
+            }
             else ((unsigned*)dp)[(size_t)tap * per_tap] = mt_pk16<MT_F16>(a0, v1 ? w0[o + P.s_ci] : 0.f);
           }
     }
@@ -2621,14 +2689,15 @@
                      const int32_t* tapmap) {
   MT_REQUIRE(ck >= 2 && (ck % 2) == 0, "pack: ck must be even (got %d)", ck);
   MT_REQUIRE(layout == 0 || (layout == 1 && (ck % 8) == 0) || (layout == 2 && ck == 8 && KD == 3 && KH == 3 && KW == 3 && tapmap == nullptr) ||
-             ((layout == 3 || layout == 4) && ck == 16),
-             "pack: layout 1 needs ck %% 8 == 0; layout 2 (Winograd) needs ck == 8 and a 3x3x3 kernel; layouts 3 / 4 (bf16 / fp16) need ck == 16");
+             ((layout == 3 || layout == 4 || layout == 5) && ck == 16),
+             "pack: layout 1 needs ck %% 8 == 0; layout 2 (Winograd) needs ck == 8 and a 3x3x3 kernel; layouts 3 / 4 / 5 (bf16 / fp16 / bf16 pieces) need ck == 16");
   std::memset((void*)&P, 0, sizeof(P));
   P.nchunks = mt_build_chunks(C0, C1, ck, P.chunk);
   MT_REQUIRE(P.nchunks > 0, "pack: too many chunks");
   P.ntiles = mt_cdiv(Cout, 32);
   P.nkp = ck / 2;
   if (packed_floats) *packed_floats = layout == 2 ? (size_t)P.ntiles * P.nchunks * 64 * 256
+                                    : layout == 5 ? (size_t)P.ntiles * P.nchunks * KD * KH * KW * 3 * 256
                                     : layout >= 3 ? (size_t)P.ntiles * P.nchunks * KD * KH * KW * 256
                                                   : (size_t)P.ntiles * P.nchunks * KD * KH * KW * P.nkp * 64;
   P.w = w; P.dst = dst; P.Cout = Cout; P.KD = KD; P.KH = KH; P.KW = KW; P.flip = flip; P.layout = layout;
diff --git a/multitalent_amd/engine.py b/multitalent_amd/engine.py
--- a/multitalent_amd/engine.py
+++ b/multitalent_amd/engine.py
@@ -70,6 +70,9 @@
         Cout = self.conv.out_channels
         self.pw_strided = self._pw_strided_geom and tuple(o * st for o, st in zip(self.geom.out, self.stride)) == tuple(self.geom.inp)
         self.mma = eng.mma
+        split = eng.mma == 0 and eng.split_fp32 and self.stride != (1, 1, 1) and not self.pointwise
+        self.mma_b = 2 if split else self.mma
+        self.mma_f = 2 if split and eng.split_fp32_forward else self.mma
         buf = eng.buffer(self.name + '.y', (N,) + self.geom.out + (Cout,), self._out_dtype(eng))
         if self.norm is not None:
             st = eng.buffer(self.name + '.stats', (4, N, Cout))
@@ -91,7 +94,7 @@
                 return ops.fill_pointwise(a, self.geom.out, a.spatial, self.stride, (1, 1, 1), Cout, eng.dummy, self.conv.bias, outs[0],
                                           mma=eng.mma if self.pointwise else 0)
             return eng.io(self.name + '.fwd', acts, [self.out.act], build, ops.pointwise_io_supported)
-        build = lambda ins, outs: ops.fill_conv(ins, self.geom, Cout, bias=self.conv.bias, out0=outs[0], mma=self.mma)
+        build = lambda ins, outs: ops.fill_conv(ins, self.geom, Cout, bias=self.conv.bias, out0=outs[0], mma=self.mma_f)
         return eng.io(self.name + '.fwd', acts, [self.out.act], build, ops.conv_io_supported)
 
     def _fwd_params(self, eng, io=None):
@@ -152,7 +155,7 @@
         dx = Act(s0.grad) if s0.grad is not None else Act(self._grad_like(eng, s0))
 
         def build(ins, outs):
-            p = ops.fill_conv(ins, self.geom, self.conv.out_channels, out0=outs[0], mma=self.mma)
+            p = ops.fill_conv(ins, self.geom, self.conv.out_channels, out0=outs[0], mma=self.mma_b)
             p.Cin = s0.C
             return p
         return eng.io(self.name + '.bwdd', [gact], [dx], build, ops.conv_bwd_data_strided_io_supported, grad_ins=True)
@@ -556,6 +559,8 @@
         self.grad_ready_hook = None
         self.dummy = None
         self.mma = 0
+        self._split_fp32 = True
+        self._split_fp32_forward = False
         self._io_cache = {}
         self._fp32_copies = {}
         self._iter = 0
@@ -575,6 +580,26 @@
     @fuse_norm_bwd.setter
     def fuse_norm_bwd(self, v):
         self._fuse_norm_bwd = v
+
+    @property
+    def split_fp32(self):
+        return self._split_fp32
+
+    @split_fp32.setter
+    def split_fp32(self, on):
+        if bool(on) != self._split_fp32:
+            self._split_fp32 = bool(on)
+            self._replan()
+
+    @property
+    def split_fp32_forward(self):
+        return self._split_fp32_forward
+
+    @split_fp32_forward.setter
+    def split_fp32_forward(self, on):
+        if bool(on) != self._split_fp32_forward:
+            self._split_fp32_forward = bool(on)
+            self._replan()
 
     def set_precision(self, precision):
         mma = {'fp32': 0, 'bf16': 1, 0: 0, 1: 1, False: 0, True: 1}[precision]
```

Result: no change. 68.02 patches/s (median of 6 runs) (+0.9%).
